# tphakala/go-audio-resampler

Hardware: AMD Instinct MI355X
Metric: Msamples/s resampled (float32, 44.1k→48k QualityHigh) + RMS error vs Go ref (higher is better)
Workload: dtype f32

## Files before the change

### go-audio-resampler_amd/csrc/gar_engine.cpp

```cpp
#include <hip/hip_runtime.h>
#include <immintrin.h>

#include <algorithm>
#include <chrono>
#include <atomic>
#include <cmath>
#include <condition_variable>
#include <cstdio>
#include <cstdlib>
#include <cstring>
#include <functional>
#include <memory>
#include <mutex>
#include <string>
#include <thread>
#include <type_traits>
#include <vector>

#include "gar.h"
#include "gar_design.hpp"
#include "gar_hxs_launch.hpp"
#include "gar_kernels.hpp"
#include "gar_plan.hpp"
#include "gar_pool.hpp"
// ... 133 lines not shown
    d.hRbK0 = p.rbAligned ? p.rbK0.data() : nullptr;
    for (size_t rb = 0; p.rbAligned && rb + 1 < p.rbStart.size(); ++rb)
        d.maxPrb = std::max(d.maxPrb, p.rbStart[rb + 1] - p.rbStart[rb]);
    if (dry) return d;
    if (p.f64) A.upload(p.A64); else A.upload(p.A32);
    std::vector<int> t = p.progTable();
    const std::vector<int> rt = p.redTable();
    const size_t redOff = t.size();
    t.insert(t.end(), rt.begin(), rt.end());
    const size_t rbOff = t.size();
    t.insert(t.end(), p.rbStart.begin(), p.rbStart.end());
    T.upload(t);
    d.A = A.p;
    d.progs = static_cast<const int*>(T.p);
    d.reds = static_cast<const int*>(T.p) + redOff;
    d.rbStart = p.rbAligned ? static_cast<const int*>(T.p) + rbOff : nullptr;
    return d;
}

void attachExact(const BgPlan& p, DevBuf& X, StageRT& s, BgDev& d, bool dry) {
    d.xRowMax = p.rowMax;
    d.xTwoStage = p.twoStage ? 1 : 0;
    d.xT1 = s.d.dft.taps;
    d.xT2 = s.d.poly.taps;
    if (dry) return;
    const size_t nr = p.rows.size(), ni = p.rowInfo.size();
    const size_t listOff = (nr * 8 + ni * 4 + 15) / 16 * 16;
    X.ensure(listOff + kBgNfListBytes);
    HIPCHK(hipMemcpy(X.p, p.rows.data(), nr * 8, hipMemcpyHostToDevice));
    HIPCHK(hipMemcpy(static_cast<char*>(X.p) + nr * 8, p.rowInfo.data(), ni * 4, hipMemcpyHostToDevice));
    HIPCHK(hipMemset(static_cast<char*>(X.p) + listOff, 0, kBgNfListBytes));
    d.xRows = static_cast<const double*>(X.p);
    d.xInfo = reinterpret_cast<const int*>(static_cast<const char*>(X.p) + nr * 8);
    d.nfList = reinterpret_cast<int*>(static_cast<char*>(X.p) + listOff);
    if (p.twoStage) {
        if (!s.xBankA.p) s.xBankA.upload(s.d.poly.a);
        if (!s.xBankC.p) s.xBankC.upload(s.d.dft.c);
        d.xPolyA = static_cast<const double*>(s.xBankA.p);
        d.xDftC = static_cast<const double*>(s.xBankC.p);
    }
}

template <class T>
void uploadBank(const std::vector<double>& v, DevBuf& b) {
    std::vector<T> c(v.begin(), v.end());
    b.upload(c);
}

bool buildStage(StageRT& s, bool f64, bool hx, bool dry, std::string& err) {
    s.f64 = f64;
    hx = hx && !f64;
    const EngineDesign& d = s.d;
    if (d.kind == EngineKind::Cubic) return true;
    if (d.kind == EngineKind::DftOnly || d.kind == EngineKind::DftPoly) {
        if (!buildBgPlan(firFromDft(d.dft), f64, s.dftP)) { err = "DFT plan"; return false; }
        s.dftD = uploadPlan(s.dftP, s.dftA, s.dftT, dry);
        attachExact(s.dftP, s.dftX, s, s.dftD, dry);
        if (hx) attachHx(firFromDft(d.dft), s.dftH, s.dftD, dry, d);
    }
    if (d.kind == EngineKind::Decim) {
        if (!buildBgPlan(firFromDecim(d.decim), f64, s.decimP)) { err = "decimator plan"; return false; }
        s.decimD = uploadPlan(s.decimP, s.decimA, s.decimT, dry);
        attachExact(s.decimP, s.decimX, s, s.decimD, dry);
        if (hx) attachHx(firFromDecim(d.decim), s.decimH, s.decimD, dry, d);
    }
    if (d.kind == EngineKind::DftPoly) {
        if (firComposite(d.dft, d.poly, s.compositeFir) && buildBgPlan(s.compositeFir, f64, s.fusedP)) {
            s.fused = true;
            s.fusedD = uploadPlan(s.fusedP, s.fusedA, s.fusedT, dry);
            attachExact(s.fusedP, s.fusedX, s, s.fusedD, dry);
            if (hx) attachHx(s.compositeFir, s.fusedH, s.fusedD, dry, d);
        }
        PolyDev& p = s.polyD;
        p.f64 = f64 ? 1 : 0;
        p.L = d.poly.L;
        p.T = d.poly.taps;
        p.step = d.poly.step;
        if (!dry) {
            if (f64) {
                uploadBank<double>(d.poly.a, s.pa); uploadBank<double>(d.poly.b, s.pb);
                uploadBank<double>(d.poly.cc, s.pc); uploadBank<double>(d.poly.d, s.pd);
            } else {
                uploadBank<float>(d.poly.a, s.pa); uploadBank<float>(d.poly.b, s.pb);
                uploadBank<float>(d.poly.cc, s.pc); uploadBank<float>(d.poly.d, s.pd);
            }
            p.a = s.pa.p; p.b = s.pb.p; p.c = s.pc.p; p.d = s.pd.p;
            std::vector<double> il(4 * d.poly.a.size());
            for (size_t i = 0; i < d.poly.a.size(); ++i) {
                il[4 * i] = d.poly.a[i]; il[4 * i + 1] = d.poly.b[i]; il[4 * i + 2] = d.poly.cc[i]; il[4 * i + 3] = d.poly.d[i];
            }
            if (f64) uploadBank<double>(il, s.pabcd); else uploadBank<float>(il, s.pabcd);
            p.abcd = s.pabcd.p;
        }
    }
    return true;
}

int stageLatency(const EngineDesign& d) {
    if (d.kind == EngineKind::Cubic) return 2;
    int lat = 0;
    if ((d.kind == EngineKind::DftOnly || d.kind == EngineKind::DftPoly) && d.dft.factor > 1)
        lat += (d.dft.taps * d.dft.factor) / 2;
    if (d.kind == EngineKind::DftPoly) lat += d.poly.taps / 2;
    return lat;
}

struct Counters {
    bool staged = false;
    int64_t x_count = 0;
    int64_t dft_hist = 0;
    int64_t poly_hist = 0;
    int64_t at = 0;
    int64_t u_base = 0;
    int64_t u_count = 0;
    int64_t dec_hist = 0;
    int dec_phase = 0;
    int64_t y_count = 0;
    double cub_phase = 0.0;
};

int64_t cntDft(Counters& s, const DftBank& b, int64_t n) {
    if (b.factor == 1) return n;
    if (n == 0) return 0;
    s.x_count += n;
    s.dft_hist += n;
    if (s.dft_hist < b.taps) return 0;
    const int64_t p = s.dft_hist - b.taps + 1;
    s.dft_hist -= p;
    return p * b.factor;
}

int64_t cntPoly(Counters& s, const PolyBank& b, int64_t m, bool& quirk) {
    if (m == 0) return 0;
    s.poly_hist += m;
    s.u_count += m;
    const int64_t numIn = s.poly_hist - b.taps + 1;
    if (numIn <= 0) return 0;
    const int64_t L = b.L;
    const int64_t limit = (numIn * L) << 16;
    const int64_t nout = (limit - s.at + b.step - 1) / b.step;
    if (nout <= 0) return 0;
    const int64_t at = s.at + nout * b.step;
    const int64_t consumed = (at >> 16) / L;
    if (consumed > 0 && consumed <= s.poly_hist) {
        s.poly_hist -= consumed;
        s.u_base += consumed;
    } else if (consumed > s.poly_hist) {
        quirk = true;
    }
    s.at = at - ((consumed * L) << 16);
    return nout;
}

int64_t cntDecim(Counters& s, const DecimBank& b, int64_t n) {
    if (b.factor == 1) return n;
    if (n == 0) return 0;
    s.x_count += n;
    s.dec_hist += n;
    if (s.dec_hist < b.taps) return 0;
    const int64_t nf = s.dec_hist - b.taps + 1;
    const int64_t nout = s.dec_phase < nf ? (nf - s.dec_phase + b.factor - 1) / b.factor : 0;
    if (nout == 0) return 0;
    s.dec_phase = static_cast<int>(((s.dec_phase - nf) % b.factor + b.factor) % b.factor);
    s.dec_hist -= nf;
    return nout;
}

namespace {
struct CubicRot {
    int F = 0;
    int64_t S = 0, P0 = 0;
};
bool cubicRotation(double step, double ph, CubicRot& r) {
    int e = 0;
    (void)std::frexp(step, &e);
    r.F = 53 - e;
    if (r.F < 1 || r.F > 60) return false;
    const double Sd = std::ldexp(step, r.F), Pd = std::ldexp(ph, r.F);
    if (Sd != std::floor(Sd) || Pd != std::floor(Pd) || Pd < 0.0 || Pd >= Sd) return false;
    r.S = static_cast<int64_t>(Sd);
    r.P0 = static_cast<int64_t>(Pd);
    const int64_t one = int64_t(1) << r.F;
    int bits = 0;
    for (uint64_t v = static_cast<uint64_t>(one + r.S - 1); v; v >>= 1) ++bits;
    const int64_t grid = bits > 53 ? (int64_t(1) << (bits - 53)) : 1;
    return r.S % grid == 0 && r.P0 % grid == 0 && one % grid == 0;
}
}

int64_t cntCubic(Counters& s, double ratio, int64_t n, std::vector<CubicSeg>* segs, int* segLen = nullptr) {
    const double step = 1.0 / ratio;
    CubicRot rot;
    if (n > 0 && cubicRotation(step, s.cub_phase, rot)) {
        const __int128 one = static_cast<__int128>(1) << rot.F, S = rot.S, P0 = rot.P0;
        auto phaseAt = [&](int64_t i) {
            __int128 v = (P0 - static_cast<__int128>(i) * one) % S;
            return v < 0 ? v + S : v;
        };
        auto outsBefore = [&](int64_t i, __int128 Pi) {
            return static_cast<int64_t>((static_cast<__int128>(i) * one + Pi - P0) / S);
        };
        if (segs)
            for (int64_t i = 0; i < n; i += (segLen ? *segLen : kCubicSegInputs)) {
                const __int128 Pi = phaseAt(i);
                segs->push_back({std::ldexp(static_cast<double>(static_cast<int64_t>(Pi)), -rot.F), s.y_count + outsBefore(i, Pi),
                                 s.x_count + i});
            }
        const __int128 Pn = phaseAt(n);
        const int64_t nout = outsBefore(n, Pn);
        s.cub_phase = std::ldexp(static_cast<double>(static_cast<int64_t>(Pn)), -rot.F);
        s.x_count += n;
        return nout;
    }
    if (segLen) *segLen = static_cast<int>(kCubicSegInputs);
    double ph = s.cub_phase;
    int64_t nout = 0;
    for (int64_t i = 0; i < n; ++i) {
        if (segs && i % kCubicSegInputs == 0) segs->push_back({ph, s.y_count + nout, s.x_count + i});
        while (ph < 1.0) {
            ++nout;
            ph += step;
        }
        ph -= 1.0;
    }
    s.cub_phase = ph;
    s.x_count += n;
    return nout;
}

struct Hist {
    DevBuf buf[2];
    int cur = 0;
    int64_t base = 0, len = 0;
    bool zero = false;
    void* ptr() const { return zero ? nullptr : buf[cur].p; }
    void clear() { base = 0; len = 0; zero = false; }
};

struct StageDev {
    Hist xh;
    Hist uh;
};

struct InView {
    const void* p = nullptr;
    int64_t fs = 0, cs = 0;
    int f64 = 0;
    int pcm = 0;
    int64_t n = 0;
    bool zeros = false;
};

struct OutView {
    void* p = nullptr;
    int64_t fs = 0, cs = 0;
    int f64 = 0;
    int pcm = 0;
};

struct PinBuf {
    void* p = nullptr;
    size_t cap = 0;
    hipEvent_t ev = nullptr;
    bool pending = false;
    PinBuf() = default;
    PinBuf(const PinBuf&) = delete;
    PinBuf& operator=(const PinBuf&) = delete;
    PinBuf(PinBuf&& o) noexcept : p(o.p), cap(o.cap), ev(o.ev), pending(o.pending) { o.p = nullptr; o.ev = nullptr; o.cap = 0; o.pending = false; }
    PinBuf& operator=(PinBuf&& o) noexcept {
        if (this != &o) {
            release();
            p = o.p; cap = o.cap; ev = o.ev; pending = o.pending;
            o.p = nullptr; o.ev = nullptr; o.cap = 0; o.pending = false;
        }
        return *this;
    }
    ~PinBuf() { release(); }
    void release() {
        if (ev) { (void)hipEventSynchronize(ev); (void)hipEventDestroy(ev); }
        if (p) (void)hipHostFree(p);
        p = nullptr; ev = nullptr; cap = 0; pending = false;
    }
    void* acquire(size_t bytes) {
        if (pending) HIPCHK(hipEventSynchronize(ev));
        pending = false;
        if (!ev) HIPCHK(hipEventCreateWithFlags(&ev, hipEventDisableTiming));
        if (bytes > cap) {
            if (p) HIPCHK(hipHostFree(p));
            p = nullptr;
            cap = 0;
            const size_t nb = bytes + bytes / 2 + 4096;
            HIPCHK(hipHostMalloc(&p, nb, hipHostMallocDefault));
            cap = nb;
        }
        return p;
    }
    void issued(hipStream_t s) {
        HIPCHK(hipEventRecord(ev, s));
        pending = true;
    }
};

struct HostBuf {
    void* p = nullptr;
    size_t cap = 0;
    unsigned flags = 0;
    HostBuf() = default;
    explicit HostBuf(unsigned f) : flags(f) {}
    HostBuf(const HostBuf&) = delete;
    HostBuf& operator=(const HostBuf&) = delete;
    ~HostBuf() { release(); }
    void release() {
        if (p) (void)hipHostFree(p);
        p = nullptr;
        cap = 0;
    }
    void* ensure(size_t bytes) {
        if (bytes <= cap) return p;
        release();
        const size_t nb = bytes + bytes / 4 + 4096;
        HIPCHK(hipHostMalloc(&p, nb, hipHostMallocMapped | flags));
        cap = nb;
        return p;
    }
};

inline void forSlices(int C, int64_t n, size_t bytesPerSample, const std::function<void(int, int64_t, int64_t)>& f) {
    const size_t total = static_cast<size_t>(C) * static_cast<size_t>(std::max<int64_t>(n, 0)) * bytesPerSample;
    if (total < (size_t(1) << 20)) {
        for (int c = 0; c < C; ++c) f(c, 0, n);
        return;
    }
    Pool& pool = Pool::get();
    const int J = pool.workers() * 2;
    if (C >= J) {
        pool.run(J, [&](int j) {
            for (int c = static_cast<int>(static_cast<int64_t>(C) * j / J); c < static_cast<int64_t>(C) * (j + 1) / J; ++c) f(c, 0, n);
        });
        return;
    }
    const int per = std::max<int>(1, (J + C - 1) / C);
    const int64_t step = (n + per - 1) / per;
    pool.run(C * per, [&](int i) {
        const int c = i / per, k = i - c * per;
        const int64_t lo = k * step, hi = std::min<int64_t>(n, lo + step);
        if (lo < hi) f(c, lo, hi);
    });
}

struct Group {
    int c0 = 0, C = 1;
    std::vector<Counters> cnt;
    int64_t statIn = 0, statOut = 0;
    std::vector<StageDev> dev;
    std::vector<DevBuf> tmp;
    DevBuf utmp;
    PinBuf cubPin[2];
    int cubCur = 0;
    std::vector<CubicSeg> cubSegs;
};

}
}

struct gar_resampler {
    bool newPath = true;
    int channels = 1;
    double ratio = 1.0;
    bool f64 = true;
    bool hx = false;
    bool dry = false;
    int device = 0;
    bool engineF32Io = false;
    hipStream_t stream = nullptr;
    hipEvent_t orderEv = nullptr;
    hipStream_t lastStream = nullptr;
    bool orderValid = false;
    bool unordered = false;
    bool multiStream = false;
    bool poisoned = false;
    hipEvent_t failEv = nullptr;
    bool failEvValid = false;
    int* errHost = nullptr;
    int* errDev = nullptr;
    gar_config cfg{};
    std::vector<std::unique_ptr<gar::StageRT>> stages;
    std::vector<gar::Group> groups;
    gar::DevBuf inStage, outStage;
    gar::HostBuf hostIn{hipHostMallocWriteCombined | hipHostMallocCoherent}, hostOut{hipHostMallocCoherent};
    std::vector<int64_t> scratchSizes;
    bool profile = false;
    uint32_t profileKinds = 0x3f;
    struct Ev { int tag; hipEvent_t a, b; };
    std::vector<Ev> events;
    std::vector<std::pair<hipEvent_t, hipEvent_t>> evPool;
    double profiledMs[6] = {0, 0, 0, 0, 0, 0};
    int64_t profiledLaunches[6] = {0, 0, 0, 0, 0, 0};
    std::vector<float> launchMs[6], readMs[6];
};

namespace gar {
namespace {

using Handle = gar_resampler;

constexpr size_t kPinKeep = size_t(64) << 20;
void trimHost(Handle* h) {
    if (h->hostIn.cap > kPinKeep) h->hostIn.release();
    if (h->hostOut.cap > kPinKeep) h->hostOut.release();
}

struct Ctx {
    Handle* h;
    Group* g;
    hipStream_t s;
    bool launch;
};

template <class L>
hipError_t timed(Ctx& x, int tag, L&& launch) {
    if (!x.h->profile || !((x.h->profileKinds >> tag) & 1u)) return launch();
    hipEvent_t a, b;
    if (!x.h->evPool.empty()) {
        a = x.h->evPool.back().first;
        b = x.h->evPool.back().second;
        x.h->evPool.pop_back();
    } else {
        HIPCHK(hipEventCreateWithFlags(&a, hipEventDisableSystemFence));
        HIPCHK(hipEventCreateWithFlags(&b, hipEventDisableSystemFence));
    }
    HIPCHK(hipEventRecord(a, x.s));
    const hipError_t e = launch();
    HIPCHK(hipEventRecord(b, x.s));
    x.h->events.push_back({tag, a, b});
    return e;
}

hipError_t timedBg(Ctx& x, int tag, const BgDev& p, const SrcDesc& src, const OutDesc& od, int C,
                   HistCopy* hc = nullptr) {
    return timed(x, tag, [&] { return launchBg(p, src, od, C, x.s, hc); });
}

SrcDesc mkSrc(const Hist& hs, int C, int64_t x0, const InView& in) {
    SrcDesc s{};
    s.hist = hs.ptr();
    s.hist_base = hs.base;
    s.hist_len = hs.len;
    s.hist_ld = C;
    s.in = in.zeros ? nullptr : in.p;
    s.in_base = x0;
    s.in_len = in.zeros ? 0 : in.n;
    s.in_fs = in.fs;
    s.in_cs = in.cs;
    s.in_f64 = in.f64;
    s.in_pcm = in.zeros ? 0 : in.pcm;
    s.valid_end = in.zeros ? x0 : x0 + in.n;
    return s;
}

thread_local int* g_curErr = nullptr;

OutDesc mkOut(const OutView& o, int64_t o0, int64_t n) {
    OutDesc d{};
    d.err = g_curErr;
    d.out = o.p;
    d.o0 = o0;
    d.fs = o.fs;
    d.cs = o.cs;
    d.f64 = o.f64;
    d.pcm = o.pcm;
    d.o_lo = o0;
    d.o_hi = o0 + n;
    return d;
}

void hist_update(Ctx& x, Hist& hs, const SrcDesc& src, int64_t k0, int64_t k1) {
    const int C = x.g->C;
    const int tc = x.h->f64 ? 8 : 4;
    if (k1 < k0) k1 = k0;
    if (!x.launch) { hs.base = k0; hs.len = k1 - k0; hs.zero = false; return; }
    const int other = 1 - hs.cur;
    hs.buf[other].ensure(static_cast<size_t>(std::max<int64_t>(k1 - k0, 1)) * C * tc);
    HIPCHK(launchGather(x.h->f64, src, hs.buf[other].p, k0, k1 - k0, C, x.s));
    hs.cur = other;
    hs.base = k0;
    hs.len = k1 - k0;
    hs.zero = false;
}

template <class L>
void withHist(Ctx& x, Hist& hs, const SrcDesc& src, int64_t k0, int64_t k1, bool launch, L&& l) {
    HistCopy hc;
    const int other = 1 - hs.cur;
    if (x.launch && launch && k1 > k0) {
        hs.buf[other].ensure(static_cast<size_t>(k1 - k0) * x.g->C * (x.h->f64 ? 8 : 4));
        hc.dst = hs.buf[other].p;
        hc.t0 = k0;
        hc.n = k1 - k0;
    }
    if (x.launch && launch) HIPCHK(l(&hc));
    if (hc.done) {
        hs.cur = other;
        hs.base = k0;
        hs.len = k1 - k0;
        hs.zero = false;
    } else {
        hist_update(x, hs, src, k0, k1);
    }
}

void materialize(Ctx& x, StageRT& rt, Counters& c, StageDev& dv, const SrcDesc& xsrc) {
    const int C = x.g->C;
    const int tc = rt.tc();
    if (x.launch) {
        Hist& uh = dv.uh;
        const int other = 1 - uh.cur;
        const int64_t n = c.u_count - c.u_base;
        uh.buf[other].ensure(static_cast<size_t>(std::max<int64_t>(n, 1)) * C * tc);
        OutView ov{uh.buf[other].p, C, 1, rt.f64 ? 1 : 0};
        HIPCHK(timedBg(x, 1, rt.dftD, xsrc, mkOut(ov, c.u_base, n), C));
        uh.cur = other;
        uh.base = c.u_base;
        uh.len = n;
    } else {
        dv.uh.base = c.u_base;
        dv.uh.len = c.u_count - c.u_base;
    }
    hist_update(x, dv.xh, xsrc, c.x_count - c.dft_hist, c.x_count);
    c.staged = true;
}

int64_t stageProcess(Ctx& x, int si, const InView& in, const OutView& out) {
    StageRT& rt = *x.h->stages[si];
    Counters& c = x.g->cnt[si];
    StageDev& dv = x.g->dev[si];
    const int C = x.g->C;
    const EngineDesign& d = rt.d;
    const int64_t n = in.n;
    if (n == 0) return 0;
    switch (d.kind) {
        case EngineKind::Cubic: {
            const int64_t x0 = c.x_count;
            std::vector<CubicSeg>* segs = x.launch ? &x.g->cubSegs : nullptr;
            if (segs) segs->clear();
            const SrcDesc src = mkSrc(dv.xh, C, x0, in);
            const int64_t y0 = c.y_count;
            int segLen = n * C <= (int64_t(1) << 20) ? kCubicSegInputsShort : static_cast<int>(kCubicSegInputs);
            const int64_t nout = cntCubic(c, d.ratio, n, segs, &segLen);
            if (x.launch && nout > 0) {
                PinBuf& pb = x.g->cubPin[x.g->cubCur];
                x.g->cubCur ^= 1;
                void* hp = pb.acquire(segs->size() * sizeof(CubicSeg));
                std::memcpy(hp, segs->data(), segs->size() * sizeof(CubicSeg));
                HIPCHK(timed(x, 5, [&] {
                    return launchCubic(rt.f64 ? 1 : 0, static_cast<const CubicSeg*>(hp), static_cast<int64_t>(segs->size()),
                                       c.x_count, 1.0 / d.ratio, src, mkOut(out, y0, nout), C, x.s, segLen);
                }));
                pb.issued(x.s);
            }
            hist_update(x, dv.xh, src, std::max<int64_t>(0, c.x_count - 3), c.x_count);
            c.y_count += nout;
            return nout;
        }
        case EngineKind::Passthrough: {
            if (x.launch && !in.zeros) {
                HIPCHK(launchCopy(in.p, in.f64, in.fs, in.cs, out.p, out.f64, out.fs, out.cs, n, C, x.s));
            }
            c.y_count += n;
            return n;
        }
        case EngineKind::DftOnly: {
            const int64_t x0 = c.x_count;
            const int64_t y0 = c.y_count;
            const int64_t nout = cntDft(c, d.dft, n);
            const SrcDesc src = mkSrc(dv.xh, C, x0, in);
            withHist(x, dv.xh, src, c.x_count - c.dft_hist, c.x_count, nout > 0,
                     [&](HistCopy* hc) { return timedBg(x, 1, rt.dftD, src, mkOut(out, y0, nout), C, hc); });
            c.y_count += nout;
            return nout;
        }
        case EngineKind::Decim: {
            const int64_t x0 = c.x_count;
            const int64_t y0 = c.y_count;
            const int64_t nout = cntDecim(c, d.decim, n);
            const SrcDesc src = mkSrc(dv.xh, C, x0, in);
            withHist(x, dv.xh, src, c.x_count - c.dec_hist, c.x_count, nout > 0,
                     [&](HistCopy* hc) { return timedBg(x, 2, rt.decimD, src, mkOut(out, y0, nout), C, hc); });
            c.y_count += nout;
            return nout;
        }
        case EngineKind::DftPoly: {
            const int64_t x0 = c.x_count;
            const int64_t y0 = c.y_count;
            const Counters before = c;
            const SrcDesc xsrc = mkSrc(dv.xh, C, x0, in);
            const int64_t nu = cntDft(c, d.dft, n);
            bool quirk = false;
            const int64_t nout = cntPoly(c, d.poly, nu, quirk);
            if (!c.staged) {
                if (quirk) {
                    if (x.launch && nout > 0) HIPCHK(timedBg(x, 0, rt.fusedD, xsrc, mkOut(out, y0, nout), C));
                    materialize(x, rt, c, dv, xsrc);
                } else {
                    withHist(x, dv.xh, xsrc, c.u_base / 2, c.x_count, nout > 0, [&](HistCopy* hc) {
                        return timedBg(x, 0, rt.fusedD, xsrc, mkOut(out, y0, nout), C, hc);
                    });
                }
            } else {
                const int64_t p0 = before.x_count - before.dft_hist;
                const int64_t dy0 = p0 * d.dft.factor;
                InView uin;
                if (x.launch) x.g->utmp.ensure(static_cast<size_t>(std::max<int64_t>(nu, 1)) * C * rt.tc());
                withHist(x, dv.xh, xsrc, c.x_count - c.dft_hist, c.x_count, nu > 0, [&](HistCopy* hc) {
                    OutView uv{x.g->utmp.p, C, 1, rt.f64 ? 1 : 0};
                    return timedBg(x, 1, rt.dftD, xsrc, mkOut(uv, dy0, nu), C, hc);
                });
                uin.p = x.g->utmp.p; uin.fs = C; uin.cs = 1; uin.f64 = rt.f64 ? 1 : 0; uin.n = nu;
                const SrcDesc usrc = mkSrc(dv.uh, C, before.u_count, uin);
                if (x.launch && nout > 0) {
                    PolyDev p = rt.polyD;
                    p.at0 = before.at;
                    p.u_base = before.u_base;
                    p.m0 = before.y_count;
                    HIPCHK(timed(x, 4, [&] { return launchPoly(p, usrc, mkOut(out, y0, nout), nout, C, x.s); }));
                }
                if (nu > 0) hist_update(x, dv.uh, usrc, c.u_base, c.u_count);
            }
            c.y_count += nout;
            return nout;
        }
        default:
            throw DevError{hipErrorNotSupported, "unsupported stage"};
    }
}

int64_t stageFlush(Ctx& x, int si, const OutView& out) {
    StageRT& rt = *x.h->stages[si];
    Counters& c = x.g->cnt[si];
    StageDev& dv = x.g->dev[si];
    const int C = x.g->C;
    const EngineDesign& d = rt.d;
    InView z;
    z.zeros = true;
    switch (d.kind) {
        case EngineKind::Passthrough:
            return 0;
        case EngineKind::DftOnly:
            if (c.dft_hist == 0) return 0;
            z.n = d.dft.taps;
            return stageProcess(x, si, z, out);
        case EngineKind::Decim:
            if (c.dec_hist == 0) return 0;
            z.n = d.decim.taps;
            return stageProcess(x, si, z, out);
        case EngineKind::DftPoly: {
            if (!c.staged) {
                InView none;
                none.zeros = true;
                const SrcDesc xsrc = mkSrc(dv.xh, C, c.x_count, none);
                Counters t = c;
                bool quirk = false;
                int64_t nA = 0, nB = 0;
                if (t.dft_hist > 0) nA = cntPoly(t, d.poly, cntDft(t, d.dft, d.dft.taps), quirk);
                if (t.poly_hist > 0) nB = cntPoly(t, d.poly, d.poly.taps, quirk);
                if (!quirk) {
                    const int64_t y0 = c.y_count, n = nA + nB;
                    if (x.launch && n > 0) HIPCHK(timedBg(x, 3, rt.fusedD, xsrc, mkOut(out, y0, n), C));
                    c = t;
                    c.y_count = y0 + n;
                    c.staged = true;
                    dv.xh.base = c.x_count - c.dft_hist;
                    dv.xh.len = c.dft_hist;
                    dv.xh.zero = true;
                    dv.uh.base = c.u_base;
                    dv.uh.len = c.u_count - c.u_base;
                    dv.uh.zero = true;
                    return n;
                }
                materialize(x, rt, c, dv, xsrc);
            }
            int64_t total = 0;
            if (c.dft_hist > 0) {
                z.n = d.dft.taps;
                total += stageProcess(x, si, z, out);
            }
            if (c.poly_hist > 0) {
                const int64_t y0 = c.y_count;
                const Counters before = c;
                bool quirk = false;
                const int64_t nout = cntPoly(c, d.poly, d.poly.taps, quirk);
                InView uz;
                uz.zeros = true;
                uz.n = d.poly.taps;
                const SrcDesc usrc = mkSrc(dv.uh, C, before.u_count, uz);
                OutView o2 = out;
                if (x.launch && nout > 0) {
                    const int es = out.f64 ? 8 : 4;
                    o2.p = static_cast<char*>(out.p) + total * out.fs * es;
                    PolyDev p = rt.polyD;
                    p.at0 = before.at;
                    p.u_base = before.u_base;
                    p.m0 = before.y_count;
                    HIPCHK(timed(x, 4, [&] { return launchPoly(p, usrc, mkOut(o2, y0, nout), nout, C, x.s); }));
                }
                hist_update(x, dv.uh, usrc, c.u_base, c.u_count);
                c.y_count += nout;
                total += nout;
            }
            return total;
        }
        default:
            return 0;
    }
}

OutView offsetView(const OutView& o, int64_t rows) {
    OutView r = o;
    if (o.p) r.p = static_cast<char*>(o.p) + rows * o.fs * (o.pcm ? pcmBytes(o.pcm) : (o.f64 ? 8 : 4));
    return r;
}

int64_t chainProcess(Ctx& x, const InView& in, const OutView& out, std::vector<int64_t>& sizes) {
    const int ns = static_cast<int>(x.h->stages.size());
    sizes.assign(ns, 0);
    if (ns == 0) {
        if (x.launch && in.n > 0)
            HIPCHK(launchCopy(in.p, in.f64, in.fs, in.cs, out.p, out.f64, out.fs, out.cs, in.n, x.g->C, x.s));
        return in.n;
    }
    InView cur = in;
    for (int i = 0; i < ns; ++i) {
        const bool last = i == ns - 1;
        OutView o = out;
        if (!last) {
            const int tc = x.h->f64 ? 8 : 4;
            if (x.launch) {
                x.g->tmp[i].ensure(static_cast<size_t>(std::max<int64_t>(x.h->scratchSizes[i], 1)) * x.g->C * tc);
                o = OutView{x.g->tmp[i].p, x.g->C, 1, x.h->f64 ? 1 : 0};
            }
        }
        int64_t m = 0;
        if (cur.n >= 1) m = stageProcess(x, i, cur, o);
        sizes[i] = m;
        InView nx;
        nx.p = o.p; nx.fs = o.fs; nx.cs = o.cs; nx.f64 = o.f64; nx.n = m;
        cur = nx;
    }
    return cur.n;
}

int64_t chainFlush(Ctx& x, const OutView& out, std::vector<int64_t>& sizes) {
    const int ns = static_cast<int>(x.h->stages.size());
    sizes.assign(ns, 0);
    if (ns == 0) return 0;
    InView pending;
    for (int i = 0; i < ns; ++i) {
        const bool last = i == ns - 1;
        OutView o = out;
        if (!last && x.launch) {
            const int tc = x.h->f64 ? 8 : 4;
            x.g->tmp[i].ensure(static_cast<size_t>(std::max<int64_t>(x.h->scratchSizes[i], 1)) * x.g->C * tc);
            o = OutView{x.g->tmp[i].p, x.g->C, 1, x.h->f64 ? 1 : 0};
        }
        int64_t m = 0;
        if (pending.n > 0) m += stageProcess(x, i, pending, o);
        m += stageFlush(x, i, offsetView(o, m));
        sizes[i] = m;
        InView nx;
        nx.p = o.p; nx.fs = o.fs; nx.cs = o.cs; nx.f64 = o.f64; nx.n = m;
        pending = nx;
    }
    return pending.n;
}

Group* groupOf(Handle* h, int ch) {
    for (auto& g : h->groups)
        if (ch >= g.c0 && ch < g.c0 + g.C) return &g;
    return nullptr;
}

Group freshGroup(Handle* h, int c0, int C) {
    Group g;
    g.c0 = c0;
    g.C = C;
    const size_t ns = h->stages.size();
    g.cnt.assign(ns, Counters());
    g.dev.resize(ns);
    g.tmp.resize(ns);
    for (size_t i = 0; i < ns; ++i)
        if (!h->stages[i]->fused) g.cnt[i].staged = true;
    return g;
}

Group splitCopy(Handle* h, Group& g, int k0, int kc) {
    Group ng = freshGroup(h, g.c0 + k0, kc);
    const int tc = h->f64 ? 8 : 4;
    for (size_t i = 0; i < h->stages.size(); ++i) {
        ng.cnt[i] = g.cnt[i];
        ng.statIn = g.statIn;
        ng.statOut = g.statOut;
        Hist* src[2] = {&g.dev[i].xh, &g.dev[i].uh};
        Hist* dst[2] = {&ng.dev[i].xh, &ng.dev[i].uh};
        for (int k = 0; k < 2; ++k) {
            dst[k]->base = src[k]->base;
            dst[k]->len = src[k]->len;
            dst[k]->zero = src[k]->zero;
            if (!h->dry && src[k]->len > 0 && !src[k]->zero) {
                dst[k]->buf[0].ensure(static_cast<size_t>(src[k]->len) * kc * tc);
                const char* sp = static_cast<const char*>(src[k]->ptr()) + static_cast<size_t>(k0) * tc;
                HIPCHK(launchCopy(sp, h->f64, g.C, 1, dst[k]->buf[0].p, h->f64, kc, 1, src[k]->len, kc, h->stream));
            }
        }
    }
    return ng;
}

void isolate(Handle* h, int ch) {
    Group* g = groupOf(h, ch);
    if (!g || g->C == 1) return;
    std::vector<Group> out;
    for (auto& gg : h->groups) {
        if (&gg != g) { out.push_back(std::move(gg)); continue; }
        const int k = ch - gg.c0;
        if (k > 0) out.push_back(splitCopy(h, gg, 0, k));
        out.push_back(splitCopy(h, gg, k, 1));
        if (k + 1 < gg.C) out.push_back(splitCopy(h, gg, k + 1, gg.C - k - 1));
    }
    if (!h->dry) HIPCHK(hipStreamSynchronize(h->stream));
    h->groups = std::move(out);
}

int64_t simulate(Handle* h, Group& g, int64_t n, bool flush, std::vector<int64_t>& sizes) {
    Group sim;
    sim.c0 = g.c0;
    sim.C = g.C;
    sim.cnt = g.cnt;
    sim.dev.resize(g.dev.size());
    for (size_t i = 0; i < g.dev.size(); ++i) {
        sim.dev[i].xh.base = g.dev[i].xh.base; sim.dev[i].xh.len = g.dev[i].xh.len;
        sim.dev[i].uh.base = g.dev[i].uh.base; sim.dev[i].uh.len = g.dev[i].uh.len;
    }
    Ctx x{h, &sim, nullptr, false};
    InView in;
    in.n = n;
    OutView o;
    return flush ? chainFlush(x, o, sizes) : chainProcess(x, in, o, sizes);
}

void countStats(const Handle* h, Group& g, int64_t nIn, int64_t nOut, bool flush) {
    if (!flush) {
        if (nIn <= 0) return;
        g.statIn += nIn;
        g.statOut += nOut;
        return;
    }
    const bool cubicEngine = !h->newPath && h->stages.size() == 1 && h->stages[0]->d.kind == EngineKind::Cubic;
    if (!cubicEngine) g.statOut += nOut;
}

int64_t runGroup(Handle* h, Group& g, const InView& in, const OutView& out, bool flush, hipStream_t s,
                 int64_t cap, gar_status& st) {
    std::vector<int64_t> sizes;
    const int64_t n = simulate(h, g, in.n, flush, sizes);
    if (n > cap) { st = GAR_ERR_BUFFER_TOO_SMALL; return n; }
    st = GAR_OK;
    if (h->dry) {
        Ctx x{h, &g, nullptr, false};
        std::vector<int64_t> s2;
        OutView o;
        if (flush) chainFlush(x, o, s2); else chainProcess(x, in, o, s2);
        countStats(h, g, in.n, n, flush);
        return n;
    }
    h->scratchSizes = sizes;
    Ctx x{h, &g, s, true};
    std::vector<int64_t> s2;
    const int64_t got = flush ? chainFlush(x, out, s2) : chainProcess(x, in, out, s2);
    if (got != n) { st = GAR_ERR_INTERNAL; g_err = "size mismatch between count and launch"; }
    else countStats(h, g, in.n, got, flush);
    return got;
}

gar_status guard(gar_status s, const char* msg) {
    if (s != GAR_OK) g_err = msg;
    return s;
}

struct DeviceGuard {
    int prev = -1;
    bool set = false;
    explicit DeviceGuard(int dev) {
        if (dev < 0) return;
        if (hipGetDevice(&prev) == hipSuccess && prev != dev && hipSetDevice(dev) == hipSuccess) set = true;
    }
    ~DeviceGuard() {
        if (set) (void)hipSetDevice(prev);
    }
    DeviceGuard(const DeviceGuard&) = delete;
    DeviceGuard& operator=(const DeviceGuard&) = delete;
};

thread_local bool g_launchLimit = false;

template <class F>
gar_status wrap(F&& f) {
    g_launchLimit = false;
    try {
        return f();
    } catch (const DevError& e) {
        if (e.e == hipErrorInvalidConfiguration && !launchLimitMsg().empty()) {
            g_err = launchLimitMsg() + " (at " + e.what + ")";
            launchLimitMsg().clear();
            g_launchLimit = true;
            return GAR_ERR_INVALID_ARGUMENT;
        }
        g_err = std::string("HIP error ") + hipGetErrorString(e.e) + " at " + e.what;
        return GAR_ERR_DEVICE;
    } catch (const std::bad_alloc&) {
        g_err = "out of host memory";
        return GAR_ERR_INTERNAL;
    }
}

bool devFault(Handle* h) {
    if (!h->errHost) return false;
    const int v = __atomic_load_n(h->errHost, __ATOMIC_ACQUIRE);
    if (!v) return false;
    h->poisoned = true;
    const char* what = v == kHxtErrLoadWait   ? "hxt_kernel: a compute wave's LDS load-progress wait expired"
                       : v == kHxtErrSlotWait ? "hxt_kernel: a loader's LDS ring-slot wait expired"
                                              : "unknown code";
    g_err = std::string("device error reported by ") + what + " (code " + std::to_string(v) +
            "); outputs of the launch are invalid; call Reset";
    return true;
}

void drainOrder(Handle* h) {
    if (h->orderValid) (void)hipEventSynchronize(h->orderEv);
    else if (h->unordered) (void)hipDeviceSynchronize();
    h->unordered = false;
}

template <class F>
gar_status callOn(Handle* h, hipStream_t s, F&& f, bool hostSynced = false) {
    if (h->poisoned) return guard(GAR_ERR_DEVICE, "handle unusable after an earlier device error; call Reset");
    if (h->dry) return wrap(f);
    if (devFault(h)) return GAR_ERR_DEVICE;
    DeviceGuard dg(h->device);
    struct ErrScope {
        int* prev;
        explicit ErrScope(int* e) : prev(g_curErr) { g_curErr = e; }
        ~ErrScope() { g_curErr = prev; }
    } es(h->errDev);
    gar_status st = wrap([&]() -> gar_status {
        if (h->orderValid && h->lastStream != s) {
            HIPCHK(hipStreamWaitEvent(s, h->orderEv, 0));
        } else if (h->unordered && h->lastStream != s) {
            HIPCHK(hipDeviceSynchronize());
            h->unordered = false;
            h->multiStream = true;
        }
        const gar_status r = f();
        if (hostSynced) {
            h->orderValid = false;
            h->unordered = false;
        } else if (h->multiStream) {
            HIPCHK(hipEventRecord(h->orderEv, s));
            h->lastStream = s;
            h->orderValid = true;
        } else {
            h->lastStream = s;
            h->orderValid = false;
            h->unordered = true;
        }
        return r;
    });
    if (st == GAR_ERR_DEVICE || (st == GAR_ERR_INVALID_ARGUMENT && g_launchLimit)) {
        h->poisoned = true;
        h->failEvValid = h->failEv && hipEventRecord(h->failEv, s) == hipSuccess;
    } else if (st == GAR_OK && hostSynced && devFault(h)) {
        st = GAR_ERR_DEVICE;
    }
    return st;
}

gar_quality_spec presetSpec(int32_t preset) {
    gar_quality_spec q{};
    switch (preset) {
        case GAR_QUALITY_QUICK: q = {GAR_QUALITY_QUICK, 8, 50.0, 0.7, 1.0, 0}; break;
        case GAR_QUALITY_LOW: q = {GAR_QUALITY_LOW, 16, 50.0, 0.80, 0.95, 0}; break;
        case GAR_QUALITY_MEDIUM: q = {GAR_QUALITY_MEDIUM, 16, 50.0, 0.90, 0.98, 0}; break;
        case GAR_QUALITY_HIGH: q = {GAR_QUALITY_HIGH, 24, 50.0, 0.95, 0.99, 0}; break;
        case GAR_QUALITY_VERYHIGH: q = {GAR_QUALITY_VERYHIGH, 32, 50.0, 0.99, 0.995, 0}; break;
        default: q = {GAR_QUALITY_MEDIUM, 0, 0, 0, 0, 0}; break;
    }
    return q;
}

gar_status validate(const gar_config* c) {
    if (!c) return guard(GAR_ERR_INVALID_CONFIG, "invalid resampler configuration: config is nil");
    if (!(c->input_rate > 0) || !(c->output_rate > 0))
        return guard(GAR_ERR_INVALID_CONFIG, "invalid resampler configuration: sample rates must be positive");
    if (c->channels < 1) return guard(GAR_ERR_INVALID_CONFIG, "invalid resampler configuration: channels must be at least 1");
    if (c->channels > 256) return guard(GAR_ERR_INVALID_CONFIG, "invalid resampler configuration: too many channels (max 256)");
    if (c->compute_dtype == GAR_F16 || c->compute_dtype == GAR_BF16)
        return guard(GAR_ERR_INVALID_CONFIG, "invalid resampler configuration: f16 / bf16 are sample types of the device entry points, not compute types");
    if (c->compute_dtype == GAR_PCM24_PACKED)
        return guard(GAR_ERR_INVALID_CONFIG, "invalid resampler configuration: packed 24-bit PCM is a sample type of the device entry points, not a compute type");
    const double r = c->output_rate / c->input_rate;
    if (r < 1.0 / 256.0 || r > 256.0)
        return guard(GAR_ERR_INVALID_CONFIG, "invalid resampler configuration: resampling ratio out of range");
    const gar_quality_spec& q = c->quality;
    if (q.preset == GAR_QUALITY_CUSTOM) {
        if (q.precision < 8 || q.precision > 33) return guard(GAR_ERR_INVALID_CONFIG, "precision must be 8-33 bits");
        if (q.phase_response < 0 || q.phase_response > 100) return guard(GAR_ERR_INVALID_CONFIG, "phase response must be 0-100");
        if (q.passband_end <= 0 || q.passband_end >= 1) return guard(GAR_ERR_INVALID_CONFIG, "passband end must be in (0, 1)");
        if (q.stopband_begin <= q.passband_end || q.stopband_begin > 1)
            return guard(GAR_ERR_INVALID_CONFIG, "stopband begin must be in (passband_end, 1]");
    }
    return GAR_OK;
}

bool hxEnabled() {
    static const bool on = [] {
        const char* e = std::getenv("GAR_HX");
        return !(e && e[0] == '0');
    }();
    return on;
}

gar_status initDevice(Handle* h) {
    if (h->dry) return GAR_OK;
    int n = 0;
    if (hipGetDeviceCount(&n) != hipSuccess || n <= h->device) {
        g_err = "no HIP device visible (the GPU path requires an MI355X / gfx950)";
        return GAR_ERR_DEVICE;
    }
    HIPCHK(hipSetDevice(h->device));
    HIPCHK(hipStreamCreateWithFlags(&h->stream, hipStreamNonBlocking));
    HIPCHK(hipEventCreateWithFlags(&h->orderEv, hipEventDisableTiming | hipEventDisableSystemFence));
    HIPCHK(hipEventCreateWithFlags(&h->failEv, hipEventDisableTiming));
    void* w = nullptr;
    HIPCHK(hipHostMalloc(&w, 64, hipHostMallocMapped | hipHostMallocCoherent));
    h->errHost = static_cast<int*>(w);
    *h->errHost = 0;
    void* d = nullptr;
    HIPCHK(hipHostGetDevicePointer(&d, w, 0));
    h->errDev = static_cast<int*>(d);
    return GAR_OK;
}

gar_status addStage(Handle* h, double inRate, double outRate, Quality q) {
    auto rt = std::make_unique<StageRT>();
    std::string err;
    if (!designEngine(inRate, outRate, q, rt->d, err)) return guard(GAR_ERR_INVALID_CONFIG, err.c_str());
    if (!buildStage(*rt, h->f64, h->hx, h->dry, err)) {
        g_err = err;
        return GAR_ERR_INTERNAL;
    }
    h->stages.push_back(std::move(rt));
    return GAR_OK;
}

gar_status newCommon(gar_config* cfg, int32_t nstreams, gar_resampler** out) {
    if (!out) return guard(GAR_ERR_INVALID_ARGUMENT, "out is NULL");
    *out = nullptr;
    gar_status s = validate(cfg);
    if (s != GAR_OK) return s;
    if (nstreams < 1) return guard(GAR_ERR_INVALID_CONFIG, "n_streams must be >= 1");
    if (cfg->quality.preset != GAR_QUALITY_CUSTOM) cfg->quality = presetSpec(cfg->quality.preset);
    auto h = std::make_unique<Handle>();
    h->newPath = true;
    h->cfg = *cfg;
    h->channels = cfg->channels * nstreams;
    h->ratio = cfg->output_rate / cfg->input_rate;
    h->f64 = cfg->compute_dtype != GAR_F32 && cfg->compute_dtype != GAR_F32_EXACT;
    h->hx = cfg->compute_dtype == GAR_F32 && hxEnabled();
    h->dry = cfg->dry_run != 0;
    h->device = cfg->device;
    DeviceGuard dg(h->dry ? -1 : cfg->device);
    return wrap([&]() -> gar_status {
        gar_status st = initDevice(h.get());
        if (st != GAR_OK) return st;
        const int prec = cfg->quality.precision;
        const std::vector<StageSpec> specs = buildPipeline(h->ratio, prec);
        for (const StageSpec& sp : specs) {
            if (sp.type == StageType::Cubic) {
                st = addStage(h.get(), 1.0, sp.ratio, Quality::Quick);
                if (st != GAR_OK) return st;
                continue;
            }
            const double ir = 48000.0;
            st = addStage(h.get(), ir, ir * sp.ratio, precisionToEngineQuality(prec));
            if (st != GAR_OK) return st;
        }
        h->groups.push_back(freshGroup(h.get(), 0, h->channels));
        *out = h.release();
        return GAR_OK;
    });
}

gar_status newEngineCommon(double in_rate, double out_rate, Quality q, int32_t dtype, bool dry, gar_resampler** out) {
    if (!out) return guard(GAR_ERR_INVALID_ARGUMENT, "out is NULL");
    *out = nullptr;
    if (dtype != GAR_F64 && dtype != GAR_F32 && dtype != GAR_F32_EXACT) return guard(GAR_ERR_INVALID_ARGUMENT, "unknown dtype");
    if (!(in_rate > 0) || !(out_rate > 0)) return guard(GAR_ERR_INVALID_CONFIG, "sample rates must be positive");
    auto h = std::make_unique<gar_resampler>();
    h->newPath = false;
    h->channels = 1;
    h->dry = dry;
    h->f64 = dtype == GAR_F64;
    h->hx = dtype == GAR_F32 && hxEnabled();
    h->engineF32Io = dtype != GAR_F64;
    h->ratio = out_rate / in_rate;
    DeviceGuard dg(dry ? -1 : 0);
    return wrap([&]() -> gar_status {
        gar_status st = initDevice(h.get());
        if (st != GAR_OK) return st;
        st = addStage(h.get(), in_rate, out_rate, q);
        if (st != GAR_OK) return st;
        h->ratio = h->stages[0]->d.ratio;
        h->groups.push_back(freshGroup(h.get(), 0, 1));
        *out = h.release();
        return GAR_OK;
    });
}

int64_t estimate(const Handle* h, int64_t n) {
    return static_cast<int64_t>(static_cast<double>(n) * h->ratio) + 64;
}

__attribute__((target("avx2"))) void cvtD2F(float* d, const double* s, int64_t n) {
    int64_t i = 0;
    for (; i + 8 <= n; i += 8)
        _mm256_storeu_ps(d + i, _mm256_set_m128(_mm256_cvtpd_ps(_mm256_loadu_pd(s + i + 4)),
                                                _mm256_cvtpd_ps(_mm256_loadu_pd(s + i))));
    for (; i < n; ++i) d[i] = static_cast<float>(s[i]);
}
__attribute__((target("avx2"))) void cvtF2DStream(double* d, const float* s, int64_t n) {
    int64_t i = 0;
    for (; i < n && (reinterpret_cast<uintptr_t>(d + i) & 31); ++i) d[i] = static_cast<double>(s[i]);
    for (; i + 8 <= n; i += 8) {
        _mm256_stream_pd(d + i, _mm256_cvtps_pd(_mm_loadu_ps(s + i)));
        _mm256_stream_pd(d + i + 4, _mm256_cvtps_pd(_mm_loadu_ps(s + i + 4)));
    }
    for (; i < n; ++i) d[i] = static_cast<double>(s[i]);
    _mm_sfence();
}
__attribute__((target("avx2"))) void copyD2DStream(double* d, const double* s, int64_t n) {
    int64_t i = 0;
    for (; i < n && (reinterpret_cast<uintptr_t>(d + i) & 31); ++i) d[i] = s[i];
    for (; i + 8 <= n; i += 8) {
        _mm256_stream_pd(d + i, _mm256_loadu_pd(s + i));
        _mm256_stream_pd(d + i + 4, _mm256_loadu_pd(s + i + 4));
    }
    for (; i < n; ++i) d[i] = s[i];
    _mm_sfence();
}
bool hostAvx2() {
    static const bool a = __builtin_cpu_supports("avx2");
    return a;
}

template <class T>
void packChannel(void* dst, bool f64, const T* src, int64_t lo, int64_t hi) {
    if constexpr (std::is_same<T, double>::value) {
        if (!f64 && hostAvx2()) {
            cvtD2F(static_cast<float*>(dst) + lo, src + lo, hi - lo);
            return;
        }
    }
    if (f64) {
        double* d = static_cast<double*>(dst);
        for (int64_t i = lo; i < hi; ++i) d[i] = static_cast<double>(src[i]);
    } else {
        float* d = static_cast<float*>(dst);
        for (int64_t i = lo; i < hi; ++i) d[i] = static_cast<float>(src[i]);
    }
}
template <class T>
void unpackChannel(T* dst, bool f64, const void* src, int64_t lo, int64_t hi) {
    if constexpr (std::is_same<T, double>::value) {
        if (hostAvx2() && hi - lo >= 64) {
            if (f64) copyD2DStream(dst + lo, static_cast<const double*>(src) + lo, hi - lo);
            else cvtF2DStream(dst + lo, static_cast<const float*>(src) + lo, hi - lo);
            return;
        }
    }
    if (f64) {
        const double* s = static_cast<const double*>(src);
        for (int64_t i = lo; i < hi; ++i) dst[i] = static_cast<T>(s[i]);
    } else {
        const float* s = static_cast<const float*>(src);
        for (int64_t i = lo; i < hi; ++i) dst[i] = static_cast<T>(s[i]);
    }
}

template <class T>
gar_status monoCall(Handle* h, int ch, const T* in, int64_t n, T* out, int64_t cap, int64_t* nOut, bool flush,
                    bool intoSemantics) {
    if (!h) return guard(GAR_ERR_INVALID_ARGUMENT, "nil resampler");
// ... 341 lines not shown
int64_t gar_device_output_size(const gar_resampler* r, int64_t frames) {
    if (!r || r->groups.size() != 1) return -1;
    gar_resampler* h = const_cast<gar_resampler*>(r);
    std::vector<int64_t> s;
    return simulate(h, h->groups[0], frames, false, s);
}

int64_t gar_device_flush_size(const gar_resampler* r) {
    if (!r || r->groups.size() != 1) return -1;
    gar_resampler* h = const_cast<gar_resampler*>(r);
    std::vector<int64_t> s;
    return simulate(h, h->groups[0], 0, true, s);
}

gar_status gar_process_device(gar_resampler* r, const void* in, int32_t in_dtype, int64_t in_fs, int64_t in_cs,
                              int64_t frames, int32_t channels, void* out, int32_t out_dtype, int64_t out_fs,
                              int64_t out_cs, int64_t out_cap, int64_t* out_frames, void* stream) {
    if (!r) return guard(GAR_ERR_INVALID_ARGUMENT, "nil resampler");
    if (out_frames) *out_frames = 0;
    if (channels != r->channels) {
        g_err = "expected " + std::to_string(r->channels) + " channels, got " + std::to_string(channels);
        return GAR_ERR_CHANNEL_MISMATCH;
    }
    if (frames < 0) return guard(GAR_ERR_INVALID_ARGUMENT, "negative length");
    if (frames > 0 && !in) return guard(GAR_ERR_INVALID_ARGUMENT, "input is NULL");
    if (!ioTypeOk(in_dtype) || !ioTypeOk(out_dtype)) return guard(GAR_ERR_INVALID_ARGUMENT, "unknown sample type");
    if (r->groups.size() != 1) return guard(GAR_ERR_NOT_SUPPORTED, "channels are not in lockstep (per-channel calls were made)");
    return callOn(r, static_cast<hipStream_t>(stream), [&]() -> gar_status {
        hipStream_t s = static_cast<hipStream_t>(stream);
        const bool fuseAny = pcmFusable(r);
        bool fuse = fuseAny && in_dtype != GAR_PCM24_PACKED;
        InView iv;
        iv.p = in;
        iv.f64 = in_dtype == GAR_F64 ? 1 : 0;
        iv.fs = in_fs;
        iv.cs = in_cs;
        iv.n = frames;
        if (isNarrow(in_dtype)) {
            iv.f64 = 0;
            if (fuse) {
                iv.pcm = in_dtype;
            } else if (!r->dry) {
                const int cf = r->f64 ? 1 : 0;
                r->inStage.ensure(static_cast<size_t>(std::max<int64_t>(frames, 1)) * r->channels * (cf ? 8 : 4));
                HIPCHK(launchConvert(in, in_dtype, in_fs, in_cs, r->inStage.p, cf, r->channels, 1, frames, r->channels, s));
                iv.p = r->inStage.p;
                iv.f64 = cf;
                iv.fs = r->channels;
                iv.cs = 1;
            }
        }
        fuse = fuseAny && out_dtype != GAR_PCM24_PACKED;
        OutView ov;
        ov.p = out;
        ov.f64 = out_dtype == GAR_F64 ? 1 : 0;
        ov.fs = out_fs;
        ov.cs = out_cs;
        const bool stageOut = isNarrow(out_dtype) && !fuse && !r->dry;
        if (isNarrow(out_dtype)) {
            ov.f64 = 0;
            if (fuse) ov.pcm = out_dtype;
        }
        if (stageOut) {
            std::vector<int64_t> sz;
            const int64_t need = simulate(r, r->groups[0], frames, false, sz);
            const int cf = r->f64 ? 1 : 0;
            r->outStage.ensure(static_cast<size_t>(std::max<int64_t>(need, 1)) * r->channels * (cf ? 8 : 4));
            ov.p = r->outStage.p;
            ov.f64 = cf;
            ov.fs = r->channels;
            ov.cs = 1;
        }
        gar_status st;
        const int64_t got = runGroup(r, r->groups[0], iv, ov, false, s, out_cap, st);
        if (st == GAR_OK && stageOut && got > 0)
            HIPCHK(launchConvert(r->outStage.p, r->f64 ? 1 : 0, r->channels, 1, out, out_dtype, out_fs, out_cs, got,
                                 r->channels, s));
        if (st == GAR_OK && out_frames) *out_frames = got;
        return st;
    });
}

gar_status gar_flush_device(gar_resampler* r, int32_t channels, void* out, int32_t out_dtype, int64_t out_fs,
                            int64_t out_cs, int64_t out_cap, int64_t* out_frames, void* stream) {
    if (!r) return guard(GAR_ERR_INVALID_ARGUMENT, "nil resampler");
    if (out_frames) *out_frames = 0;
    if (channels != r->channels) {
        g_err = "expected " + std::to_string(r->channels) + " channels, got " + std::to_string(channels);
        return GAR_ERR_CHANNEL_MISMATCH;
    }
    if (!ioTypeOk(out_dtype)) return guard(GAR_ERR_INVALID_ARGUMENT, "unknown sample type");
    if (r->groups.size() != 1) return guard(GAR_ERR_NOT_SUPPORTED, "channels are not in lockstep");
    return callOn(r, static_cast<hipStream_t>(stream), [&]() -> gar_status {
        hipStream_t s = static_cast<hipStream_t>(stream);
        const bool fuse = pcmFusable(r) && out_dtype != GAR_PCM24_PACKED;
        OutView ov;
        ov.p = out;
        ov.f64 = out_dtype == GAR_F64 ? 1 : 0;
        ov.fs = out_fs;
        ov.cs = out_cs;
        const bool stageOut = isNarrow(out_dtype) && !fuse && !r->dry;
        if (isNarrow(out_dtype)) {
            ov.f64 = 0;
            if (fuse) ov.pcm = out_dtype;
        }
        if (stageOut) {
            std::vector<int64_t> sz;
            const int64_t need = simulate(r, r->groups[0], 0, true, sz);
            const int cf = r->f64 ? 1 : 0;
            r->outStage.ensure(static_cast<size_t>(std::max<int64_t>(need, 1)) * r->channels * (cf ? 8 : 4));
            ov.p = r->outStage.p;
            ov.f64 = cf;
            ov.fs = r->channels;
            ov.cs = 1;
        }
        gar_status st;
        const int64_t got = runGroup(r, r->groups[0], InView(), ov, true, s, out_cap, st);
        if (st == GAR_OK && stageOut && got > 0)
            HIPCHK(launchConvert(r->outStage.p, r->f64 ? 1 : 0, r->channels, 1, out, out_dtype, out_fs, out_cs, got,
                                 r->channels, s));
        if (st == GAR_OK && out_frames) *out_frames = got;
        return st;
    });
}

void gar_reset(gar_resampler* r) {
    if (!r) return;
    DeviceGuard dg(r->dry ? -1 : r->device);
    try {
        if (!r->dry) (void)devFault(r);
        if (r->poisoned) {
            if (r->failEvValid) (void)hipEventSynchronize(r->failEv);
            if (r->stream) (void)hipStreamSynchronize(r->stream);
            drainOrder(r);
            (void)hipGetLastError();
            if (r->errHost) __atomic_store_n(r->errHost, 0, __ATOMIC_RELEASE);
            r->groups.clear();
            r->groups.push_back(freshGroup(r, 0, r->channels));
            r->poisoned = false;
            r->failEvValid = false;
            r->orderValid = false;
            return;
        }
        if (r->groups.size() == 1 && r->groups[0].c0 == 0 && r->groups[0].C == r->channels) {
            gar::Group& g = r->groups[0];
            for (size_t i = 0; i < g.cnt.size(); ++i) {
                g.cnt[i] = gar::Counters();
                g.cnt[i].staged = !r->stages[i]->fused;
            }
            for (auto& d : g.dev) {
                d.xh.clear();
                d.uh.clear();
            }
            g.statIn = g.statOut = 0;
            return;
        }
        if (r->stream) (void)hipStreamSynchronize(r->stream);
        drainOrder(r);
        r->groups.clear();
        r->groups.push_back(freshGroup(r, 0, r->channels));
    } catch (...) {
    }
}

double gar_get_ratio(const gar_resampler* r) { return r ? r->ratio : 0.0; }

int32_t gar_get_latency(const gar_resampler* r) {
    if (!r || r->stages.empty()) return 0;
    int tot = 0;
    for (const auto& s : r->stages) tot += static_cast<int>(static_cast<double>(stageLatency(s->d)) * s->d.ratio);
    return tot;
}

int32_t gar_channels(const gar_resampler* r) { return r ? r->channels : 0; }

gar_status gar_get_statistics(const gar_resampler* r, int32_t ch, int64_t* samples_in, int64_t* samples_out) {
    if (samples_in) *samples_in = 0;
    if (samples_out) *samples_out = 0;
    if (!r || ch < 0 || ch >= r->channels) return guard(GAR_ERR_INVALID_ARGUMENT, "channel out of range");
    const Group* g = groupOf(const_cast<gar_resampler*>(r), ch);
    if (!g) return guard(GAR_ERR_INTERNAL, "channel without a group");
    if (samples_in) *samples_in = g->statIn;
    if (samples_out) *samples_out = g->statOut;
    return GAR_OK;
}

gar_status gar_get_info(const gar_resampler* r, gar_info* info) {
    if (!r || !info) return GAR_ERR_INVALID_ARGUMENT;
    std::memset(info, 0, sizeof(*info));
    std::snprintf(info->algorithm, sizeof(info->algorithm), "%s", "multi-stage");
    info->latency = gar_get_latency(r);
    const int64_t es = 8;
    int64_t perCh = 0;
    for (size_t j = 0; j <= r->stages.size(); ++j)
        perCh += (j == 0 && r->cfg.max_input_size > 0 ? r->cfg.max_input_size * 2 : 8192) * 8;
    for (const auto& s : r->stages) {
        const EngineDesign& d = s->d;
        if ((d.kind == EngineKind::DftOnly || d.kind == EngineKind::DftPoly) && d.dft.factor > 1)
            perCh += static_cast<int64_t>(d.dft.factor) * d.dft.taps * es + 2 * static_cast<int64_t>(d.dft.taps) * es;
        if (d.kind == EngineKind::DftPoly)
            perCh += static_cast<int64_t>(d.poly.L) * d.poly.taps * es + 2 * static_cast<int64_t>(d.poly.taps) * es;
    }
    info->memory_usage = perCh * r->channels;
    if (!r->stages.empty()) {
        const EngineDesign& d = r->stages[0]->d;
        int len = 0;
        if ((d.kind == EngineKind::DftOnly || d.kind == EngineKind::DftPoly) && d.dft.factor > 1) len += d.dft.taps * d.dft.factor;
        if (d.kind == EngineKind::DftPoly) len += d.poly.taps * d.poly.L;
        if (d.kind == EngineKind::Cubic) {
            info->filter_length = 4;
            info->phases = 0;
            info->memory_usage += 64 * r->channels;
        } else {
            info->filter_length = len;
            info->phases = d.kind == EngineKind::DftPoly ? d.poly.L : 0;
            info->simd_enabled = 1;
            std::snprintf(info->simd_type, sizeof(info->simd_type), "%s", "gfx950 MFMA (HIP)");
        }
    }
    return GAR_OK;
}

const char* gar_status_string(gar_status s) {
    switch (s) {
        case GAR_OK: return "ok";
        case GAR_ERR_INVALID_CONFIG: return "invalid resampler configuration";
        case GAR_ERR_BUFFER_TOO_SMALL: return "output buffer too small";
        case GAR_ERR_NOT_SUPPORTED: return "operation not supported";
        case GAR_ERR_CHANNEL_MISMATCH: return "channel count mismatch";
        case GAR_ERR_DEVICE: return "device error";
        case GAR_ERR_INTERNAL: return "internal error";
        case GAR_ERR_INVALID_ARGUMENT: return "invalid argument";
    }
    return "unknown";
}

const char* gar_last_error(void) { return g_err.c_str(); }

void gar_profile_enable(gar_resampler* r, int32_t on) {
    if (!r) return;
    r->profile = on != 0;
}

gar_status gar_dev_half_convert(int32_t half_type, const double* in, int64_t n, uint16_t* from_f64, uint16_t* from_f32,
                                float* widened) {
    if (!isHalf(half_type) || n < 0 || (n > 0 && !in)) return guard(GAR_ERR_INVALID_ARGUMENT, "bad half conversion arguments");
    for (int64_t i = 0; i < n; ++i) {
        const uint16_t b = halfOfF64(in[i], half_type);
        if (from_f64) from_f64[i] = b;
        if (from_f32) from_f32[i] = halfOfF32(static_cast<float>(in[i]), half_type);
        if (widened) widened[i] = halfToF32(b, half_type);
    }
    return GAR_OK;
}

gar_status gar_dev_pcm24_convert(const double* in, int64_t n, uint8_t* packed, int32_t* unpacked) {
    if (n < 0 || (n > 0 && !in)) return guard(GAR_ERR_INVALID_ARGUMENT, "bad packed 24-bit conversion arguments");
    static_assert(kSampPcm24P == GAR_PCM24_PACKED, "the kernels' packed 24-bit code is the ABI's");
    for (int64_t i = 0; i < n; ++i) {
        uint8_t b[3];
        pcmWrite(b, 0, kSampPcm24P, in[i]);
        if (packed) std::memcpy(packed + 3 * i, b, 3);
        if (unpacked) unpacked[i] = pcm24Load(b);
    }
    return GAR_OK;
}

gar_status gar_dev_hxs_plan(const gar_resampler* r, int32_t stage, int32_t in_type, int64_t in_fs, int64_t in_cs,
                            uint64_t in_addr, int64_t in_base, int64_t in_len, int64_t valid_end, uint64_t hist_addr,
                            int64_t hist_len, int64_t hist_ld, int32_t out_type, uint64_t out_addr, int64_t o0,
                            int64_t out_fs, int64_t out_cs, int64_t o_lo, int64_t o_hi, int32_t channels,
                            int32_t cu_count, int64_t hist_keep, char* buf, int64_t cap) {
    if (!r || !buf || cap < 1 || stage < 0 || stage >= static_cast<int32_t>(r->stages.size()) || channels < 1 ||
        cu_count < 1 || !ioTypeOk(in_type) || !ioTypeOk(out_type))
        return guard(GAR_ERR_INVALID_ARGUMENT, "bad launch-plan arguments");
    const gar::StageRT& st = *r->stages[stage];
    const HxDev* hx = st.fusedD.hx ? st.fusedD.hx : (st.dftD.hx ? st.dftD.hx : st.decimD.hx);
    if (!hx) return guard(GAR_ERR_INVALID_ARGUMENT, "the stage has no split-f16 plan");
    SrcDesc src{};
    src.hist = reinterpret_cast<const void*>(static_cast<uintptr_t>(hist_addr));
    src.hist_len = hist_len;
    src.hist_ld = hist_ld;
    src.in = reinterpret_cast<const void*>(static_cast<uintptr_t>(in_addr));
    src.in_base = in_base; src.in_len = in_len; src.in_fs = in_fs; src.in_cs = in_cs;
    src.in_f64 = in_type == GAR_F64;
    src.in_pcm = isNarrow(in_type) ? in_type : 0;
    src.valid_end = valid_end;
    OutDesc od{};
    od.out = reinterpret_cast<void*>(static_cast<uintptr_t>(out_addr));
    od.o0 = o0; od.fs = out_fs; od.cs = out_cs;
    od.f64 = out_type == GAR_F64;
    od.pcm = isNarrow(out_type) ? out_type : 0;
    od.o_lo = o_lo; od.o_hi = o_hi;
    buf[0] = 0;
    if (o_hi <= o_lo) return GAR_OK;
    const gar::HxsLaunchPlan pl = gar::hxsPlanLaunch(*hx, src, od, channels, cu_count, gar::hxsReadKnobs(), hist_keep > 0, hist_keep);
    if (!pl.ok) std::snprintf(buf, static_cast<size_t>(cap), "not supported\n");
    else gar::hxsTraceLines(pl, od, channels, buf, static_cast<size_t>(cap));
    return GAR_OK;
}

int64_t gar_dev_pool_selftest(int32_t threads, int32_t iters, int32_t channels, int64_t frames) {
    if (threads < 1 || iters < 0 || channels < 1 || frames < 0) return -1;
    std::atomic<int64_t> bad{0};
    auto body = [&](int t) {
        const int channels_t = channels + t;
        std::vector<double> src(static_cast<size_t>(channels_t) * frames), dst(src.size());
        std::vector<float> mid(src.size());
        for (size_t i = 0; i < src.size(); ++i) src[i] = static_cast<double>((i * 2654435761u + t) % 65536) / 65536.0 - 0.5;
        for (int k = 0; k < iters; ++k) {
            std::fill(dst.begin(), dst.end(), -9.0);
            gar::forSlices(channels_t, frames, 12, [&](int c, int64_t lo, int64_t hi) {
                gar::packChannel<double>(mid.data() + static_cast<size_t>(c) * frames, false,
                                         src.data() + static_cast<size_t>(c) * frames, lo, hi);
            });
            gar::forSlices(channels_t, frames, 12, [&](int c, int64_t lo, int64_t hi) {
                gar::unpackChannel<double>(dst.data() + static_cast<size_t>(c) * frames, false,
                                           mid.data() + static_cast<size_t>(c) * frames, lo, hi);
            });
            int64_t b = 0;
            for (size_t i = 0; i < src.size(); ++i) b += dst[i] != static_cast<double>(static_cast<float>(src[i]));
            bad += b;
        }
    };
    std::vector<std::thread> th;
    for (int t = 1; t < threads; ++t) th.emplace_back(body, t);
    body(0);
    for (auto& x : th) x.join();
    return bad.load();
}

void gar_profile_kinds(gar_resampler* r, uint32_t kinds) {
    if (!r) return;
    r->profileKinds = kinds & 0x3fu;
}

gar_status gar_stage_state(const gar_resampler* r, int32_t stage, int32_t* fused_plan, int32_t* fused_now) {
    if (!r || !fused_plan || !fused_now || stage < 0 || stage >= static_cast<int32_t>(r->stages.size()))
        return GAR_ERR_INVALID_ARGUMENT;
    const gar::StageRT& st = *r->stages[stage];
    *fused_plan = st.fused ? 1 : 0;
    const gar::Group* g = r->groups.empty() ? nullptr : &r->groups[0];
    *fused_now = (st.fused && g && !g->cnt[stage].staged) ? 1 : 0;
    return GAR_OK;
}

gar_status gar_stage_geometry(const gar_resampler* r, int32_t stage, double* stage_ratio, gar_engine_geometry* geom) {
    if (!r || !geom || stage < 0 || stage >= static_cast<int32_t>(r->stages.size())) return GAR_ERR_INVALID_ARGUMENT;
    const gar::EngineDesign& d = r->stages[stage]->d;
    fillGeometry(d, geom);
    if (stage_ratio) *stage_ratio = d.ratio;
    return GAR_OK;
}

int32_t gar_num_stages(const gar_resampler* r) { return r ? static_cast<int32_t>(r->stages.size()) : 0; }

gar_status gar_profile_read(gar_resampler* r, int32_t kind, double* ms, int64_t* launches) {
    if (!r || kind < 0 || kind > 5) return GAR_ERR_INVALID_ARGUMENT;
    DeviceGuard dg(r->dry ? -1 : r->device);
    return wrap([&]() -> gar_status {
        for (auto& ev : r->events) {
            HIPCHK(hipEventSynchronize(ev.b));
            float t = 0;
            HIPCHK(hipEventElapsedTime(&t, ev.a, ev.b));
            r->profiledMs[ev.tag] += t;
            r->profiledLaunches[ev.tag] += 1;
            r->launchMs[ev.tag].push_back(t);
            r->evPool.emplace_back(ev.a, ev.b);
        }
        r->events.clear();
        if (ms) *ms = r->profiledMs[kind];
        if (launches) *launches = r->profiledLaunches[kind];
        r->profiledMs[kind] = 0;
        r->profiledLaunches[kind] = 0;
        r->readMs[kind].swap(r->launchMs[kind]);
        r->launchMs[kind].clear();
        return GAR_OK;
    });
}

gar_status gar_profile_launch_stats(gar_resampler* r, int32_t kind, double* min_ms, double* median_ms, double* max_ms) {
    if (!r || kind < 0 || kind > 5) return GAR_ERR_INVALID_ARGUMENT;
    std::vector<float> v = r->readMs[kind];
    if (v.empty()) {
        if (min_ms) *min_ms = 0;
        if (median_ms) *median_ms = 0;
        if (max_ms) *max_ms = 0;
        return GAR_OK;
    }
    std::sort(v.begin(), v.end());
    const size_t n = v.size();
    if (min_ms) *min_ms = v.front();
    if (max_ms) *max_ms = v.back();
    if (median_ms) *median_ms = n % 2 ? v[n / 2] : 0.5 * (static_cast<double>(v[n / 2 - 1]) + v[n / 2]);
    return GAR_OK;
}

gar_status gar_design_engine(double in_rate, double out_rate, int32_t q, gar_engine_geometry* geom, double* dft,
                             double* pa, double* pb, double* pc, double* pd, double* decim) {
    EngineDesign d;
    std::string err;
    if (!designEngine(in_rate, out_rate, static_cast<Quality>(q), d, err)) return guard(GAR_ERR_INVALID_CONFIG, err.c_str());
    if (geom) fillGeometry(d, geom);
    if (dft && !d.dft.c.empty()) std::memcpy(dft, d.dft.c.data(), d.dft.c.size() * 8);
    if (pa && !d.poly.a.empty()) std::memcpy(pa, d.poly.a.data(), d.poly.a.size() * 8);
    if (pb && !d.poly.b.empty()) std::memcpy(pb, d.poly.b.data(), d.poly.b.size() * 8);
    if (pc && !d.poly.cc.empty()) std::memcpy(pc, d.poly.cc.data(), d.poly.cc.size() * 8);
    if (pd && !d.poly.d.empty()) std::memcpy(pd, d.poly.d.data(), d.poly.d.size() * 8);
    if (decim && !d.decim.c.empty()) std::memcpy(decim, d.decim.c.data(), d.decim.c.size() * 8);
    return GAR_OK;
}

gar_status gar_design_composite(double in_rate, double out_rate, int32_t q, double* rows, int64_t* offsets) {
    EngineDesign d;
    std::string err;
    if (!designEngine(in_rate, out_rate, static_cast<Quality>(q), d, err)) return guard(GAR_ERR_INVALID_CONFIG, err.c_str());
    FirPeriodic f;
    if (d.kind != EngineKind::DftPoly || !firComposite(d.dft, d.poly, f)) return guard(GAR_ERR_NOT_SUPPORTED, "no composite FIR");
    size_t w = 0;
    for (const auto& r : f.rows) w = std::max(w, r.size());
    for (int r = 0; r < f.P; ++r) {
        if (offsets) offsets[r] = f.off[r];
        if (rows)
            for (size_t k = 0; k < w; ++k) rows[r * w + k] = k < f.rows[r].size() ? f.rows[r][k] : 0.0;
    }
    return GAR_OK;
}

}
```

### go-audio-resampler_amd/csrc/gar_hxs.hip

```cpp
#include <hip/hip_runtime.h>

#include <algorithm>
#include <cstdio>
#include <cstdlib>
#include <utility>
#include <vector>

#include "gar_hxs_launch.hpp"
#include "gar_hxt.hpp"

namespace gar {

#define GAR_HXS_EXT(NS, V) extern template hipError_t hxsLaunch<NS, V>(const HxsArgs&, size_t, int64_t, hipStream_t);
GAR_HXS_FOR_ALL(GAR_HXS_EXT)
#undef GAR_HXS_EXT
#define GAR_HXT_EXT(NS, F, V, L) extern template hipError_t hxtLaunch<NS, F, V, L>(const HxsArgs&, size_t, int64_t, hipStream_t);
GAR_HXT_FOR_A(GAR_HXT_EXT)
GAR_HXT_FOR_B(GAR_HXT_EXT)
#undef GAR_HXT_EXT
#define GAR_HXT_EXT_LEAN(NS, F, V, L, E) extern template hipError_t hxtLaunch<NS, F, V, L, E>(const HxsArgs&, size_t, int64_t, hipStream_t);
GAR_HXT_FOR_LEAN(GAR_HXT_EXT_LEAN)
#undef GAR_HXT_EXT_LEAN

namespace {
constexpr int kProfWords = 64 + 2 * 4096;
unsigned long long* profBuf(bool on) {
    static unsigned long long* p = nullptr;
    static bool init = false;
    if (!init) {
        init = true;
        if (on && hipMalloc(&p, kProfWords * sizeof(unsigned long long)) == hipSuccess) {
            (void)hipMemset(p, 0, kProfWords * sizeof(unsigned long long));
            (void)hipMemset(p + 10, 0xff, sizeof(unsigned long long));
            (void)hipMemset(p + 13, 0xff, sizeof(unsigned long long));
            std::atexit([] {
                static unsigned long long h[kProfWords] = {};
                if (hipDeviceSynchronize() == hipSuccess && hipMemcpy(h, p, sizeof(h), hipMemcpyDeviceToHost) == hipSuccess) {
                    const double nl = h[3] ? static_cast<double>(h[3]) : 1, nc = h[6] ? static_cast<double>(h[6]) : 1;
                    fprintf(stderr, "hxs prof per wave (cycles): loaders convert %.0f issue+wait %.0f (issue %.0f) barrier %.0f (life %.1f us) | compute convert+mfma %.0f barrier %.0f\n",
                            h[0] / nl, h[1] / nl, h[7] / nl, h[2] / nl, h[9] / nl / 100.0, h[4] / nc, h[5] / nc);
                    fprintf(stderr, "hxs loader pre-loop %.2f us, post-loop %.2f us; compute convert %.0f\n", h[8] / nl / 100.0, h[12] / nl / 100.0, h[15] / nc);
                    if (h[23]) fprintf(stderr, "hxs wave-0 first block (cycles): entry->window %.0f, window->steps done %.0f, ->exit (stores drained) %.0f, n %llu\n",
                                       static_cast<double>(h[20]) / h[23], static_cast<double>(h[21]) / h[23], static_cast<double>(h[22]) / h[23], h[23]);
                    if (h[23]) fprintf(stderr, "hxs wave-0: entry->A landed %.0f, entry->barrier 1 %.0f; wave entry spread in a workgroup %.0f, wave 0 after first wave %.0f\n",
                                       static_cast<double>(h[24]) / h[23], static_cast<double>(h[25]) / h[23], static_cast<double>(h[26]) / h[23], static_cast<double>(h[27]) / h[23]);
                    if (h[34]) fprintf(stderr, "hxt roles per block (cycles): compute wave 0 %.0f (waiting %.0f), loader 0 %.0f (waiting %.0f), n %llu\n",
                                       static_cast<double>(h[30]) / h[34], static_cast<double>(h[32]) / h[34], static_cast<double>(h[31]) / h[34],
                                       static_cast<double>(h[33]) / h[34], h[34]);
                    if (h[34]) fprintf(stderr, "hxt compute wave 0: entry -> first group %.0f cycles, last group -> exit %.0f cycles, periods %.0f, arrivals %.0f\n",
                                       static_cast<double>(h[35]) / h[34], static_cast<double>(h[36]) / h[34],
                                       static_cast<double>(h[37]) / h[34], static_cast<double>(h[38]) / h[34]);
                    if (h[34] && h[57]) fprintf(stderr, "hxt fill (cycles): entry -> A issued %.0f, -> fill barrier %.0f, -> first group %.0f; in-kernel clock %.3f GHz\n",
                                       static_cast<double>(h[53]) / h[34], static_cast<double>(h[54]) / h[34], static_cast<double>(h[55]) / h[34],
                                       0.1 * static_cast<double>(h[56]) / static_cast<double>(h[57]));
                    if (h[34]) fprintf(stderr, "hxt loader 0 phases (cycles): load data wait %.0f, conversion %.0f, arrival %.0f\n",
                                       static_cast<double>(h[50]) / h[34], static_cast<double>(h[51]) / h[34], static_cast<double>(h[52]) / h[34]);
                    if (h[44]) fprintf(stderr, "hxq wave 0 (cycles): entry->barrier 1 %.0f, ->image %.0f, ->MFMA+stores issued %.0f, ->drained %.0f, n %llu\n",
                                       static_cast<double>(h[40]) / h[44], static_cast<double>(h[41]) / h[44], static_cast<double>(h[42]) / h[44],
                                       static_cast<double>(h[43]) / h[44], h[44]);
                    fprintf(stderr, "hxs span: first start -> last end %.1f us; loader wave life min %.1f max %.1f us\n",
                            (h[11] - h[10]) / 100.0, h[13] / 100.0, h[14] / 100.0);
                    std::vector<std::pair<double, int>> v;
                    unsigned long long t0 = ~0ull;
                    for (int b = 0; b < 4096; ++b)
                        if (h[65 + 2 * b]) { v.push_back({h[65 + 2 * b] / 100.0, b}); t0 = std::min(t0, h[64 + 2 * b]); }
                    if (!v.empty()) {
                        std::vector<std::pair<double, int>> sv = v;
                        std::sort(sv.begin(), sv.end());
                        auto pc = [&](double q) { return sv[std::min(sv.size() - 1, static_cast<size_t>(q * sv.size()))].first; };
                        fprintf(stderr, "hxs WG life us: n %zu min %.1f p10 %.1f p50 %.1f p90 %.1f max %.1f |", sv.size(), sv.front().first, pc(0.1), pc(0.5), pc(0.9), sv.back().first);
                        for (int m = 0; m < 8; ++m) {
                            double s = 0; int n = 0;
                            for (auto& e : v) if (e.second % 8 == m) { s += e.first; ++n; }
                            fprintf(stderr, " x%d %.1f", m, n ? s / n : 0.0);
                        }
                        fprintf(stderr, "\n  slowest:");
                        for (size_t k = sv.size(); k-- > 0 && k + 8 >= sv.size();)
                            fprintf(stderr, " b%d %.1fus@+%.1f", sv[k].second, sv[k].first, (h[64 + 2 * sv[k].second] - t0) / 100.0);
                        fprintf(stderr, "\n");
                    }
                }
            });
        }
    }
    return p;
}

template <int NS, int NL>
hipError_t hxtFmtL(const HxsArgs& x, size_t lds, int64_t blocks, hipStream_t st, bool lean) {
    if constexpr (NS == kHxtLeanNS)
        if (lean && x.fmt == kFmtStereo && x.vst == kVstStereo) return hxtLaunch<NS, kFmtStereo, kVstStereo, NL, 1>(x, lds, blocks, st);
    if (x.fmt == kFmtStereo && x.vst == kVstStereo) return hxtLaunch<NS, kFmtStereo, kVstStereo, NL>(x, lds, blocks, st);
    if (x.fmt == kFmtRow16 && x.vst == kVstAny) return hxtLaunch<NS, kFmtRow16, kVstAny, NL>(x, lds, blocks, st);
    if (x.fmt == kFmtRow16 && x.vst == kVstRows) return hxtLaunch<NS, kFmtRow16, kVstRows, NL>(x, lds, blocks, st);
    if (x.fmt == kFmtRow32 && x.vst == kVstAny) return hxtLaunch<NS, kFmtRow32, kVstAny, NL>(x, lds, blocks, st);
    return hipErrorNotSupported;
}
template <int NS>
hipError_t hxtFmt(const HxsArgs& x, size_t lds, int64_t blocks, hipStream_t st, bool lean) {
    return hxtLoadersFor(x.ncomp) == 6 ? hxtFmtL<NS, 6>(x, lds, blocks, st, lean) : hxtFmtL<NS, 4>(x, lds, blocks, st, lean);
}

template <int NS>
hipError_t hxsVst(const HxsArgs& x, size_t lds, int64_t blocks, hipStream_t st) {
    switch (x.vst) {
        case kVstAny: return hxsLaunch<NS, kVstAny>(x, lds, blocks, st);
        case kVstRows: return hxsLaunch<NS, kVstRows>(x, lds, blocks, st);
        case kVstStereo: return hxsLaunch<NS, kVstStereo>(x, lds, blocks, st);
        case kVstStereoPcm16: return hxsLaunch<NS, kVstStereoPcm16>(x, lds, blocks, st);
        case kVstStereoHalf: return hxsLaunch<NS, kVstStereoHalf>(x, lds, blocks, st);
        default: return hxsLaunch<NS, kVstF64>(x, lds, blocks, st);
    }
}

HxsArgs hxsArgsOf(const HxsLaunchPlan& pl, const HxDev& p, const SrcDesc& src, const OutDesc& od, int C, const HxsKnobs& k) {
    HxsArgs x{};
    x.A = static_cast<const h8v*>(p.A);
    x.progs = p.progs;
    x.ea = p.ea;
    x.Pc = p.Pc; x.Qc = p.Qc; x.Kc = p.Kc; x.Kread = p.Kread; x.G = pl.G; x.C = C;
    x.nprog = p.nw;
    x.ncols = static_cast<int>(pl.ncols);
    x.nblocks = pl.nblocks;
    x.Np = static_cast<int>(pl.Np);
    x.ngroups = pl.ngroups;
    x.R = pl.R; x.Rt = pl.Rt; x.mirror = pl.mirror; x.Wg = pl.Wg;
    x.a_lo = pl.a_lo; x.a_hi = pl.a_hi;
    x.dbg = k.dbg;
    x.prof = profBuf(k.prof != 0);
    x.o_lo = od.o_lo; x.o_hi = od.o_hi;
    x.in_esz = pl.in_esz;
    x.in_pcm = src.in_pcm;
    x.in = reinterpret_cast<const char*>(pl.inBase);
    x.in_fs = src.in_fs;
    x.in_cs = src.in_cs;
    x.fastLo = pl.fastLo;
    x.fastHi = pl.fastHi;
    x.fmt = pl.fmt;
    x.small = pl.small;
    x.bigSmall = pl.bigSmall;
    x.nt = k.nt;
    x.xcdPair = pl.xcdPair;
    x.out_pcm = od.pcm;
    x.out_f64 = od.f64;
    x.out = reinterpret_cast<char*>(pl.outBase);
    x.out_fs = od.fs * pl.out_esz;
    x.out_cs = od.cs * pl.out_esz;
    x.vst = pl.vst;
    x.ncomp = pl.ncomp;
    for (int w = 0; w < kHxtMaxComp; ++w) x.role[w] = pl.role[w];
    const bool fault = pl.kernel == HxsKernel::Hxt && k.fault;
    x.err = od.err;
    x.pollMax = fault ? 1 << 12 : 1 << 24;
    x.faultNeed = fault ? 1 << 28 : 0;
    x.coop = std::max(0, std::min(2, k.coop));
    x.src = src;
    x.od = od;
    x.rows = p.rows;
    x.rowOff = p.rowOff;
    x.rowLen = p.rowLen;
    x.rowMax = p.rowMax;
    x.twoStage = p.twoStage;
    x.rowPh = p.rowPh;
    x.rowPar = p.rowPar;
    x.polyA = p.polyA;
    x.dftC = p.dftC;
    x.T1 = p.T1;
    x.T2 = p.T2;
    if (pl.qGroups > 0) {
        x.qOpt = pl.qOpt;
        x.qRbs = pl.qRbs;
        x.qGroups = pl.qGroups;
        for (int w = 0; w < p.nw; ++w) { x.qU0[w] = p.hU0[w]; x.qRbw[w] = p.hRbw[w]; }
    }
    return x;
}
}

hipError_t launchHxs(const HxDev& p, const SrcDesc& src, const OutDesc& od, int C, hipStream_t stream, HistCopy* hc) {
    if (od.o_hi <= od.o_lo) return hipSuccess;
    int dev = 0, ncu = 256;
    if (hipGetDevice(&dev) == hipSuccess) (void)hipDeviceGetAttribute(&ncu, hipDeviceAttributeMultiprocessorCount, dev);
    const HxsKnobs k = hxsLaunchKnobs();
    const HxsLaunchPlan pl = hxsPlanLaunch(p, src, od, C, ncu, k, hc && hc->dst, hc ? hc->n : 0);
    if (!pl.ok) return hipErrorNotSupported;
    if (k.trace) {
        char line[512];
        hxsTraceLines(pl, od, C, line, sizeof(line));
        fputs(line, stderr);
    }
    HxsArgs x = hxsArgsOf(pl, p, src, od, C, k);
    if (pl.histFolded) {
        x.hdst = static_cast<float*>(hc->dst);
        x.ht0 = hc->t0;
        x.hn = hc->n;
        hc->done = true;
    }
    const int64_t blocks = pl.nblocks;
    if (pl.kernel == HxsKernel::Hxt) {
        switch (p.NS) {
#define GAR_HXT_NS(n) case n: return hxtFmt<n>(x, pl.lds, blocks, stream, pl.lean);
#if !GAR_HXS_QUICK
            GAR_HXT_NS(1) GAR_HXT_NS(2) GAR_HXT_NS(3) GAR_HXT_NS(4) GAR_HXT_NS(5) GAR_HXT_NS(6) GAR_HXT_NS(7)
            GAR_HXT_NS(8)
#endif
            GAR_HXT_NS(9) GAR_HXT_NS(10)
#undef GAR_HXT_NS
            default: return hipErrorNotSupported;
        }
    }
    switch (p.NS) {
#define GAR_HXS_NS(n) case n: return hxsVst<n>(x, pl.lds, blocks, stream);
#if !GAR_HXS_QUICK
        GAR_HXS_NS(1) GAR_HXS_NS(2) GAR_HXS_NS(3) GAR_HXS_NS(4) GAR_HXS_NS(5) GAR_HXS_NS(6) GAR_HXS_NS(7)
        GAR_HXS_NS(8)
#endif
        GAR_HXS_NS(9) GAR_HXS_NS(10)
#undef GAR_HXS_NS
        default: return hipErrorNotSupported;
    }
}

}
```

### go-audio-resampler_amd/csrc/gar_hxs.hpp

```cpp
#pragma once
#include <climits>

#include "gar_hx.hpp"
#include "gar_hxs_geo.hpp"

namespace gar {

#ifndef GAR_HXS_D
#define GAR_HXS_D 2
#endif
constexpr int kHxsD = GAR_HXS_D;
constexpr int kHxsItems = (4 * kHxsNP + kHxsLoaders - 1) / kHxsLoaders;
#ifndef GAR_HXS_PRIO
#define GAR_HXS_PRIO 0
#endif
#ifndef GAR_HXS_PF2
#define GAR_HXS_PF2 0
#endif

struct HxsArgs {
    const h8v* A;
    const int* progs;
    int ea, Pc, Qc, Kc, Kread, G, C, nprog;
    int ncols, nblocks, Np, ngroups;
    int R, Rt, mirror;
    int Wg;
    unsigned long long* prof;
    int dbg;
    int small;
    int bigSmall;
    int vst, fmt;
    int xcdPair;
    int nt;
    int64_t a_lo, a_hi;
    int64_t o_lo, o_hi;
    const char* in;
    int64_t in_fs, in_cs, fastLo, fastHi;
    int in_esz, in_pcm;
    int out_pcm;
    float* hdst;
    int64_t ht0, hn;
    char* out;
    int64_t out_fs, out_cs;
    int out_f64;
    SrcDesc src;
    OutDesc od;
    const double* rows;
    const int* rowOff;
    const int* rowLen;
    int rowMax;
    int twoStage;
    const int* rowPh;
    const int* rowPar;
    const double* polyA;
    const double* dftC;
    int T1, T2;
    int ncomp;
    int role[12];
    int* err;
    int pollMax;
    int faultNeed;
    int coop;
    int qRbs, qGroups;
    int qU0[12], qRbw[12];
    int qOpt;
};
typedef const __attribute__((address_space(4))) HxsArgs* HxsArgsP;

__device__ __forceinline__ void hxsBarrier() {
    __atomic_signal_fence(__ATOMIC_SEQ_CST);
    __builtin_amdgcn_s_waitcnt(0xC07F);
    __builtin_amdgcn_s_barrier();
    __atomic_signal_fence(__ATOMIC_SEQ_CST);
}

__device__ __forceinline__ HxsArgsP hxsCold() {
    uint64_t v = reinterpret_cast<uint64_t>(__builtin_amdgcn_kernarg_segment_ptr());
    asm volatile("" : "+s"(v));
    return reinterpret_cast<HxsArgsP>(v);
}

__device__ __forceinline__ int hxsBlock(const HxsArgs& x, int i) {
    if (!x.xcdPair) return i;
    const int s = i >> 3, xc = i & 7;
    return ((s >> 1) * 8 + xc) * 2 + (s & 1);
}

__device__ __forceinline__ double hxsExact(HxsArgsP x, int64_t a, int r, int c) {
    const SrcDesc src = kload(&x->src);
    const int64_t t = a * x->Qc + x->rowOff[r];
    const int len = x->rowLen[r];
    const double* row = x->rows + static_cast<size_t>(r) * x->rowMax;
    double s = 0.0, z = 0.0;
    for (int k = 0; k < len; ++k) {
        const double v = static_cast<double>(srcRead<float>(src, t + k, c));
        s += row[k] * v;
        z += v * 0.0;
    }
    if (z == z || !x->twoStage) return s;
    const int ph = x->rowPh[r], par = x->rowPar[r], T1 = x->T1, T2 = x->T2;
    const double* pa = x->polyA + static_cast<size_t>(ph) * T2;
    double y = 0.0;
    for (int k2 = 0; k2 < T2; ++k2) {
        const int q = par + k2;
        const double* cq = x->dftC + static_cast<size_t>(q & 1) * T1;
        double u = 0.0;
        for (int k1 = 0; k1 < T1; ++k1) u += cq[k1] * static_cast<double>(srcRead<float>(src, t + (q >> 1) + k1, c));
        y += pa[k2] * u;
    }
    return y;
}

__device__ __forceinline__ void hxsFixup(HxsArgsP xp, int b, const int* loudLo, const int* loudHi) {
    const SrcDesc src = kload(&xp->src);
    const OutDesc od = kload(&xp->od);
    const int Pc = xp->Pc, Qc = xp->Qc, Np = xp->Np, C = xp->C, ncols = xp->ncols;
    const int64_t a_lo = xp->a_lo, a_hi = xp->a_hi;
    for (int j = 0; j < 16; ++j) {
        const int lo = loudLo[j], hi = loudHi[j];
        const int col = b * 16 + j;
        if (hi < 0 || col >= ncols) continue;
        const int k = col / C, c = col - k * C;
        const int p0 = max(0, (lo - xp->Kread) / Qc), p1 = min(Np - 1, hi / Qc);
        const int n = (p1 - p0 + 1) * Pc;
        for (int idx = threadIdx.x; idx < n; idx += blockDim.x) {
            const int p = p0 + idx / Pc, r = idx - (idx / Pc) * Pc;
            const int64_t a = a_lo + static_cast<int64_t>(k) * Np + p;
            if (a >= a_hi) continue;
            const int64_t o = a * Pc + r;
            if (o < od.o_lo || o >= od.o_hi) continue;
            const int w0 = p * Qc + xp->rowOff[r], w1 = w0 + xp->rowLen[r];
            if (w1 <= lo || w0 > hi) continue;
            const int64_t t0 = a * Qc + xp->rowOff[r];
            bool loud = false;
            for (int kk = 0; kk < w1 - w0 && !loud; ++kk) loud = hxLoud(srcRead<float>(src, t0 + kk, c));
            if (loud) outWrite<float>(od, o, c, static_cast<float>(hxsExact(xp, a, r, c)));
        }
    }
}

struct HxsStage {
    int T0, nrow;
    bool fast;
};

typedef unsigned u32x4v __attribute__((ext_vector_type(4)));
template <class XP>
__device__ __forceinline__ u32x4v hxsRsrc(XP x, int64_t row0, int64_t cofs, int elemBytes) {
    const uint64_t base = reinterpret_cast<uint64_t>(x->in + (row0 * x->in_fs + cofs) * x->in_esz);
    const int64_t nb = x->fastHi > row0 ? (x->fastHi - row0 - 1) * x->in_fs * x->in_esz + elemBytes : 0;
    const unsigned nrec = static_cast<unsigned>(nb < 0x7fffffff ? nb : 0x7fffffff);
    u32x4v r;
    r.x = __builtin_amdgcn_readfirstlane(static_cast<unsigned>(base));
    r.y = __builtin_amdgcn_readfirstlane(static_cast<unsigned>(base >> 32) & 0xffffu);
    r.z = __builtin_amdgcn_readfirstlane(nrec);
    r.w = 0x00020000u;
    return r;
}

template <class XP>
__device__ __forceinline__ __amdgpu_buffer_rsrc_t hxsRsrcT(XP x, int64_t row0, int64_t cofs, int elemBytes) {
    const u32x4v r = hxsRsrc(x, row0, cofs, elemBytes);
    const uint64_t base = static_cast<uint64_t>(r.x) | (static_cast<uint64_t>(r.y) << 32);
    return __builtin_amdgcn_make_buffer_rsrc(reinterpret_cast<void*>(base), 0, static_cast<int>(r.z), 0x00020000);
}

__device__ __forceinline__ float hxsGather(const SrcDesc& s, int64_t t, int c, const void* dummy) {
    const int64_t h = t - s.hist_base, i = t - s.in_base;
    const bool valid = t >= 0 && t < s.valid_end;
    const bool inH = valid && s.hist && h >= 0 && h < s.hist_len;
    const bool inI = valid && !inH && s.in && i >= 0 && i < s.in_len;
    const float* hp = static_cast<const float*>(s.hist) + (inH ? h * s.hist_ld + c : 0);
    if (s.in_pcm) {
        const int64_t e = inI ? i * s.in_fs + static_cast<int64_t>(c) * s.in_cs : 0;
        const float vh = *(inH ? hp : static_cast<const float*>(dummy));
        const float vi = inI ? static_cast<float>(pcmRead(s.in, e, s.in_pcm)) : 0.f;
        return inH ? vh : vi;
    }
    if (s.in_f64) {
        const double* ip = static_cast<const double*>(s.in) + (inI ? i * s.in_fs + static_cast<int64_t>(c) * s.in_cs : 0);
        const float vh = *(inH ? hp : static_cast<const float*>(dummy));
        const double vi = *(inI ? ip : static_cast<const double*>(dummy));
        return inH ? vh : (inI ? static_cast<float>(vi) : 0.f);
    }
    const float* ip = static_cast<const float*>(s.in) + (inI ? i * s.in_fs + static_cast<int64_t>(c) * s.in_cs : 0);
    const float v = *(inH ? hp : (inI ? ip : static_cast<const float*>(dummy)));
    return (inH || inI) ? v : 0.f;
}

template <class XP>
__device__ __forceinline__ int64_t hxsChunkRow(XP x, int k, int T0) {
    return (x->a_lo + static_cast<int64_t>(k) * x->Np) * x->Qc + T0;
}

template <class XP>
__device__ __forceinline__ HxsStage hxsStage(XP x, int b, int T0, int nrow) {
    HxsStage s;
    s.T0 = T0;
    s.nrow = nrow;
    const int c0 = b * 16, c1 = c0 + 15;
    const int64_t tlo = (x->a_lo + static_cast<int64_t>(c0 / x->C) * x->Np) * x->Qc + T0;
    s.fast = ((x->fmt >= 1 && x->fmt <= 4) || x->fmt == 6 || x->fmt == 7) && c1 < x->ncols && tlo >= x->fastLo && x->fastHi > x->fastLo;
    return s;
}
template <class XP>
__device__ __forceinline__ HxsStage hxsLoad(XP x, int b, int j, int P) {
    const int GQ = x->G * x->Qc;
    if (j < P) return hxsStage(x, b, j * GQ, min(GQ, x->Wg - j * GQ));
    return hxsStage(x, b, x->Wg + (j - P) * GQ, GQ);
}

template <class XP>
__device__ __forceinline__ void hxsPutItem(XP x, const HxsStage& st, int p0, int q, int row, f32x4 e,
                                           char* ring, uint32_t QS, int* loudLo, int* loudHi, int* flag) {
    const int t = st.T0 + row;
    int p = p0 + row;
    if (p >= x->R) p -= x->R;
    const bool l0 = hxLoud(e[0]), l1 = hxLoud(e[1]), l2 = hxLoud(e[2]), l3 = hxLoud(e[3]);
    if (__builtin_expect(l0 | l1 | l2 | l3, 0)) {
        if (l0) { atomicMin(loudLo + 4 * q, t); atomicMax(loudHi + 4 * q, t); e[0] = 0.f; }
        if (l1) { atomicMin(loudLo + 4 * q + 1, t); atomicMax(loudHi + 4 * q + 1, t); e[1] = 0.f; }
        if (l2) { atomicMin(loudLo + 4 * q + 2, t); atomicMax(loudHi + 4 * q + 2, t); e[2] = 0.f; }
        if (l3) { atomicMin(loudLo + 4 * q + 3, t); atomicMax(loudHi + 4 * q + 3, t); e[3] = 0.f; }
        *flag = 1;
    }
    uint2 hv, lv;
    hxSplit2(e[0], e[1], hv.x, lv.x);
    hxSplit2(e[2], e[3], hv.y, lv.y);
    char* qb = ring + q * QS;
    *reinterpret_cast<uint2*>(qb + 8 * p) = hv;
    *reinterpret_cast<uint2*>(qb + 8 * x->Rt + 8 * p) = lv;
    if (p < x->mirror) {
        p += x->R;
        *reinterpret_cast<uint2*>(qb + 8 * p) = hv;
        *reinterpret_cast<uint2*>(qb + 8 * x->Rt + 8 * p) = lv;
    }
}

template <class XP>
__device__ __forceinline__ void hxsSmallStage(XP x, int b, int tid, int nth, char* ring, uint32_t QS,
                                              int* loudLo, int* loudHi, int* flag) {
    const HxsArgsP xc = hxsCold();
    const SrcDesc src = kload(&xc->src);
    HxsStage st;
    st.T0 = 0;
    st.nrow = x->Wg;
    st.fast = false;
    constexpr int kB = 4;
    const int nit = 4 * x->Wg;
    for (int i0 = tid; i0 < nit; i0 += kB * nth) {
        f32x4 e[kB];
#pragma unroll
        for (int u = 0; u < kB; ++u) {
            const int i = i0 + u * nth;
            const int q = i & 3, row = i >> 2;
#pragma unroll
            for (int n = 0; n < 4; ++n) {
                const int col = b * 16 + 4 * q + n;
                const int k = col / x->C, c = col - k * x->C;
                e[u][n] = (i < nit && col < x->ncols) ? hxsGather(src, hxsChunkRow(x, k, row), c, x->A) : 0.f;
            }
        }
#pragma unroll
        for (int u = 0; u < kB; ++u) {
            const int i = i0 + u * nth;
            if (i < nit) hxsPutItem(x, st, 0, i & 3, i >> 2, e[u], ring, QS, loudLo, loudHi, flag);
        }
    }
}

template <int FMT>
struct HxsRegBuf {
    f2v a[kHxsItems], b[kHxsItems];
};
template <>
struct HxsRegBuf<2> {
    f32x4 v[kHxsItems];
};
template <>
struct HxsRegBuf<3> {
    uint32_t a[kHxsItems], b[kHxsItems];
};
template <>
struct HxsRegBuf<4> {
    uint2 a[kHxsItems], b[kHxsItems];
};
template <>
struct HxsRegBuf<6> {
    uint32_t a[kHxsItems], b[kHxsItems];
// ... 992 lines not shown
```

### go-audio-resampler_amd/csrc/gar_hxs_launch.cpp

```cpp
#include "gar_hxs_launch.hpp"

#include <algorithm>
#include <cstdio>
#include <cstdlib>

namespace gar {

namespace {
enum KnobKind { kInt, kIsSet, kIsOne };
struct KnobRow {
    const char* name;
    int HxsKnobs::*field;
    KnobKind kind;
    bool perLaunch;
};
constexpr KnobRow kHxsKnobTable[] = {
    {"GAR_HXS_G", &HxsKnobs::g, kInt, false},
    {"GAR_HXS_WGPERCU", &HxsKnobs::wgPerCu, kInt, false},
    {"GAR_HX_TRACE", &HxsKnobs::trace, kIsSet, false},
    {"GAR_HXS_DBG", &HxsKnobs::dbg, kInt, false},
    {"GAR_HXS_PROF", &HxsKnobs::prof, kIsSet, false},
    {"GAR_HXS_SMALL", &HxsKnobs::small, kInt, false},
    {"GAR_HXS_NP", &HxsKnobs::np, kInt, false},
    {"GAR_HXT", &HxsKnobs::hxt, kInt, false},
    {"GAR_HXS_SMALLK", &HxsKnobs::smallK, kInt, false},
    {"GAR_HXS_NT", &HxsKnobs::nt, kInt, false},
    {"GAR_HXS_PAIR", &HxsKnobs::pair, kInt, false},
    {"GAR_HXT_CHUNKMAJOR", &HxsKnobs::chunkMajor, kInt, false},
    {"GAR_HXT_COOP", &HxsKnobs::coop, kInt, false},
    {"GAR_HXQ", &HxsKnobs::hxq, kInt, false},
    {"GAR_HXQ_NR", &HxsKnobs::hxqNr, kInt, false},
    {"GAR_HXQ_OPT", &HxsKnobs::hxqOpt, kInt, false},
    {"GAR_HXT_ROLES", &HxsKnobs::roles, kInt, true},
    {"GAR_HXT_WIDE", &HxsKnobs::wide, kInt, true},
    {"GAR_HXT_LEAN", &HxsKnobs::lean, kInt, true},
    {"GAR_HXT_FAULT", &HxsKnobs::fault, kIsOne, true},
};

void readKnobs(HxsKnobs& k, bool perLaunchOnly) {
    for (const KnobRow& r : kHxsKnobTable) {
        if (perLaunchOnly && !r.perLaunch) continue;
        const char* e = std::getenv(r.name);
        if (r.kind == kIsSet) k.*r.field = e != nullptr;
        else if (r.kind == kIsOne) k.*r.field = e && e[0] == '1';
        else k.*r.field = e ? std::atoi(e) : HxsKnobs{}.*r.field;
    }
}
}

HxsKnobs hxsReadKnobs() {
    HxsKnobs k;
    readKnobs(k, false);
    return k;
}

HxsKnobs hxsLaunchKnobs() {
    static const HxsKnobs perProcess = hxsReadKnobs();
    HxsKnobs k = perProcess;
    readKnobs(k, true);
    return k;
}

namespace {

int sampleBytes(int pcm, int f64) { return pcm ? pcmBytes(pcm) : (f64 ? 8 : 4); }

struct HxtRoles {
    int ncomp = 0, maxStride = 1;
    int role[kHxtMaxComp] = {};
};
HxtRoles hxtRoles(int nprog, int NS, bool leanPlan, const HxsKnobs& k) {
    const bool balanced = k.roles >= 0 ? k.roles != 0 : (NS >= 10 || leanPlan);
    HxtRoles r;
    int w = 0;
    if (!balanced) {
        for (int i = 0; i < nprog; ++i) r.role[w++] = i | (1 << 16);
        r.ncomp = w;
        return r;
    }
    const int q = nprog / 4 * 4, rem = nprog - q;
    for (int i = 0; i < q; ++i) r.role[w++] = i | (1 << 16);
    if (rem == 2 && q + 4 <= kHxtMaxComp) {
        for (int i = 0; i < 4; ++i) r.role[w++] = (q + (i & 1)) | ((i >> 1) << 8) | (2 << 16);
        r.maxStride = 2;
    } else if (rem == 1 && q + 4 <= kHxtMaxComp) {
        for (int i = 0; i < 4; ++i) r.role[w++] = q | (i << 8) | (4 << 16);
        r.maxStride = 4;
    } else {
        for (int i = q; i < nprog; ++i) r.role[w++] = i | (1 << 16);
    }
    r.ncomp = w;
    return r;
}

bool isSmall(int64_t nmac, int C, int ncu, const HxsKnobs& k) {
    return k.small >= 0 ? k.small == 1 : nmac * C <= static_cast<int64_t>(16) * 2 * ncu;
}

bool wantsWideBlocks(const HxDev& p, const SrcDesc& src, const OutDesc& od, int C, bool small, const HxsKnobs& k) {
    const bool rows32 = !small && src.in && !src.in_pcm && !src.in_f64 && !od.pcm && !od.f64 && C % 32 == 0 && od.cs == 1 &&
                        (reinterpret_cast<uintptr_t>(src.in) & 15) == 0 && src.in_cs == 1 && src.in_fs % 4 == 0;
    if (!rows32 || k.wide == 0) return false;
    const HxtRoles roles = hxtRoles(p.nw, p.NS, false, k);
    const HxsRing r2 = hxsRingFor(p.Qc, p.Kread, 2);
    return roles.maxStride == 1 && hxtLdsWide(r2.Rt) <= kHxsLdsMax &&
           2 * p.Qc <= hxtMaxRowsF(kFmtRow32, hxtLoadersFor(roles.ncomp)) && r2.R / (2 * p.Qc) + 3 <= kHxtSlots;
}

struct HxsChunks {
    int64_t Np, nchunk, ncols;
    bool rawSpan;
};
HxsChunks chunkLaunch(const HxDev& p, const SrcDesc& src, int C, int ncu, int64_t nmac, bool small, int bw, int inEsz,
                      const HxsKnobs& k) {
    const int64_t Qc = p.Qc;
    const int64_t targetBlocks = static_cast<int64_t>(ncu) * (k.wgPerCu > 0 ? k.wgPerCu : 1);
    const int64_t nchunkT = small ? nmac : std::max<int64_t>(1, (targetBlocks * bw + C - 1) / C);
    const int64_t NpT = (k.np > 0 && !small) ? k.np : std::max<int64_t>(1, ceilDiv(nmac, nchunkT));
    const int64_t rowBytes = std::max<int64_t>(4, src.in_fs * inEsz);
    const int64_t chunksPerRsrc = (C <= 16 && 16 % C == 0) ? 16 / C : 1;
    const int64_t npMax = ((int64_t(1) << 31) / rowBytes / chunksPerRsrc - (3 * Qc + p.Kread + 256)) / Qc;
    HxsChunks c;
    c.rawSpan = npMax >= 1;
    c.Np = c.rawSpan ? std::min(NpT, npMax) : NpT;
    const int64_t nchunk = ceilDiv(nmac, c.Np);
    c.nchunk = (16 % C == 0 && !small) ? ceilDiv(nchunk * C, 16) * 16 / C : nchunk;
    c.ncols = c.nchunk * C;
    return c;
}

int loadLayout(const SrcDesc& src, int C) {
    if (!src.in) {
        const uintptr_t hA = reinterpret_cast<uintptr_t>(src.hist);
        if (C == 2 && src.hist_ld == 2 && (hA & 7) == 0) return kFmtStereo;
        if (C % 16 == 0 && src.hist_ld % 4 == 0 && (hA & 15) == 0) return kFmtRow16;
        return kFmtGather;
    }
    const uintptr_t inA = reinterpret_cast<uintptr_t>(src.in);
    const bool stereoIl = C == 2 && src.in_fs == 2 && src.in_cs == 1;
    const bool rows16 = C % 16 == 0 && src.in_cs == 1 && src.in_fs % 4 == 0;
    if (sampIsHalf(src.in_pcm)) {
        if ((inA & 3) == 0 && stereoIl) return kFmtStereoHalf;
        if ((inA & 7) == 0 && rows16) return kFmtRow16Half;
        return kFmtGather;
    }
    if (src.in_pcm == 16) return ((inA & 3) == 0 && stereoIl) ? kFmtStereoPcm16 : kFmtGather;
    if (src.in_pcm) return ((inA & 7) == 0 && stereoIl) ? kFmtStereoPcm32 : kFmtGather;
    if (src.in_f64) return kFmtGather;
    if ((inA & 7) == 0 && stereoIl) return kFmtStereo;
    if ((inA & 15) == 0 && rows16) return kFmtRow16;
    return kFmtGather;
}

int storeLayout(const OutDesc& od, int C, int Pc, uintptr_t outBase) {
    const bool al = (outBase & 15) == 0;
    const bool stereoIl = C == 2 && od.fs == 2 && od.cs == 1 && Pc % 4 == 0;
    if (od.pcm == 16 && al && stereoIl) return kVstStereoPcm16;
    if (sampIsHalf(od.pcm) && (outBase & 7) == 0 && stereoIl) return kVstStereoHalf;
    if (od.pcm) return kVstAny;
    if (od.f64) return kVstF64;
    if (al && stereoIl) return kVstStereo;
    if (al && od.fs == 1 && (od.cs * 4) % 16 == 0 && Pc % 4 == 0) return kVstRows;
    return kVstAny;
}

bool hxtApplies(const SrcDesc& src, const OutDesc& od, bool small, int fmt, int vst, const HxsKnobs& k) {
    return k.hxt != 0 && !small && !od.pcm && !od.f64 && !src.in_pcm &&
           ((fmt == kFmtStereo && vst == kVstStereo) || (fmt == kFmtRow16 && (vst == kVstAny || vst == kVstRows)));
}

bool isLeanPlan(const HxDev& p, const SrcDesc& src, bool hxt, int fmt, int vst, int inEsz, int64_t Np, const HxsKnobs& k) {
    using Geo = HxtLeanGeo<4>;
    return hxt && !kHxsDev && p.NS == kHxtLeanNS && p.Pc == kHxtLeanPc && p.Qc == Geo::Qc && p.Kread == Geo::Kread &&
           p.nw == kHxtLeanNw && fmt == kFmtStereo && vst == kVstStereo && src.in_fs == 2 && inEsz == 4 && Np >= Geo::G &&
           k.lean != 0;
}
template <int NL>
bool leanGeoIs(const HxDev& p, int G, const HxsRing& r) {
    using Geo = HxtLeanGeo<NL>;
    return p.Qc == Geo::Qc && G == Geo::G && r.R == Geo::R && r.Rt == Geo::Rt && r.Wg == Geo::Wg &&
           std::max(0, r.Wg - G * p.Qc) == Geo::mirror;
}

struct HxsGroup {
    int G = 0;
    HxsRing ring{0, 0, 0};
};
HxsGroup pickGroup(const HxDev& p, int fmt, bool hxt, const HxtRoles& roles, bool small, int64_t Np, const HxsKnobs& k) {
    for (int pass = hxt && roles.maxStride > 1 ? 0 : 1; pass < 2; ++pass) {
        for (int cand = small ? 1 : kHxsMaxG; cand >= 1; --cand) {
            const HxsRing r = hxsRingFor(p.Qc, p.Kread, cand);
            if (cand > 1 && cand > Np) continue;
            if (k.g > 0 && cand > k.g && cand > 1) continue;
            if (fmt == kFmtRow32 ? hxtLdsWide(r.Rt) > kHxsLdsMax : !hxsRingFits(p.Qc, cand, r.Rt)) continue;
            if (hxt && cand * p.Qc > hxtMaxRowsF(fmt, hxtLoadersFor(roles.ncomp))) continue;
            if (hxt && r.R / (cand * p.Qc) + 3 > kHxtSlots) continue;
            if (pass == 0 && cand % roles.maxStride != 0) continue;
            return {cand, r};
        }
    }
    return {};
}

struct HxsChoice {
    bool hxt = false;
    int fmt = kFmtGather;
    HxtRoles roles;
    HxsGroup grp;
};
HxsChoice chooseKernel(const HxDev& p, int fmt, bool hxt, bool wide, const HxtRoles& roles, bool small, int64_t Np,
                       const HxsKnobs& k) {
    if (wide) {
        const HxsGroup g = pickGroup(p, kFmtRow32, true, roles, small, Np, k);
        if (g.G >= 2 && roles.maxStride == 1) return {true, kFmtRow32, roles, g};
    }
    const HxsGroup g = pickGroup(p, fmt, hxt, roles, small, Np, k);
    if (g.G > 0 || !hxt) return {hxt, fmt, hxt ? roles : HxtRoles{}, g};
    return {false, fmt, HxtRoles{}, pickGroup(p, fmt, false, HxtRoles{}, small, Np, k)};
}

int xcdOrder(int fmt, int C, int nblocks, const HxsKnobs& k) {
    if (k.chunkMajor && fmt == kFmtRow32 && nblocks % 8 == 0) return 2;
    return k.pair && fmt == kFmtRow16 && (C / 16) % 2 == 0 && nblocks % 16 == 0 ? 1 : 0;
}

int hxqRowBlocks(const HxDev& p, const SrcDesc& src, int C, int ncu, const HxsLaunchPlan& pl, bool rawSpan, int64_t histN,
                 const HxsKnobs& k) {
    const int fmt = pl.fmt, inEsz = pl.in_esz;
    const uintptr_t hA = reinterpret_cast<uintptr_t>(src.hist);
    const int hAl = fmt == kFmtStereo ? 8 : (fmt == kFmtRow16 ? 16 : 4), hLd = fmt == kFmtStereo ? 2 : (fmt == kFmtRow16 ? 4 : 1);
    const bool histOk = !src.hist || src.hist_len <= 0 ||
                        ((hA % hAl) == 0 && src.hist_ld % hLd == 0 && src.hist_len * src.hist_ld * 4 < (int64_t(1) << 31));
    const int64_t spanRows = (16 / C + 2) * pl.Np * p.Qc + pl.Wg;
    const bool gen = fmt == kFmtGather && !src.in_pcm && src.in_fs >= 0 && src.in_cs >= 0 &&
                     (spanRows * src.in_fs + static_cast<int64_t>(C) * src.in_cs) * inEsz < (int64_t(1) << 31);
    const bool hkOk = histN <= 0 || (histN * src.in_fs + static_cast<int64_t>(C) * src.in_cs) * inEsz < (int64_t(1) << 31);
    const bool loadsOk = (fmt == kFmtStereo || fmt == kFmtRow16) ? rawSpan : gen;
    if (!(pl.small && k.hxq && loadsOk && histOk && hkOk && p.nw <= 12 && pl.Np == 1)) return 0;
    if (k.hxqNr > 0) return std::min(k.hxqNr, p.nw);
    for (int cand = p.nw; cand >= 1; --cand)
        if (pl.nblocks * static_cast<int64_t>(ceilDiv(p.nw, cand)) >= static_cast<int64_t>(ncu)) return cand;
    return 1;
}

}

bool hxsPlanFits(const HxDev& p) {
    if (!p.rb || p.nw > kHxRbMaxWaves || !hxsNsBuilt(p.NS)) return false;
    return hxsRingFits(p.Qc, 1, hxsRingFor(p.Qc, p.Kread, 1).Rt);
}

HxsLaunchPlan hxsPlanLaunch(const HxDev& p, const SrcDesc& src, const OutDesc& od, int C, int ncu, const HxsKnobs& k,
                            bool histKeep, int64_t histN) {
    HxsLaunchPlan pl;
    if (!p.rb || p.nw > kHxRbMaxWaves || !hxsNsBuilt(p.NS)) return pl;
    pl.a_lo = floorDiv(od.o_lo, p.Pc);
    pl.a_hi = ceilDiv(od.o_hi, p.Pc);
    const int64_t nmac = pl.a_hi - pl.a_lo;
    const bool small = isSmall(nmac, C, ncu, k);
    const bool wideWanted = wantsWideBlocks(p, src, od, C, small, k);
    pl.in_esz = sampleBytes(src.in_pcm, src.in_f64);
    pl.out_esz = sampleBytes(od.pcm, od.f64);
    const HxsChunks ch = chunkLaunch(p, src, C, ncu, nmac, small, wideWanted ? 32 : 16, pl.in_esz, k);
    if (ch.ncols > (int64_t(1) << 30) || ch.Np > (int64_t(1) << 24)) return pl;
    pl.inBase = reinterpret_cast<uintptr_t>(src.in) - static_cast<uintptr_t>(src.in_base * src.in_fs * pl.in_esz);
    pl.outBase = reinterpret_cast<uintptr_t>(od.out) - static_cast<uintptr_t>(od.o0 * od.fs * pl.out_esz);
    const int fmt = loadLayout(src, C);
    pl.vst = storeLayout(od, C, p.Pc, pl.outBase);
    const bool hxtWanted = hxtApplies(src, od, small, fmt, pl.vst, k);
    const bool leanPlan = isLeanPlan(p, src, hxtWanted, fmt, pl.vst, pl.in_esz, ch.Np, k);
    const HxtRoles roles = hxtWanted ? hxtRoles(p.nw, p.NS, leanPlan, k) : HxtRoles{};
    const bool wide = wideWanted && hxtWanted && fmt == kFmtRow16 && pl.vst == kVstAny;
    const HxsChoice c = chooseKernel(p, fmt, hxtWanted, wide, roles, small, ch.Np, k);
    if (c.grp.G == 0) return pl;

    pl.ok = true;
    pl.fmt = c.fmt;
    pl.small = small ? 1 : 0;
    pl.bigSmall = k.smallK ? 0 : 1;
    pl.Np = ch.Np; pl.nchunk = ch.nchunk; pl.ncols = ch.ncols;
    pl.nblocks = static_cast<int>(c.fmt == kFmtRow32 ? (ch.ncols + 31) / 32 : (ch.ncols + 15) / 16);
    pl.G = c.grp.G;
    pl.ngroups = static_cast<int>(ceilDiv(ch.Np, pl.G));
    pl.Wg = c.grp.ring.Wg;
    pl.groupR = c.grp.ring.R; pl.groupRt = c.grp.ring.Rt;
    const bool window = small && !pl.bigSmall;
    const int w16 = (pl.Wg + 15) / 16 * 16;
    pl.R = window ? w16 : pl.groupR;
    pl.Rt = window ? w16 : pl.groupRt;
    pl.mirror = window ? 0 : std::max(0, pl.Wg - pl.G * p.Qc);
    pl.ncomp = c.roles.ncomp; pl.maxStride = c.roles.maxStride;
    for (int w = 0; w < kHxtMaxComp; ++w) pl.role[w] = c.roles.role[w];
    pl.loaders = c.hxt ? hxtLoadersFor(pl.ncomp) : 0;
    pl.lean = leanPlan && c.hxt && (pl.loaders == 6 ? leanGeoIs<6>(p, pl.G, c.grp.ring) : leanGeoIs<4>(p, pl.G, c.grp.ring));
    pl.xcdPair = xcdOrder(pl.fmt, C, pl.nblocks, k);
    pl.qRbs = hxqRowBlocks(p, src, C, ncu, pl, ch.rawSpan, histN, k);
    pl.qGroups = pl.qRbs ? static_cast<int>(ceilDiv(p.nw, pl.qRbs)) : 0;
    pl.qOpt = pl.qRbs ? k.hxqOpt : 0;
    const bool rawOk = src.in && pl.fmt != kFmtGather && src.in_len > 0 && src.in_fs > 0 && src.in_cs >= 0 && ch.rawSpan;
    if (rawOk || (pl.qRbs && pl.fmt == kFmtGather && src.in)) {
        pl.fastLo = src.in_base;
        pl.fastHi = std::min(src.in_base + src.in_len, src.valid_end);
    }
    pl.kernel = c.hxt ? HxsKernel::Hxt : pl.qRbs ? HxsKernel::Hxq : window ? HxsKernel::HxsSmall : HxsKernel::Hxs;
    pl.lds = pl.fmt == kFmtRow32 ? hxtLdsWide(pl.Rt) : hxsLds(pl.Rt);
    pl.histFolded = histKeep && histN > 0;
    return pl;
}

int hxsTraceLines(const HxsLaunchPlan& pl, const OutDesc& od, int C, char* buf, size_t cap) {
    const bool raw = pl.fmt != kFmtGather;
    int n = std::snprintf(buf, cap, "%s: small=%d o[%lld,%lld) C=%d G=%d Np=%lld ngroups=%d nblocks=%d R=%d Rt=%d Wg=%d fmt=%d vst=%d fast[%lld,%lld) ncomp=%d lean=%d\n",
                          pl.kernel == HxsKernel::Hxt ? "hxt" : "hxs", pl.small, (long long)od.o_lo, (long long)od.o_hi, C, pl.G,
                          (long long)pl.Np, pl.ngroups, pl.nblocks, pl.groupR, pl.groupRt, pl.Wg, pl.fmt, pl.vst,
                          (long long)(raw ? pl.fastLo : 0), (long long)(raw ? pl.fastHi : 0), pl.ncomp, pl.lean ? 1 : 0);
    if (n < 0 || static_cast<size_t>(n) >= cap) return n;
    if (pl.qGroups > 0)
        n += std::snprintf(buf + n, cap - n, "hxq: qRbs=%d qGroups=%d workgroups=%lld\n", pl.qRbs, pl.qGroups,
                           (long long)pl.nblocks * pl.qGroups);
    return n;
}

}
```

### go-audio-resampler_amd/csrc/gar_hxs_launch.hpp

```cpp
#pragma once
#include <cstddef>
#include <cstdint>

#include "gar_hxs_geo.hpp"
#include "gar_kernels.hpp"

namespace gar {

struct HxsKnobs {
    int g = 0;
    int wgPerCu = 0;
    int trace = 0;
    int dbg = 0;
    int prof = 0;
    int small = -1;
    int np = 0;
    int hxt = -1;
    int smallK = 1;
    int nt = 0;
    int pair = 1;
    int chunkMajor = 1;
    int coop = 2;
    int hxq = 1;
    int hxqNr = 0;
    int hxqOpt = 1;
    int roles = -1;
    int wide = 1;
    int lean = 1;
    int fault = 0;
};
HxsKnobs hxsReadKnobs();
HxsKnobs hxsLaunchKnobs();

enum class HxsKernel { Hxs, HxsSmall, Hxq, Hxt };

struct HxsLaunchPlan {
    bool ok = false;
    HxsKernel kernel = HxsKernel::Hxs;
    int fmt = kFmtGather, vst = kVstAny;
    int small = 0, bigSmall = 0;
    int64_t Np = 0, nchunk = 0, ncols = 0;
    int nblocks = 0, ngroups = 0;
    int G = 0, R = 0, Rt = 0, mirror = 0, Wg = 0;
    int groupR = 0, groupRt = 0;
    int64_t a_lo = 0, a_hi = 0;
    int64_t fastLo = 0, fastHi = 0;
    int in_esz = 4, out_esz = 4;
    uintptr_t inBase = 0, outBase = 0;
    int xcdPair = 0;
    int ncomp = 0, role[kHxtMaxComp] = {}, maxStride = 1;
    bool lean = false;
    int loaders = 0;
    int qRbs = 0, qGroups = 0, qOpt = 0;
    size_t lds = 0;
    bool histFolded = false;
};

HxsLaunchPlan hxsPlanLaunch(const HxDev& p, const SrcDesc& src, const OutDesc& od, int C, int ncu, const HxsKnobs& k,
                            bool histKeep, int64_t histN);
int hxsTraceLines(const HxsLaunchPlan& pl, const OutDesc& od, int C, char* buf, size_t cap);

}
```

### go-audio-resampler_amd/csrc/gar_hxt.hpp

```cpp
#pragma once
#include "gar_hxs.hpp"

namespace gar {

__host__ __device__ constexpr int hxtMaxRows(int NL) { return 64 * hxtPieces(NL); }
template <int NL>
constexpr int hxtItems() { return (4 * hxtPieces(NL) + NL - 1) / NL; }
__host__ __device__ constexpr int hxtQuads(int FMT) { return FMT == 5 ? 8 : 4; }
__host__ __device__ constexpr int hxtCols(int FMT) { return 4 * hxtQuads(FMT); }
#ifndef GAR_HXT_CPRIO
#define GAR_HXT_CPRIO 0
#endif
#ifndef GAR_HXT_LPRIO
#define GAR_HXT_LPRIO 0
#endif
#ifndef GAR_HXT_CTDBG
#define GAR_HXT_CTDBG 0
#endif
constexpr uint32_t kHxtLoudBits = 0x417FF000u;
static_assert(__builtin_bit_cast(uint32_t, kHxLoud) == kHxtLoudBits, "hxt's loud test must match hxLoud");

struct HxtRole {
    int rb, ph, st;
};
// ... 449 lines not shown
    for (int k = 0; k < M::kItems; ++k) {
        const uint32_t o = v0 + 2u * M::q(k) * chunkB + 512u * M::pcS(k);
        r.a[k] = __builtin_bit_cast(f2v, __builtin_amdgcn_raw_buffer_load_b64(rs.r, static_cast<int>(o), 0, 0));
        r.b[k] = __builtin_bit_cast(f2v, __builtin_amdgcn_raw_buffer_load_b64(rs.r, static_cast<int>(o + chunkB), 0, 0));
    }
}

template <int NL, class Geo>
__device__ __forceinline__ uint32_t hxtConvertLean(const HxtBuf<1, NL>& r, int slot, uint32_t rb, int laneRow) {
    using M = HxtLeanMap<NL>;
    constexpr int K = M::kItems, GQ = Geo::GQ, R = Geo::R, kMaxLaneRow = 64 * M::kMaxPcL + 63, kSplitChunk = 4;
    const int p0 = (Geo::mirror + (slot + 1) * GQ) % R;
    uint32_t m = 0;
#pragma unroll
    for (int k0 = 0; k0 < K; k0 += kSplitChunk) {
        uint2 hv[kSplitChunk], lv[kSplitChunk];
#pragma unroll
        for (int u = 0; u < kSplitChunk; ++u) {
            if (k0 + u >= K) break;
            const f32x4 e = hxtItem<1, NL>(r, k0 + u);
            m = max(m, max(max(hxtMag(e[0]), hxtMag(e[1])), max(hxtMag(e[2]), hxtMag(e[3]))));
            hxSplit2(e[0], e[1], hv[u].x, lv[u].x);
            hxSplit2(e[2], e[3], hv[u].y, lv[u].y);
        }
#pragma unroll
        for (int u = 0; u < kSplitChunk; ++u) {
            if (k0 + u >= K) break;
            const int rowS = 64 * M::pcS(k0 + u);
            const int pu = p0 + rowS;
            const int wrapAt = R - pu;
            const uint32_t a = rb + static_cast<uint32_t>(M::q(k0 + u)) * Geo::QS + 8u * static_cast<uint32_t>(pu);
            if (rowS + kMaxLaneRow < GQ || laneRow < GQ - rowS) {
                hxtLdsPut(a, hv[u]);
                hxtLdsPut(a + Geo::dL, lv[u]);
                if (wrapAt <= kMaxLaneRow && laneRow >= wrapAt) {
                    hxtLdsPut(a - 8u * R, hv[u]);
                    hxtLdsPut(a - 8u * R + Geo::dL, lv[u]);
                }
            }
        }
    }
    return m;
}

template <class Geo>
__device__ __forceinline__ int hxtLeanFrom(const HxsArgs& x, int b, int kU) {
    const bool blockLive = b * 16 + 15 < x.ncols && x.fastHi > x.fastLo;
    if (!blockLive) return INT_MAX;
    const int64_t row0 = (x.a_lo + static_cast<int64_t>((b * 16) / x.C) * x.Np) * Geo::Qc;
    const int64_t lack = x.fastLo - (row0 + Geo::Wg);
    const int64_t i = lack <= 0 ? 0 : (lack + Geo::GQ - 1) / Geo::GQ;
    const int64_t iu = (i + kU - 1) / kU * kU;
    return iu > (1 << 28) ? INT_MAX : Geo::P + static_cast<int>(iu);
}

template <int NL, class Geo>
__device__ __forceinline__ void hxtLoadersLean(const HxsArgs& x, const HxsShared& sh, const HxtSync& sy, int b, int l,
                                               int lane, int coop, int jBegin, unsigned long long* waited) {
    using M = HxtLeanMap<NL>;
    static_assert(M::kItems == hxtItems<NL>() && 64 * (M::kMaxPcL + 1 + M::pcS(M::kItems - 1)) >= Geo::GQ, "lean items cover a load");
    static_assert(kHxtD == 2, "two register buffers");
    constexpr int GQ = Geo::GQ, P = Geo::P, kU = (Geo::nslot % 2 ? 2 : 1) * Geo::nslot;
    if constexpr (GAR_HXT_LPRIO > 0) __builtin_amdgcn_s_setprio(GAR_HXT_LPRIO);
    const HxsArgsP xp = hxsCold();
    const int nL = P + x.ngroups - 1;
    const int dbg = kHxsDev ? x.dbg : GAR_HXT_CTDBG;
    const HxsRegSrc rs = hxsRegSrc<1>(xp, b, lane);
    const uint32_t chunkB = static_cast<uint32_t>(rs.chunkB);
    const int laneRow = 64 * M::pcL(l) + lane;
    const uint32_t rb = static_cast<uint32_t>(reinterpret_cast<uintptr_t>((lds_s4p)(sh.ring))) +
                        static_cast<uint32_t>(M::qL(l)) * Geo::QS + 8u * static_cast<uint32_t>(laneRow);
    uint32_t vo = 8u * static_cast<uint32_t>(laneRow) + 2u * static_cast<uint32_t>(M::qL(l)) * chunkB +
                  8u * static_cast<uint32_t>(Geo::Wg + (jBegin - P) * GQ);
    int jI = jBegin;
    HxtBuf<1, NL> buf[kHxtD];
    auto issue = [&](HxtBuf<1, NL>& r) {
        const bool live = jI < nL && !(dbg & 1);
        hxtIssueLean<NL>(rs, live ? vo : 0x80000000u, chunkB, r);
        vo += 8u * GQ;
        ++jI;
    };
    if (coop == 2) {
        hxsBarrier();
        issue(buf[0]);
        hxsBarrier();
        issue(buf[1]);
    } else {
        issue(buf[0]);
        issue(buf[1]);
        if (coop) hxsBarrier();
    }
    for (int j0 = jBegin; j0 < nL; j0 += kU) {
#pragma unroll
        for (int u = 0; u < kU; ++u) {
            const int j = j0 + u;
            if (j < nL) {
                const int need = j - P - Geo::i0 + 1;
                if (need > 0 && !(dbg & 64)) hxtWait(x, sy, sy.cpArr, need - 1, x.ncomp, kHxtErrSlotWait, lane, waited);
                if (!(dbg & 16)) {
                    const uint32_t m = hxtConvertLean<NL, Geo>(buf[u % kHxtD], u % Geo::nslot, rb, laneRow);
                    if (__builtin_expect(__builtin_amdgcn_ballot_w64(m >= kHxtLoudBits) != 0, 0))
                        hxtLoudLoadLean<NL, Geo>(xp, Geo::Wg + (j - P) * GQ, b, l, lane, sh);
                }
                hxtArrive(sy.ldArr, j, lane);
            }
            issue(buf[u % kHxtD]);
        }
    }
}

__device__ __forceinline__ int hxtBlock(const HxsArgs& x, int i) {
    if (x.xcdPair == 2) return (i & 7) * (x.nblocks >> 3) + (i >> 3);
    return hxsBlock(x, i);
}

#ifndef GAR_HXT_NTST2
#define GAR_HXT_NTST2 1
#endif
__device__ __forceinline__ void hxtStoreStereoNt(char* p, const f32x4& y, int lane) {
    const bool even = (lane & 1) == 0;
    const float s0 = even ? y[2] : y[0], s1 = even ? y[3] : y[1];
    const float q0 = __int_as_float(__builtin_amdgcn_mov_dpp(__float_as_int(s0), 0xB1, 0xf, 0xf, false));
    const float q1 = __int_as_float(__builtin_amdgcn_mov_dpp(__float_as_int(s1), 0xB1, 0xf, 0xf, false));
    f32x4 w;
    if (even) { w[0] = y[0]; w[1] = q0; w[2] = y[1]; w[3] = q1; }
    else      { w[0] = q0; w[1] = y[2]; w[2] = q1; w[3] = y[3]; }
    __builtin_nontemporal_store(w, reinterpret_cast<f32x4*>(p));
}

template <int NS, int VST, bool FAST, int NT = 1>
__device__ __forceinline__ void hxtGroups(const HxsArgs& x, const HxsShared& sh_, const HxtSync& sy, int wt, int lane,
                                          const h8v (&Ah)[NS], const h8v (&Al)[NS], uint32_t laneOff, int u0, int P,
                                          int nslot, const HxtRole& ro, char* obase, int64_t pstride, int64_t aCol,
                                          int64_t oRow0, bool colOk, int ccol, bool fullRb, int nl, unsigned long long* st) {
    const int sh = -(x.ea + kHxXs);
    const int GQ = x.G * x.Qc;
    const uint32_t dL = 8u * static_cast<uint32_t>(x.Rt);
    const uint32_t pst = 8u * static_cast<uint32_t>(x.Qc) * static_cast<uint32_t>(ro.st);
    const int dbg = kHxsDev ? x.dbg : GAR_HXT_CTDBG;
    const uint32_t tileLds = 4u * sh_.QS;
    const int64_t tileOut = 16 * x.out_cs;
    auto epilogue = [&](const f32x4& oA, const f32x4& oL, int p, int h) {
        const f32x4 y = hxScale(oA, oL, sh);
        if (dbg & 2) return;
        if constexpr (FAST && VST == 2 && GAR_HXT_NTST2) {
            static_assert(NT == 1, "stereo frame-pair stores: one tile per period");
            hxtStoreStereoNt(obase + static_cast<int64_t>(p) * pstride, y, lane);
        } else if constexpr (FAST) {
            hxsStoreFast<VST>(x, obase + static_cast<int64_t>(p) * pstride + h * tileOut, y, lane);
        } else {
            const int ccol_ = ccol + 16 * h;
            const int64_t a = aCol + p;
            const int64_t o0 = a * x.Pc + oRow0;
            const bool live = colOk && a < x.a_hi;
            if (fullRb && live && a * x.Pc >= x.o_lo && (a + 1) * x.Pc <= x.o_hi) {
                char* pp = x.out + (o0 + ((VST == 2 && (lane & 1)) ? 2 : 0)) * x.out_fs + (VST == 2 ? 0 : ccol_ * x.out_cs);
                hxsStoreFast<VST>(x, pp, y, lane);
            } else if (live) {
#pragma unroll
                for (int i = 0; i < 4; ++i) {
                    const int64_t o = o0 + i;
                    if (oRow0 + i < x.Pc && o >= x.o_lo && o < x.o_hi)
                        *reinterpret_cast<float*>(x.out + o * x.out_fs + ccol_ * x.out_cs) = y[i];
                }
            }
        }
    };
    int first = ro.ph;
    for (int g = 0; g < x.ngroups; ++g) {
        const int p0 = g * x.G;
        const int pend = min(p0 + x.G, x.Np);
        while (first < p0) first += ro.st;
        const int n = first >= pend ? 0 : (pend - first + ro.st - 1) / ro.st;
        if (n > 0) {
            if (!(dbg & 32)) hxtWait(x, sy, sy.ldArr, P + g - 1 + x.faultNeed, nl, kHxtErrLoadWait, lane, st);
            if (kHxsDev && st) {
                const unsigned long long tg = __builtin_amdgcn_s_memtime();
                if (st[1] == 0) st[1] = tg;
                st[5] = tg;
            }
            int ln = lane;
            asm volatile("" : "+v"(ln));
            const uint32_t lo = ((ln & 15) & 3) * sh_.QS + 8u * (4 * (ln >> 4) + ((ln & 15) >> 2));
            uint32_t aH = static_cast<uint32_t>(reinterpret_cast<uintptr_t>((lds_s4p)(sh_.ring))) + lo + 8u * static_cast<uint32_t>(u0) +
                          8u * static_cast<uint32_t>((g % nslot) * GQ) + 8u * static_cast<uint32_t>(x.Qc) * static_cast<uint32_t>(first - p0);
            h8v bh0 = (dbg & 8) ? h8v{} : bFragA(aH), bl0 = (dbg & 8) ? h8v{} : bFragA(aH + dL);
            for (int i = 0; i < n; ++i) {
#pragma unroll
              for (int h = 0; h < NT; ++h) {
                asm volatile("" : "+v"(aH));
                const bool last = i + 1 == n && h + 1 == NT;
                uint32_t aL = aH + dL;
#if GAR_HXT_LOBASE
                asm volatile("" : "+v"(aL));
#endif
                const uint32_t aN = h + 1 < NT ? aH + tileLds : aH - (NT - 1) * tileLds + pst, aNL = aN + dL;
                f32x4 nA = {0, 0, 0, 0}, nL = nA;
#pragma unroll
                for (int s = 0; s < NS; ++s) {
                    const int ug = (s + 1) / NS, us = (s + 1) % NS;
                    h8v bhn = bh0, bln = bl0;
                    if (!(ug == 1 && last) && !(dbg & 8)) {
                        bhn = bFragA((ug == 0 ? aH : aN) + 256 * us);
                        bln = bFragA((ug == 0 ? aL : aNL) + 256 * us);
                    }
                    if (!(dbg & 4)) {
                        nA = mfma16(Ah[s], bh0, nA);
                        nA = mfma16(Al[s], bh0, nA);
                        nL = mfma16(Ah[s], bl0, nL);
                    }
                    bh0 = bhn;
                    bl0 = bln;
                    __builtin_amdgcn_sched_group_barrier(0x100, 4, 0);
                    __builtin_amdgcn_sched_group_barrier(0x008, 3, 0);
                    __builtin_amdgcn_sched_barrier(0);
                }
                epilogue(nA, nL, first + i * ro.st, h);
                aH = aN;
              }
            }
        }
        const unsigned long long ta = (kHxsDev && st) ? __builtin_amdgcn_s_memtime() : 0;
        if (kHxsDev && st && n > 0) st[3] += ta - st[5];
        hxtArrive(sy.cpArr, g, lane);
        if (kHxsDev && st) st[4] += __builtin_amdgcn_s_memtime() - ta;
    }
    if (kHxsDev && st) st[2] = __builtin_amdgcn_s_memtime();
}

template <int NS, int VST, int FMT>
__device__ __forceinline__ void hxtCompute(const HxsArgs& x, const HxsShared& sh_, const HxtSync& sy, int b, int wt,
                                           int lane, int nl, int coop, unsigned long long* st) {
    if constexpr (GAR_HXT_CPRIO > 0) __builtin_amdgcn_s_setprio(GAR_HXT_CPRIO);
    const HxtRole ro = hxtRole(x, wt);
    const int* pt = x.progs + kBgProgInts * ro.rb;
    const int u0 = uni(pt[4]), rbw = uni(pt[3]);
    h8v Ah[NS], Al[NS];
#pragma unroll
    for (int i = 0; i < NS; ++i) {
        Ah[i] = x.A[((static_cast<size_t>(ro.rb) * NS + i) * 2 + 0) * 64 + lane];
        Al[i] = x.A[((static_cast<size_t>(ro.rb) * NS + i) * 2 + 1) * 64 + lane];
    }
    if (kHxsDev && st) st[6] = __builtin_amdgcn_s_memtime();
    if (coop) {
        if (coop == 2) hxtCoopStage0<FMT, 4, true>(x, sh_, b, wt, x.ncomp, lane);
        else hxtCoopStage0<FMT, 4, false>(x, sh_, b, wt, x.ncomp, lane);
        hxsBarrier();
    }
    if (kHxsDev && st) st[7] = __builtin_amdgcn_s_memtime();
    const uint32_t QS = sh_.QS;
    const int GQ = x.G * x.Qc;
    const int grp = lane >> 4, l16 = lane & 15;
    const uint32_t laneOff = (l16 & 3) * QS + 8u * (4 * grp + (l16 >> 2));
    const bool fullRb = (rbw + 1) * 16 <= x.Pc;
    const int nslot = x.R / GQ;
    const int P = (x.Wg + GQ - 1) / GQ;
    const int64_t pstride = static_cast<int64_t>(x.Pc) * x.out_fs;
    const int col = b * hxtCols(FMT) + l16;
    const bool colOk = col < x.ncols;
    const int kcol = col / x.C, ccol = col - kcol * x.C;
    const int64_t aCol = x.a_lo + static_cast<int64_t>(kcol) * x.Np;
    const int64_t oRow0 = static_cast<int64_t>(rbw) * 16 + 4 * grp;
    const bool laneFast = fullRb && colOk && aCol + x.Np <= x.a_hi && aCol * x.Pc >= x.o_lo &&
                          (aCol + x.Np) * x.Pc <= x.o_hi;
    char* obase = x.out + (aCol * x.Pc + oRow0 + ((VST == 2 && (lane & 1)) ? 2 : 0)) * x.out_fs +
                  (VST == 2 ? 0 : ccol * x.out_cs);
    constexpr int NT = FMT == 5 ? 2 : 1;
    if (__builtin_amdgcn_ballot_w64(!laneFast) == 0)
        hxtGroups<NS, VST, true, NT>(x, sh_, sy, wt, lane, Ah, Al, laneOff, u0, P, nslot, ro, obase, pstride, aCol, oRow0,
                                     colOk, ccol, fullRb, nl, st);
    else
        hxtGroups<NS, VST, false, NT>(x, sh_, sy, wt, lane, Ah, Al, laneOff, u0, P, nslot, ro, obase, pstride, aCol, oRow0,
                                      colOk, ccol, fullRb, nl, st);
}

template <int NS, int FMT, int VST, int NL, int LEAN = 0>
__global__ __launch_bounds__(64 * kHxtWaves) void hxt_kernel(HxsArgs x) {
    extern __shared__ __attribute__((aligned(16))) unsigned char smem[];
    HxsShared s;
    s.stamp = nullptr;
    s.QS = 16u * static_cast<uint32_t>(x.Rt) + 64u;
    s.ring = reinterpret_cast<char*>(smem);
    constexpr int NQ = hxtQuads(FMT), NC = hxtCols(FMT);
    s.loudLo = reinterpret_cast<int*>(smem + NQ * static_cast<size_t>(s.QS));
    s.loudHi = s.loudLo + NC;
    s.flag = s.loudHi + NC;
    HxtSync sy;
    sy.ldArr = (lds_i32*)(smem + NQ * static_cast<size_t>(s.QS) + hxtSyncOff(FMT));
    sy.cpArr = sy.ldArr + kHxtSlots;
    sy.abort = sy.cpArr + kHxtSlots;
    const int lane = threadIdx.x & 63;
    const int wt = uni(threadIdx.x >> 6);
    const bool comp = wt < x.ncomp;
    if (threadIdx.x == 0) *sy.abort = 0;
    const bool stampW = kHxsDev && x.prof && lane == 0 && (wt == 0 || wt == x.ncomp);
    const unsigned long long tEntry = stampW ? __builtin_amdgcn_s_memtime() : 0;
    const unsigned long long rEntry = stampW ? __builtin_amdgcn_s_memrealtime() : 0;
    unsigned long long st[8] = {0, 0, 0, 0, 0, 0, 0, 0};
    unsigned long long tBlockEnd = 0;
    for (int bi = blockIdx.x; bi < x.nblocks; bi += gridDim.x) {
        const int b = hxtBlock(x, bi);
        __syncthreads();
        if (threadIdx.x < NC) {
            s.loudLo[threadIdx.x] = INT_MAX;
            s.loudHi[threadIdx.x] = -1;
        }
        const int GQb = x.G * x.Qc, Pb = (x.Wg + GQb - 1) / GQb;
        const int coop = hxtStage0Fast(x, b) ? x.coop : 0;
        if (threadIdx.x < 2 * kHxtSlots) sy.ldArr[threadIdx.x] = (coop && static_cast<int>(threadIdx.x) < Pb) ? NL : 0;
        if (threadIdx.x == 64) *s.flag = 0;
        __syncthreads();
        const bool first = bi == static_cast<int>(blockIdx.x);
        unsigned long long* stp = (stampW && first) ? st : nullptr;
        if (comp) hxtCompute<NS, VST, FMT>(x, s, sy, b, wt, lane, NL, coop, stp);
        else if constexpr (LEAN != 0) {
            static_assert(FMT == 1, "lean loaders: stereo f32 frames");
// ... 71 lines not shown
```

### go-audio-resampler_amd/csrc/gar_kernels.hpp

```cpp
#pragma once
#include <string>
#include <hip/hip_runtime.h>

#include <cstdint>
#include <vector>

namespace gar {

struct SrcDesc {
    const void* hist;
    int64_t hist_base, hist_len, hist_ld;
    const void* in;
    int64_t in_base, in_len, in_fs, in_cs;
    int in_f64;
    int in_pcm;
    int64_t valid_end;
};

struct OutDesc {
    void* out;
    int64_t o0, fs, cs;
    int f64;
    int pcm;
    int64_t o_lo, o_hi;
    int* err;
};

constexpr int kSampPcm24P = 280;
__host__ __device__ inline double pcmMax(int bits) {
    return bits == 16 ? 32767.0 : ((bits == 24 || bits == kSampPcm24P) ? 8388607.0 : 2147483647.0);
}
constexpr int kSampF16 = 4, kSampBF16 = 5;
__host__ __device__ inline bool sampIsHalf(int t) { return t == kSampF16 || t == kSampBF16; }
__host__ __device__ inline float halfToF32(uint16_t b, int code) {
    if (code == kSampBF16) return __builtin_bit_cast(float, static_cast<uint32_t>(b) << 16);
    return static_cast<float>(__builtin_bit_cast(_Float16, b));
}
__host__ __device__ inline uint16_t halfOfF32(float v, int code) {
    if (code == kSampBF16) {
        uint32_t u = __builtin_bit_cast(uint32_t, v);
        if ((u & 0x7fffffffu) > 0x7f800000u) return static_cast<uint16_t>((u >> 16) | 0x40u);
        u += 0x7fffu + ((u >> 16) & 1u);
        return static_cast<uint16_t>(u >> 16);
    }
    return __builtin_bit_cast(uint16_t, static_cast<_Float16>(v));
}
__host__ __device__ inline float f32OddOfF64(double d) {
    const float f = static_cast<float>(d);
    if (d != d || static_cast<double>(f) == d) return f;
    uint32_t u = __builtin_bit_cast(uint32_t, f);
    if (u & 1u) return f;
    const double af = f < 0 ? -static_cast<double>(f) : static_cast<double>(f), ad = d < 0 ? -d : d;
    u += af > ad ? ~0u : 1u;
    return __builtin_bit_cast(float, u);
}
__host__ __device__ inline uint16_t halfOfF64(double d, int code) { return halfOfF32(f32OddOfF64(d), code); }

__host__ __device__ inline int pcmBytes(int bits) { return bits == kSampPcm24P ? 3 : (bits <= 16 ? 2 : 4); }
__host__ __device__ inline double pcmToF64(int32_t i, int bits) { return static_cast<double>(i) * (1.0 / pcmMax(bits)); }
__host__ __device__ inline int32_t pcmOfF64(double y, int bits) {
    const double v = y > 1.0 ? 1.0 : (y < -1.0 ? -1.0 : y);
    const double s = v * pcmMax(bits);
    return s == s ? static_cast<int32_t>(s) : 0;
}
__host__ __device__ inline int32_t pcm24Load(const uint8_t* b) {
    const uint32_t u = static_cast<uint32_t>(b[0]) | (static_cast<uint32_t>(b[1]) << 8) | (static_cast<uint32_t>(b[2]) << 16);
    return static_cast<int32_t>(u << 8) >> 8;
}
__host__ __device__ inline void pcm24Store(uint8_t* b, int32_t i) {
    b[0] = static_cast<uint8_t>(i);
    b[1] = static_cast<uint8_t>(i >> 8);
    b[2] = static_cast<uint8_t>(i >> 16);
}
typedef uint32_t u32x3a __attribute__((ext_vector_type(3), aligned(4)));
__host__ __device__ inline void pcm24Pack4(const int32_t (&i)[4], uint32_t (&d)[3]) {
    const uint32_t a = static_cast<uint32_t>(i[0]) & 0xffffffu, b = static_cast<uint32_t>(i[1]) & 0xffffffu;
    const uint32_t c = static_cast<uint32_t>(i[2]) & 0xffffffu, e = static_cast<uint32_t>(i[3]) & 0xffffffu;
    d[0] = a | (b << 24);
    d[1] = (b >> 8) | (c << 16);
    d[2] = (c >> 16) | (e << 8);
}
__host__ __device__ inline void pcm24Unpack4(const uint32_t (&d)[3], int32_t (&i)[4]) {
    i[0] = static_cast<int32_t>(d[0] << 8) >> 8;
    i[1] = static_cast<int32_t>(((d[0] >> 24) | (d[1] << 8)) << 8) >> 8;
    i[2] = static_cast<int32_t>(((d[1] >> 16) | (d[2] << 16)) << 8) >> 8;
    i[3] = static_cast<int32_t>(d[2]) >> 8;
}
__host__ __device__ inline double pcmRead(const void* p, int64_t e, int bits) {
    if (sampIsHalf(bits)) return static_cast<double>(halfToF32(static_cast<const uint16_t*>(p)[e], bits));
    if (bits == kSampPcm24P) return pcmToF64(pcm24Load(static_cast<const uint8_t*>(p) + 3 * e), 24);
    return bits == 16 ? pcmToF64(static_cast<const int16_t*>(p)[e], 16) : pcmToF64(static_cast<const int32_t*>(p)[e], bits);
}
__host__ __device__ inline void pcmWrite(void* p, int64_t e, int bits, double y) {
    if (sampIsHalf(bits)) {
        static_cast<uint16_t*>(p)[e] = halfOfF64(y, bits);
        return;
    }
    if (bits == kSampPcm24P) {
        pcm24Store(static_cast<uint8_t*>(p) + 3 * e, pcmOfF64(y, 24));
        return;
    }
    const double v = y > 1.0 ? 1.0 : (y < -1.0 ? -1.0 : y);
    const double s = v * pcmMax(bits);
    if (bits == 16) static_cast<int16_t*>(p)[e] = static_cast<int16_t>(s == s ? static_cast<int32_t>(s) : 0);
    else static_cast<int32_t*>(p)[e] = s == s ? static_cast<int32_t>(s) : 0;
}

struct HxDev;

constexpr int kHxtErrLoadWait = 1, kHxtErrSlotWait = 2;

std::string& launchLimitMsg();
hipError_t ldsTooBig(const char* kernel, size_t need, size_t limit);

struct BgDev {
    int f64;
    int Pc, Qc, Kc, Kread, NS, nrb;
    int nprog, kch, nw, ncg, nred, nslots;
    const void* A;
    const int* progs;
    const int* reds;
    const HxDev* hx;
    int rbAligned;
    int maxPrb;
    const int* rbStart;
    const int* hRbStart;
    const int* hRbK0;
    const double* xRows;
    const int* xInfo;
    int xRowMax, xTwoStage, xT1, xT2;
    const double* xPolyA;
    const double* xDftC;
    int* nfList;
};
constexpr size_t kBgNfListBytes = 4 * (2 + 256 * 129 + 1);

struct HxDev {
    int Pc, Qc, Kc, Kread, NS, nrb;
    int nw, kch, nred, nslots, ea, rowMax;
    int rb;
    const void* A;
    const int* progs;
    const int* reds;
    const double* rows;
    const int* rowOff;
    const int* rowLen;
    int twoStage;
    int T1, T2;
    const int* rowPh;
    const int* rowPar;
    const double* polyA;
    const double* dftC;
    int* fix;
    int fixCap;
    int hxsOk;
    int hU0[16], hRbw[16];
};

struct PolyDev {
    int f64;
    int L, T;
    int64_t step, at0, u_base;
    int64_t m0;
    const void *a, *b, *c, *d;
    const void* abcd;
};

struct CubicSeg {
    double phase;
    int64_t o, i;
};
constexpr int64_t kCubicSegInputs = 256;
constexpr int kCubicSegInputsShort = 16;

struct HistCopy {
    void* dst = nullptr;
    int64_t t0 = 0, n = 0;
    bool done = false;
};

hipError_t launchBg(const BgDev& p, const SrcDesc& src, const OutDesc& out, int C, hipStream_t stream,
                    HistCopy* hc = nullptr);
hipError_t launchHx(const HxDev& p, const SrcDesc& src, const OutDesc& out, int C, hipStream_t stream,
                    HistCopy* hc = nullptr);
bool hxsPlanFits(const HxDev& p);
hipError_t launchHxs(const HxDev& p, const SrcDesc& src, const OutDesc& out, int C, hipStream_t stream,
                     HistCopy* hc = nullptr);
hipError_t launchPoly(const PolyDev& p, const SrcDesc& src, const OutDesc& out, int64_t nout, int C,
                      hipStream_t stream);
hipError_t launchCubic(int f64, const CubicSeg* segs, int64_t nseg, int64_t x_end, double step, const SrcDesc& src,
                       const OutDesc& od, int C, hipStream_t stream, int segLen = static_cast<int>(kCubicSegInputs));
hipError_t launchGather(int f64, const SrcDesc& src, void* dst, int64_t t0, int64_t n, int C, hipStream_t stream);
hipError_t launchCopy(const void* src, int src_f64, int64_t s_fs, int64_t s_cs, void* dst, int dst_f64,
                      int64_t d_fs, int64_t d_cs, int64_t n, int C, hipStream_t stream);
hipError_t launchConvert(const void* src, int s_type, int64_t s_fs, int64_t s_cs, void* dst, int d_type, int64_t d_fs,
                         int64_t d_cs, int64_t n, int C, hipStream_t stream);

}
```

### go-audio-resampler_amd/gar/__init__.py

```python
import ctypes as C
import os

import numpy as np

_HERE = os.path.dirname(os.path.abspath(__file__))
LIB_PATH = os.environ.get("GAR_LIB_PATH") or os.path.join(os.path.dirname(_HERE), "libgar.so")

QualityQuick, QualityLow, QualityMedium, QualityHigh, QualityVeryHigh, QualityCustom = range(6)
(EngineQuick, EngineLow, EngineMedium, EngineHigh, EngineVeryHigh,
 Engine16Bit, Engine20Bit, Engine24Bit, Engine28Bit, Engine32Bit) = range(10)
F64, F32, F32_EXACT = 0, 1, 2

GAR_OK, INVALID_CONFIG, BUFFER_TOO_SMALL, NOT_SUPPORTED, CHANNEL_MISMATCH, DEVICE, INTERNAL, INVALID_ARGUMENT = range(8)


class ResamplerError(Exception):
    code = -1


class ErrInvalidConfig(ResamplerError):
    code = INVALID_CONFIG


class ErrBufferTooSmall(ResamplerError):
    code = BUFFER_TOO_SMALL


class ErrNotSupported(ResamplerError):
    code = NOT_SUPPORTED


class ErrChannelMismatch(ResamplerError):
    code = CHANNEL_MISMATCH


class ErrDevice(ResamplerError):
    code = DEVICE


class ErrInternal(ResamplerError):
    code = INTERNAL


_ERRS = {c.code: c for c in (ErrInvalidConfig, ErrBufferTooSmall, ErrNotSupported, ErrChannelMismatch,
                             ErrDevice, ErrInternal)}


class QualitySpec(C.Structure):
    _fields_ = [("Preset", C.c_int32), ("Precision", C.c_int32), ("PhaseResponse", C.c_double),
                ("PassbandEnd", C.c_double), ("StopbandBegin", C.c_double), ("Flags", C.c_uint32)]


class _Config(C.Structure):
    _fields_ = [("InputRate", C.c_double), ("OutputRate", C.c_double), ("Channels", C.c_int32),
                ("Quality", QualitySpec), ("MaxInputSize", C.c_int64), ("EnableSIMD", C.c_int32),
                ("EnableParallel", C.c_int32), ("ComputeDtype", C.c_int32), ("Device", C.c_int32),
                ("DryRun", C.c_int32)]


class Info(C.Structure):
    _fields_ = [("Algorithm", C.c_char * 32), ("FilterLength", C.c_int32), ("Phases", C.c_int32),
                ("Latency", C.c_int32), ("MemoryUsage", C.c_int64), ("SIMDEnabled", C.c_int32),
                ("SIMDType", C.c_char * 48)]


class EngineGeometry(C.Structure):
    _fields_ = [("kind", C.c_int32), ("dft_factor", C.c_int32), ("dft_taps", C.c_int32),
                ("poly_phases", C.c_int32), ("poly_taps", C.c_int32), ("poly_step", C.c_int64),
                ("decim_factor", C.c_int32), ("decim_taps", C.c_int32), ("fused", C.c_int32),
                ("fir_period_out", C.c_int32), ("fir_period_in", C.c_int32), ("fir_taps_max", C.c_int32),
                ("useful_macs_per_output", C.c_double), ("mfma_macs_per_output", C.c_double)]


EXPORTED = [
    "gar_config_validate", "gar_preset_spec", "gar_new", "gar_new_batch", "gar_new_engine", "gar_new_engine_quality", "gar_new_engine_dry", "gar_free",
    "gar_estimate_output", "gar_output_size", "gar_flush_size", "gar_process_f64", "gar_process_f32",
    "gar_process_into_f64", "gar_process_into_f32", "gar_process_multi_f64", "gar_flush_f64", "gar_flush_f32",
    "gar_flush_multi_f64", "gar_process_device", "gar_flush_device", "gar_device_output_size",
    "gar_device_flush_size", "gar_reset", "gar_get_ratio", "gar_get_latency", "gar_get_info", "gar_channels",
    "gar_status_string", "gar_last_error", "gar_design_engine", "gar_design_composite", "gar_profile_enable",
    "gar_profile_read", "gar_stage_state", "gar_num_stages", "gar_stage_geometry", "gar_get_statistics",
    "gar_synchronize", "gar_profile_launch_stats", "gar_profile_kinds", "gar_dev_half_convert",
    "gar_dev_pcm24_convert", "gar_dev_hxs_plan",
]

_lib = None


def lib():
    global _lib
    if _lib is not None:
        return _lib
    if not os.path.exists(LIB_PATH):
        raise ImportError(f"libgar.so not built ({LIB_PATH}); run __graft_entry__.build()")
    try:
        import torch
    except ImportError:
        pass
    L = C.CDLL(LIB_PATH)
    vp, i32, i64, d, dp = C.c_void_p, C.c_int32, C.c_int64, C.c_double, C.POINTER(C.c_double)
    sig = {
        "gar_config_validate": (i32, [C.POINTER(_Config)]),
        "gar_preset_spec": (QualitySpec, [i32]),
        "gar_new": (i32, [C.POINTER(_Config), C.POINTER(vp)]),
        "gar_new_batch": (i32, [C.POINTER(_Config), i32, C.POINTER(vp)]),
        "gar_new_engine": (i32, [d, d, i32, i32, C.POINTER(vp)]),
        "gar_new_engine_quality": (i32, [d, d, i32, i32, C.POINTER(vp)]),
        "gar_new_engine_dry": (i32, [d, d, i32, i32, C.POINTER(vp)]),
        "gar_free": (None, [vp]),
        "gar_estimate_output": (i64, [vp, i64]),
        "gar_output_size": (i64, [vp, i32, i64]),
        "gar_flush_size": (i64, [vp, i32]),
        "gar_process_f64": (i32, [vp, vp, i64, vp, i64, C.POINTER(i64)]),
        "gar_process_f32": (i32, [vp, vp, i64, vp, i64, C.POINTER(i64)]),
        "gar_process_into_f64": (i32, [vp, vp, i64, vp, i64, C.POINTER(i64)]),
        "gar_process_into_f32": (i32, [vp, vp, i64, vp, i64, C.POINTER(i64)]),
        "gar_process_multi_f64": (i32, [vp, vp, i32, i64, vp, i64, vp]),
        "gar_flush_f64": (i32, [vp, vp, i64, C.POINTER(i64)]),
        "gar_flush_f32": (i32, [vp, vp, i64, C.POINTER(i64)]),
        "gar_flush_multi_f64": (i32, [vp, vp, i32, i64, vp]),
        "gar_process_device": (i32, [vp, vp, i32, i64, i64, i64, i32, vp, i32, i64, i64, i64, C.POINTER(i64), vp]),
        "gar_flush_device": (i32, [vp, i32, vp, i32, i64, i64, i64, C.POINTER(i64), vp]),
        "gar_device_output_size": (i64, [vp, i64]),
        "gar_device_flush_size": (i64, [vp]),
        "gar_reset": (None, [vp]),
        "gar_get_ratio": (d, [vp]),
        "gar_get_latency": (i32, [vp]),
        "gar_get_info": (i32, [vp, C.POINTER(Info)]),
        "gar_channels": (i32, [vp]),
        "gar_status_string": (C.c_char_p, [i32]),
        "gar_last_error": (C.c_char_p, []),
        "gar_design_engine": (i32, [d, d, i32, C.POINTER(EngineGeometry), vp, vp, vp, vp, vp, vp]),
        "gar_design_composite": (i32, [d, d, i32, vp, vp]),
        "gar_profile_enable": (None, [vp, i32]),
        "gar_profile_read": (i32, [vp, i32, C.POINTER(d), C.POINTER(i64)]),
        "gar_stage_state": (i32, [vp, i32, C.POINTER(i32), C.POINTER(i32)]),
        "gar_num_stages": (i32, [vp]),
        "gar_stage_geometry": (i32, [vp, i32, C.POINTER(d), C.POINTER(EngineGeometry)]),
        "gar_get_statistics": (i32, [vp, i32, C.POINTER(i64), C.POINTER(i64)]),
        "gar_synchronize": (i32, [vp]),
        "gar_profile_kinds": (None, [vp, C.c_uint32]),
        "gar_profile_launch_stats": (i32, [vp, i32, C.POINTER(d), C.POINTER(d), C.POINTER(d)]),
        "gar_dev_half_convert": (i32, [i32, vp, i64, vp, vp, vp]),
        "gar_dev_pcm24_convert": (i32, [vp, i64, vp, vp]),
        "gar_dev_hxs_plan": (i32, [vp, i32, i32, i64, i64, C.c_uint64, i64, i64, i64, C.c_uint64, i64, i64, i32, C.c_uint64,
                                   i64, i64, i64, i64, i64, i32, i32, i64, C.c_char_p, i64]),
    }
    ab = os.environ.get("GAR_LIB_PATH") is not None
    for name, (res, args) in sig.items():
        if ab and not hasattr(L, name):
            setattr(L, name, lambda *a, _r=res: None if _r is None else 0)
            continue
        f = getattr(L, name)
        f.restype = res
        f.argtypes = args
    _lib = L
    return L


def _check(rc):
    if rc != GAR_OK:
        msg = lib().gar_last_error().decode(errors="replace")
        raise _ERRS.get(rc, ResamplerError)(msg or lib().gar_status_string(rc).decode())


def _p(a):
    return C.c_void_p(a.ctypes.data) if a is not None and a.size else C.c_void_p(0)


def Config(InputRate, OutputRate, Channels=1, Quality=None, MaxInputSize=0, EnableSIMD=True,
           EnableParallel=False, ComputeDtype=F64, Device=0, DryRun=False):
    c = _Config()
    c.InputRate, c.OutputRate, c.Channels = float(InputRate), float(OutputRate), int(Channels)
    if Quality is None:
        Quality = QualitySpec(Preset=QualityHigh)
    elif isinstance(Quality, int):
        Quality = QualitySpec(Preset=Quality)
    c.Quality = Quality
    c.MaxInputSize, c.EnableSIMD, c.EnableParallel = int(MaxInputSize), int(EnableSIMD), int(EnableParallel)
    c.ComputeDtype, c.Device, c.DryRun = int(ComputeDtype), int(Device), int(bool(DryRun))
    return c


def GetPresetSpec(preset):
    return lib().gar_preset_spec(preset)


class Resampler:

    def __init__(self, handle, f32_io=False):
        self._h = C.c_void_p(handle)
        self._f32_io = f32_io
        self._free = lib().gar_free

    def __del__(self):
        h = getattr(self, "_h", None)
        free = getattr(self, "_free", None)
        if h is not None and h.value and free is not None:
            free(h)
            self._h = None

    def Process(self, x):
        x = np.ascontiguousarray(x, dtype=np.float64)
        n = lib().gar_output_size(self._h, 0, len(x))
        out = np.empty(max(n, 1))
        got = C.c_int64(0)
        _check(lib().gar_process_f64(self._h, _p(x), len(x), _p(out), len(out), C.byref(got)))
        return out[: got.value].copy()

    def ProcessFloat32(self, x):
        x = np.ascontiguousarray(x, dtype=np.float32)
        n = lib().gar_output_size(self._h, 0, len(x))
        out = np.empty(max(n, 1), dtype=np.float32)
        got = C.c_int64(0)
        _check(lib().gar_process_f32(self._h, _p(x), len(x), _p(out), len(out), C.byref(got)))
        return out[: got.value].copy()

    def ProcessInto(self, x, out):
        x = np.ascontiguousarray(x, dtype=np.float64)
        assert out.dtype == np.float64 and out.flags.c_contiguous
        got = C.c_int64(0)
        _check(lib().gar_process_into_f64(self._h, _p(x), len(x), _p(out), len(out), C.byref(got)))
        return got.value

    def ProcessFloat32Into(self, x, out):
        x = np.ascontiguousarray(x, dtype=np.float32)
        assert out.dtype == np.float32 and out.flags.c_contiguous
        got = C.c_int64(0)
        _check(lib().gar_process_into_f32(self._h, _p(x), len(x), _p(out), len(out), C.byref(got)))
        return got.value

    def EstimateOutput(self, n):
        return lib().gar_estimate_output(self._h, n)

    def OutputSize(self, n, channel=0):
        return lib().gar_output_size(self._h, channel, n)

    def FlushSize(self, channel=0):
        return lib().gar_flush_size(self._h, channel)

    def ProcessMulti(self, xs):
        nch = len(xs)
        n = len(xs[0]) if nch else 0
        arrs = [np.ascontiguousarray(x, dtype=np.float64) for x in xs]
        if any(len(a) != n for a in arrs):
            raise ValueError("ProcessMulti requires equal channel lengths")
        cap = max([lib().gar_output_size(self._h, c, n) for c in range(self.Channels)] + [1]) if nch == self.Channels else 1
        outs = [np.empty(cap) for _ in range(nch)]
        inp = (C.c_void_p * max(nch, 1))(*[_p(a) for a in arrs])
        outp = (C.c_void_p * max(nch, 1))(*[_p(o) for o in outs])
        counts = np.zeros(max(nch, 1), dtype=np.int64)
        _check(lib().gar_process_multi_f64(self._h, inp, nch, n, outp, cap, _p(counts)))
        return [o[: counts[c]].copy() for c, o in enumerate(outs)]

    def Flush(self):
        n = lib().gar_flush_size(self._h, 0)
        out = np.empty(max(n, 1), dtype=np.float32 if self._f32_io else np.float64)
        got = C.c_int64(0)
        fn = lib().gar_flush_f32 if self._f32_io else lib().gar_flush_f64
        _check(fn(self._h, _p(out), len(out), C.byref(got)))
        return out[: got.value].copy()

    def FlushMulti(self):
        nch = self.Channels
        cap = max([lib().gar_flush_size(self._h, c) for c in range(nch)] + [1])
        outs = [np.empty(cap) for _ in range(nch)]
        outp = (C.c_void_p * nch)(*[_p(o) for o in outs])
        counts = np.zeros(nch, dtype=np.int64)
        _check(lib().gar_flush_multi_f64(self._h, outp, nch, cap, _p(counts)))
        return [o[: counts[c]].copy() for c, o in enumerate(outs)]

    def Reset(self):
        lib().gar_reset(self._h)

    def GetRatio(self):
        return lib().gar_get_ratio(self._h)

    def GetLatency(self):
        return lib().gar_get_latency(self._h)

    def GetStatistics(self, channel=0):
        a, b = C.c_int64(0), C.c_int64(0)
        _check(lib().gar_get_statistics(self._h, channel, C.byref(a), C.byref(b)))
        return {"samplesIn": a.value, "samplesOut": b.value}

    def GetInfo(self):
        info = Info()
        _check(lib().gar_get_info(self._h, C.byref(info)))
        return info

    def profile(self, on=True, kinds=None):
        lib().gar_profile_enable(self._h, int(on))
        lib().gar_profile_kinds(self._h, 0x3F if kinds is None else sum(1 << k for k in kinds))

    def profile_read(self, kind=0):
        ms, n = C.c_double(0), C.c_int64(0)
        _check(lib().gar_profile_read(self._h, kind, C.byref(ms), C.byref(n)))
        return ms.value, n.value

# ... 2 lines not shown
        _check(lib().gar_profile_launch_stats(self._h, kind, C.byref(a), C.byref(b), C.byref(c)))
        return a.value, b.value, c.value

    def synchronize(self):
        _check(lib().gar_synchronize(self._h))

    def num_stages(self):
        return lib().gar_num_stages(self._h)

    def stage_geometry(self, stage):
        ratio, g = C.c_double(0), EngineGeometry()
        _check(lib().gar_stage_geometry(self._h, stage, C.byref(ratio), C.byref(g)))
        return ratio.value, g

    def stage_state(self, stage):
        a, b = C.c_int32(0), C.c_int32(0)
        _check(lib().gar_stage_state(self._h, stage, C.byref(a), C.byref(b)))
        return bool(a.value), bool(b.value)

    @property
    def Channels(self):
        return lib().gar_channels(self._h)

    def process_device(self, x, out=None, stream=None, pcm_bits=None):
        import torch
        _check_form(x)
        if out is not None:
            _check_form(out)
        assert x.is_cuda
        if x.shape[1] != self.Channels or (out is not None and out.shape[1] != self.Channels):
            raise ErrChannelMismatch(f"expected {self.Channels} channels, got {x.shape[1]}"
                                     + ("" if out is None else f" (out {out.shape[1]})"))
        frames = x.shape[0]
        n = lib().gar_device_output_size(self._h, frames)
        if n < 0:
            raise ErrNotSupported("channels not in lockstep")
        if out is None:
            out = torch.empty((max(n, 1),) + tuple(x.shape[1:]), dtype=x.dtype, device=x.device)
        got = C.c_int64(0)
        dt = _io_type(x.dtype, pcm_bits)
        odt = _io_type(out.dtype, pcm_bits)
        (xfs, xcs), (ofs, ocs) = _sample_strides(x), _sample_strides(out)
        st = C.c_void_p(stream if stream is not None else torch.cuda.current_stream(x.device).cuda_stream)
        _check(lib().gar_process_device(self._h, C.c_void_p(x.data_ptr()), dt, xfs, xcs, frames,
                                        x.shape[1], C.c_void_p(out.data_ptr()), odt, ofs, ocs,
                                        out.shape[0], C.byref(got), st))
        return out[: got.value]

    def flush_device(self, out=None, dtype=None, stream=None, pcm_bits=None):
        import torch
        if out is not None:
            _check_form(out)
        if out is not None and out.shape[1] != self.Channels:
            raise ErrChannelMismatch(f"expected {self.Channels} channels, got {out.shape[1]}")
        n = lib().gar_device_flush_size(self._h)
        if n < 0:
            raise ErrNotSupported("channels not in lockstep")
        if out is None:
            shape = (max(n, 1), self.Channels) + ((3,) if dtype == torch.uint8 else ())
            out = torch.empty(shape, dtype=dtype or torch.float32, device="cuda")
        got = C.c_int64(0)
        odt = _io_type(out.dtype, pcm_bits)
        ofs, ocs = _sample_strides(out)
        st = C.c_void_p(stream if stream is not None else torch.cuda.current_stream(out.device).cuda_stream)
        _check(lib().gar_flush_device(self._h, out.shape[1], C.c_void_p(out.data_ptr()), odt, ofs,
                                      ocs, out.shape[0], C.byref(got), st))
        return out[: got.value]


PCM16, PCM24, PCM32 = 16, 24, 32
F16, BF16 = 4, 5
PCM24_PACKED = 280


def _io_type(dtype, pcm_bits=None):
    import torch
    if dtype == torch.uint8:
        return PCM24_PACKED
    if dtype == torch.float64:
        return F64
    if dtype == torch.float32:
        return F32
    if dtype == torch.float16:
        return F16
    if dtype == torch.bfloat16:
        return BF16
    if dtype == torch.int16:
        return PCM16
    if dtype == torch.int32:
        bits = pcm_bits or PCM32
        if bits not in (PCM24, PCM32):
            raise ValueError("int32 PCM holds 24- or 32-bit samples")
        return bits
    raise TypeError(f"unsupported sample dtype {dtype}")


def _check_form(t):
    import torch
    if t.dtype == torch.uint8:
        if t.dim() != 3 or t.shape[2] != 3:
            raise ValueError(f"packed 24-bit PCM is a uint8 tensor [frames, channels, 3], got shape {tuple(t.shape)}")
        if t.stride(2) != 1 or t.stride(0) % 3 or t.stride(1) % 3:
            raise ValueError(f"packed 24-bit PCM needs strides (3 a, 3 b, 1), got {tuple(t.stride())}")
    elif t.dim() != 2:
        raise ValueError(f"sample tensors are [frames, channels], got shape {tuple(t.shape)}")


def _sample_strides(t):
    if t.dim() == 3:
        return t.stride(0) // 3, t.stride(1) // 3
    return t.stride(0), t.stride(1)


def pack_pcm24(i):
    a = np.ascontiguousarray(i.cpu().numpy() if hasattr(i, "cpu") else i).astype(np.int32)
    u = a.astype(np.uint32)
    return np.stack([(u & 0xFF), ((u >> 8) & 0xFF), ((u >> 16) & 0xFF)], axis=-1).astype(np.uint8)


def unpack_pcm24(b):
    a = np.asarray(b.cpu().numpy() if hasattr(b, "cpu") else b, dtype=np.uint8)
    if a.ndim < 1 or a.shape[-1] != 3:
        raise ValueError(f"packed 24-bit samples have a last dimension of 3, got shape {a.shape}")
    u = a[..., 0].astype(np.uint32) | (a[..., 1].astype(np.uint32) << 8) | (a[..., 2].astype(np.uint32) << 16)
    return ((u << 8).astype(np.int32) >> 8).astype(np.int32)


def pcm24_convert(x):
    x = np.ascontiguousarray(x, dtype=np.float64)
    b = np.zeros((x.size, 3), dtype=np.uint8)
    i = np.zeros(x.size, dtype=np.int32)
    _check(lib().gar_dev_pcm24_convert(_p(x), x.size, _p(b), _p(i)))
    return b, i


def half_convert(x, half_type):
    x = np.ascontiguousarray(x, dtype=np.float64)
    a, b = np.zeros(x.size, dtype=np.uint16), np.zeros(x.size, dtype=np.uint16)
    w = np.zeros(x.size, dtype=np.float32)
    _check(lib().gar_dev_half_convert(int(half_type), _p(x), x.size, _p(a), _p(b), _p(w)))
    return a, b, w


def hxs_plan(r, in_type, in_fs, in_cs, in_addr, in_base, in_len, valid_end, hist_addr, hist_len, hist_ld,
             out_type, out_addr, o0, out_fs, out_cs, o_lo, o_hi, channels, cu_count, hist_keep=0, stage=0):
    buf = C.create_string_buffer(1024)
    _check(lib().gar_dev_hxs_plan(r._h, int(stage), int(in_type), int(in_fs), int(in_cs), int(in_addr), int(in_base),
                                  int(in_len), int(valid_end), int(hist_addr), int(hist_len), int(hist_ld), int(out_type),
                                  int(out_addr), int(o0), int(out_fs), int(out_cs), int(o_lo), int(o_hi), int(channels),
                                  int(cu_count), int(hist_keep), buf, len(buf)))
    return buf.value.decode()


def New(config):
    if config is None:
        raise ErrInvalidConfig("config is nil")
    h = C.c_void_p(0)
    _check(lib().gar_new(C.byref(config), C.byref(h)))
    return Resampler(h.value)


def NewBatch(config, n_streams):
    h = C.c_void_p(0)
    _check(lib().gar_new_batch(C.byref(config), int(n_streams), C.byref(h)))
    return Resampler(h.value)


def NewEngine(inputRate, outputRate, quality):
    h = C.c_void_p(0)
    _check(lib().gar_new_engine(float(inputRate), float(outputRate), quality, F64, C.byref(h)))
    return Resampler(h.value)


def NewEngineFloat32(inputRate, outputRate, quality):
    h = C.c_void_p(0)
    _check(lib().gar_new_engine(float(inputRate), float(outputRate), quality, F32, C.byref(h)))
    return Resampler(h.value, f32_io=True)


def EngineNewResampler(inputRate, outputRate, quality, dtype=F64):
    h = C.c_void_p(0)
    _check(lib().gar_new_engine_quality(float(inputRate), float(outputRate), int(quality), int(dtype), C.byref(h)))
    return Resampler(h.value, f32_io=dtype != F64)


def NewEngineDry(inputRate, outputRate, quality, dtype=F64):
    h = C.c_void_p(0)
    _check(lib().gar_new_engine_dry(float(inputRate), float(outputRate), quality, dtype, C.byref(h)))
    return Resampler(h.value, f32_io=dtype == F32)


def ResampleMono(x, inputRate, outputRate, quality):
    r = NewEngine(inputRate, outputRate, quality)
    return np.concatenate([r.Process(x), r.Flush()])


def ResampleMonoFloat32(x, inputRate, outputRate, quality):
    r = NewEngineFloat32(inputRate, outputRate, quality)
    return np.concatenate([r.ProcessFloat32(x), r.Flush()])


def ResampleStereo(left, right, inputRate, outputRate, quality):
    r = NewEngine(inputRate, outputRate, quality)
    lo = np.concatenate([r.Process(left), r.Flush()])
    r.Reset()
    ro = np.concatenate([r.Process(right), r.Flush()])
    return lo, ro


def design_engine(in_rate, out_rate, engine_quality):
    g = EngineGeometry()
    _check(lib().gar_design_engine(in_rate, out_rate, engine_quality, C.byref(g), None, None, None, None, None, None))
    dft = np.zeros(max(g.dft_factor * g.dft_taps, 1))
    n = g.poly_phases * g.poly_taps
    pa, pb, pc, pd = (np.zeros(max(n, 1)) for _ in range(4))
    dec = np.zeros(max(g.decim_taps, 1))
    _check(lib().gar_design_engine(in_rate, out_rate, engine_quality, C.byref(g), _p(dft), _p(pa), _p(pb), _p(pc),
                                   _p(pd), _p(dec)))
    return g, {"dft": dft[: g.dft_factor * g.dft_taps], "a": pa[:n], "b": pb[:n], "c": pc[:n], "d": pd[:n],
               "decim": dec[: g.decim_taps]}


def design_composite(in_rate, out_rate, engine_quality):
    g, _ = design_engine(in_rate, out_rate, engine_quality)
    if not g.fused:
        raise ErrNotSupported("engine has no fused composite FIR")
    rows = np.zeros((g.fir_period_out, g.fir_taps_max))
    offs = np.zeros(g.fir_period_out, dtype=np.int64)
    _check(lib().gar_design_composite(in_rate, out_rate, engine_quality, _p(rows), _p(offs)))
    return rows, offs, g
```

### include/gar.h

```cpp
#ifndef GAR_H
#define GAR_H

#include <stdint.h>

#ifdef __cplusplus
extern "C" {
#endif

typedef struct gar_resampler gar_resampler;

typedef enum gar_status {
    GAR_OK = 0,
    GAR_ERR_INVALID_CONFIG = 1,
    GAR_ERR_BUFFER_TOO_SMALL = 2,
    GAR_ERR_NOT_SUPPORTED = 3,
    GAR_ERR_CHANNEL_MISMATCH = 4,
    GAR_ERR_DEVICE = 5,
    GAR_ERR_INTERNAL = 6,
    GAR_ERR_INVALID_ARGUMENT = 7
} gar_status;

enum { GAR_QUALITY_QUICK = 0, GAR_QUALITY_LOW = 1, GAR_QUALITY_MEDIUM = 2, GAR_QUALITY_HIGH = 3,
       GAR_QUALITY_VERYHIGH = 4, GAR_QUALITY_CUSTOM = 5 };
enum { GAR_FLAG_NO_INTERPOLATION = 1, GAR_FLAG_MINIMUM_PHASE = 2, GAR_FLAG_LINEAR_PHASE = 4,
       GAR_FLAG_ALLOW_ALIASING = 8, GAR_FLAG_NO_SIMD = 16 };
enum { GAR_F64 = 0, GAR_F32 = 1, GAR_F32_EXACT = 2 };
enum { GAR_PCM16 = 16, GAR_PCM24 = 24, GAR_PCM32 = 32 };
enum { GAR_F16 = 4, GAR_BF16 = 5 };
enum { GAR_PCM24_PACKED = 0x100 | 24 };
enum { GAR_ENGINE_QUICK = 0, GAR_ENGINE_LOW, GAR_ENGINE_MEDIUM, GAR_ENGINE_HIGH, GAR_ENGINE_VERYHIGH,
       GAR_ENGINE_16BIT, GAR_ENGINE_20BIT, GAR_ENGINE_24BIT, GAR_ENGINE_28BIT, GAR_ENGINE_32BIT };

typedef struct gar_quality_spec {
    int32_t preset;
    int32_t precision;
    double phase_response;
    double passband_end;
    double stopband_begin;
    uint32_t flags;
} gar_quality_spec;

typedef struct gar_config {
    double input_rate;
    double output_rate;
    int32_t channels;
    gar_quality_spec quality;
    int64_t max_input_size;
    int32_t enable_simd;
    int32_t enable_parallel;
    int32_t compute_dtype;
    int32_t device;
    int32_t dry_run;
} gar_config;

typedef struct gar_info {
    char algorithm[32];
    int32_t filter_length;
    int32_t phases;
    int32_t latency;
    int64_t memory_usage;
    int32_t simd_enabled;
    char simd_type[48];
} gar_info;

gar_status gar_config_validate(const gar_config *cfg);
gar_quality_spec gar_preset_spec(int32_t preset);
gar_status gar_new(gar_config *cfg, gar_resampler **out);
gar_status gar_new_batch(gar_config *cfg, int32_t n_streams, gar_resampler **out);
gar_status gar_new_engine(double input_rate, double output_rate, int32_t preset, int32_t dtype,
                          gar_resampler **out);
void gar_free(gar_resampler *r);
gar_status gar_new_engine_quality(double input_rate, double output_rate, int32_t engine_quality, int32_t dtype,
                                  gar_resampler **out);
gar_status gar_new_engine_dry(double input_rate, double output_rate, int32_t preset, int32_t dtype,
                              gar_resampler **out);

int64_t gar_estimate_output(const gar_resampler *r, int64_t input_len);
int64_t gar_output_size(const gar_resampler *r, int32_t channel, int64_t input_len);
int64_t gar_flush_size(const gar_resampler *r, int32_t channel);

gar_status gar_process_f64(gar_resampler *r, const double *in, int64_t n, double *out, int64_t cap, int64_t *n_out);
gar_status gar_process_f32(gar_resampler *r, const float *in, int64_t n, float *out, int64_t cap, int64_t *n_out);
gar_status gar_process_into_f64(gar_resampler *r, const double *in, int64_t n, double *out, int64_t cap,
                                int64_t *n_out);
gar_status gar_process_into_f32(gar_resampler *r, const float *in, int64_t n, float *out, int64_t cap,
                                int64_t *n_out);
gar_status gar_process_multi_f64(gar_resampler *r, const double *const *in, int32_t n_channels, int64_t n,
                                 double *const *out, int64_t cap, int64_t *n_out);
gar_status gar_flush_f64(gar_resampler *r, double *out, int64_t cap, int64_t *n_out);
gar_status gar_flush_f32(gar_resampler *r, float *out, int64_t cap, int64_t *n_out);
gar_status gar_flush_multi_f64(gar_resampler *r, double *const *out, int32_t n_channels, int64_t cap,
                               int64_t *n_out);

gar_status gar_process_device(gar_resampler *r, const void *in, int32_t in_dtype, int64_t in_frame_stride,
                              int64_t in_channel_stride, int64_t frames, int32_t channels, void *out,
                              int32_t out_dtype, int64_t out_frame_stride, int64_t out_channel_stride,
                              int64_t out_cap_frames, int64_t *out_frames, void *stream);
gar_status gar_flush_device(gar_resampler *r, int32_t channels, void *out, int32_t out_dtype,
                            int64_t out_frame_stride, int64_t out_channel_stride, int64_t out_cap_frames,
                            int64_t *out_frames, void *stream);
int64_t gar_device_output_size(const gar_resampler *r, int64_t frames);
int64_t gar_device_flush_size(const gar_resampler *r);
gar_status gar_synchronize(gar_resampler *r);

void gar_reset(gar_resampler *r);
double gar_get_ratio(const gar_resampler *r);
int32_t gar_get_latency(const gar_resampler *r);
gar_status gar_get_info(const gar_resampler *r, gar_info *info);
int32_t gar_channels(const gar_resampler *r);
gar_status gar_get_statistics(const gar_resampler *r, int32_t ch, int64_t *samples_in, int64_t *samples_out);
const char *gar_status_string(gar_status s);
const char *gar_last_error(void);
void gar_profile_enable(gar_resampler *r, int32_t on);
void gar_profile_kinds(gar_resampler *r, uint32_t kinds);
gar_status gar_profile_read(gar_resampler *r, int32_t kind, double *ms, int64_t *launches);
gar_status gar_profile_launch_stats(gar_resampler *r, int32_t kind, double *min_ms, double *median_ms,
                                    double *max_ms);
gar_status gar_stage_state(const gar_resampler *r, int32_t stage, int32_t *fused_plan, int32_t *fused_now);

int64_t gar_dev_pool_selftest(int32_t threads, int32_t iters, int32_t channels, int64_t frames);

gar_status gar_dev_half_convert(int32_t half_type, const double *in, int64_t n, uint16_t *from_f64,
                                uint16_t *from_f32, float *widened);

gar_status gar_dev_pcm24_convert(const double *in, int64_t n, uint8_t *packed, int32_t *unpacked);

gar_status gar_dev_hxs_plan(const gar_resampler *r, int32_t stage, int32_t in_type, int64_t in_fs, int64_t in_cs,
                            uint64_t in_addr, int64_t in_base, int64_t in_len, int64_t valid_end, uint64_t hist_addr,
                            int64_t hist_len, int64_t hist_ld, int32_t out_type, uint64_t out_addr, int64_t o0,
                            int64_t out_fs, int64_t out_cs, int64_t o_lo, int64_t o_hi, int32_t channels,
                            int32_t cu_count, int64_t hist_keep, char *buf, int64_t cap);

typedef struct gar_engine_geometry {
    int32_t kind;
    int32_t dft_factor, dft_taps;
    int32_t poly_phases, poly_taps;
    int64_t poly_step;
    int32_t decim_factor, decim_taps;
    int32_t fused;
    int32_t fir_period_out, fir_period_in, fir_taps_max;
    double useful_macs_per_output;
    double mfma_macs_per_output;
} gar_engine_geometry;
gar_status gar_design_engine(double input_rate, double output_rate, int32_t engine_quality,
                             gar_engine_geometry *geom, double *dft, double *poly_a, double *poly_b,
                             double *poly_c, double *poly_d, double *decim);
gar_status gar_design_composite(double input_rate, double output_rate, int32_t engine_quality, double *rows,
                                int64_t *offsets);

int32_t gar_num_stages(const gar_resampler *r);
gar_status gar_stage_geometry(const gar_resampler *r, int32_t stage, double *stage_ratio, gar_engine_geometry *geom);

#ifdef __cplusplus
}
#endif
#endif
```

Baseline: 448,200.

## Fold flush tail outputs into main HXT launch and cache device CU count

During the main fused DFT+poly launch, the HXT kernel now also computes the flush-tail outputs that would be produced at flush time, when they fall within the last column chunk. It stores them in a side device buffer. At flush, if the counters still match, a cheap copy or convert replaces a second full filter launch. The CU count is also queried once at init and passed through OutDesc, avoiding a per-launch device attribute query. This adds state-validity tracking and extra work in the main kernel, which is wasted if more input arrives before flush.

Result: no change. 456,600 (median of 3 runs) (+1.9%).

```diff
diff --git a/go-audio-resampler_amd/csrc/gar_engine.cpp b/go-audio-resampler_amd/csrc/gar_engine.cpp
--- a/go-audio-resampler_amd/csrc/gar_engine.cpp
+++ b/go-audio-resampler_amd/csrc/gar_engine.cpp
@@ -309,6 +309,19 @@
     return nout;
 }
 
+int64_t cntFusedFlush(Counters& t, const DftBank& dft, const PolyBank& poly, bool& quirk) {
+    int64_t nA = 0, nB = 0;
+    if (t.dft_hist > 0) nA = cntPoly(t, poly, cntDft(t, dft, dft.taps), quirk);
+    if (t.poly_hist > 0) nB = cntPoly(t, poly, poly.taps, quirk);
+    return nA + nB;
+}
+
+bool sameCounters(const Counters& a, const Counters& b) {
+    return a.staged == b.staged && a.x_count == b.x_count && a.dft_hist == b.dft_hist && a.poly_hist == b.poly_hist &&
+           a.at == b.at && a.u_base == b.u_base && a.u_count == b.u_count && a.dec_hist == b.dec_hist &&
+           a.dec_phase == b.dec_phase && a.y_count == b.y_count && a.cub_phase == b.cub_phase;
+}
+
 int64_t cntDecim(Counters& s, const DecimBank& b, int64_t n) {
     if (b.factor == 1) return n;
     if (n == 0) return 0;
@@ -515,6 +528,11 @@
     PinBuf cubPin[2];
     int cubCur = 0;
     std::vector<CubicSeg> cubSegs;
+    DevBuf tail;
+    bool tailValid = false;
+    int tailStage = 0;
+    int64_t tailY0 = 0, tailN = 0;
+    Counters tailCnt;
 };
 
 }
@@ -540,6 +558,7 @@
     bool failEvValid = false;
     int* errHost = nullptr;
     int* errDev = nullptr;
+    int ncu = 0;
     gar_config cfg{};
     std::vector<std::unique_ptr<gar::StageRT>> stages;
     std::vector<gar::Group> groups;
@@ -616,10 +635,12 @@
 }
 
 thread_local int* g_curErr = nullptr;
+thread_local int g_curNcu = 0;
 
 OutDesc mkOut(const OutView& o, int64_t o0, int64_t n) {
     OutDesc d{};
     d.err = g_curErr;
+    d.ncu = g_curNcu;
     d.out = o.p;
     d.o0 = o0;
     d.fs = o.fs;
@@ -695,6 +716,7 @@
     const EngineDesign& d = rt.d;
     const int64_t n = in.n;
     if (n == 0) return 0;
+    if (x.g->tailStage == si) x.g->tailValid = false;
     switch (d.kind) {
         case EngineKind::Cubic: {
             const int64_t x0 = c.x_count;
@@ -759,9 +781,35 @@
                     if (x.launch && nout > 0) HIPCHK(timedBg(x, 0, rt.fusedD, xsrc, mkOut(out, y0, nout), C));
                     materialize(x, rt, c, dv, xsrc);
                 } else {
+                    int64_t tailN = 0;
+                    bool folded = false;
+                    if (x.launch && nout > 0 && si == 0 && !rt.f64 && rt.fusedD.hx &&
+                        hxsTailFoldPossible(*rt.fusedD.hx, y0, y0 + nout, C, x.h->ncu)) {
+                        Counters t = c;
+                        bool tq = false;
+                        tailN = cntFusedFlush(t, d.dft, d.poly, tq);
+                        if (tq) tailN = 0;
+                        if (tailN > 0) x.g->tail.ensure(static_cast<size_t>(tailN) * C * sizeof(float));
+                    }
                     withHist(x, dv.xh, xsrc, c.u_base / 2, c.x_count, nout > 0, [&](HistCopy* hc) {
-                        return timedBg(x, 0, rt.fusedD, xsrc, mkOut(out, y0, nout), C, hc);
+                        if (tailN > 0) {
+                            hc->tail = x.g->tail.p;
+                            hc->tailY0 = y0 + nout;
+                            hc->tailN = tailN;
+                        }
+                        const hipError_t e = timedBg(x, 0, rt.fusedD, xsrc, mkOut(out, y0, nout), C, hc);
+                        folded = hc->tailDone;
+                        return e;
                     });
+                    if (folded) {
+                        Group& g = *x.g;
+                        g.tailValid = true;
+                        g.tailStage = si;
+                        g.tailY0 = y0 + nout;
+                        g.tailN = tailN;
+                        g.tailCnt = c;
+                        g.tailCnt.y_count = y0 + nout;
+                    }
                 }
             } else {
                 const int64_t p0 = before.x_count - before.dft_hist;
@@ -817,12 +865,20 @@
                 const SrcDesc xsrc = mkSrc(dv.xh, C, c.x_count, none);
                 Counters t = c;
                 bool quirk = false;
-                int64_t nA = 0, nB = 0;
-                if (t.dft_hist > 0) nA = cntPoly(t, d.poly, cntDft(t, d.dft, d.dft.taps), quirk);
-                if (t.poly_hist > 0) nB = cntPoly(t, d.poly, d.poly.taps, quirk);
+                const int64_t n = cntFusedFlush(t, d.dft, d.poly, quirk);
                 if (!quirk) {
-                    const int64_t y0 = c.y_count, n = nA + nB;
-                    if (x.launch && n > 0) HIPCHK(timedBg(x, 3, rt.fusedD, xsrc, mkOut(out, y0, n), C));
+                    const int64_t y0 = c.y_count;
+                    Group& g = *x.g;
+                    const bool folded = g.tailValid && g.tailStage == si && g.tailY0 == y0 && g.tailN == n && sameCounters(g.tailCnt, c);
+                    if (x.launch && n > 0 && folded) {
+                        HIPCHK(timed(x, 3, [&] {
+                            if (out.pcm) return launchConvert(g.tail.p, 0, C, 1, out.p, out.pcm, out.fs, out.cs, n, C, x.s);
+                            return launchCopy(g.tail.p, 0, C, 1, out.p, out.f64, out.fs, out.cs, n, C, x.s);
+                        }));
+                    } else if (x.launch && n > 0) {
+                        HIPCHK(timedBg(x, 3, rt.fusedD, xsrc, mkOut(out, y0, n), C));
+                    }
+                    g.tailValid = false;
                     c = t;
                     c.y_count = y0 + n;
                     c.staged = true;
@@ -1106,9 +1162,10 @@
     DeviceGuard dg(h->device);
     struct ErrScope {
         int* prev;
-        explicit ErrScope(int* e) : prev(g_curErr) { g_curErr = e; }
-        ~ErrScope() { g_curErr = prev; }
-    } es(h->errDev);
+        int prevNcu;
+        ErrScope(int* e, int ncu) : prev(g_curErr), prevNcu(g_curNcu) { g_curErr = e; g_curNcu = ncu; }
+        ~ErrScope() { g_curErr = prev; g_curNcu = prevNcu; }
+    } es(h->errDev, h->ncu);
     gar_status st = wrap([&]() -> gar_status {
         if (h->orderValid && h->lastStream != s) {
             HIPCHK(hipStreamWaitEvent(s, h->orderEv, 0));
@@ -1134,6 +1191,7 @@
     });
     if (st == GAR_ERR_DEVICE || (st == GAR_ERR_INVALID_ARGUMENT && g_launchLimit)) {
         h->poisoned = true;
+        for (auto& g : h->groups) g.tailValid = false;
         h->failEvValid = h->failEv && hipEventRecord(h->failEv, s) == hipSuccess;
     } else if (st == GAR_OK && hostSynced && devFault(h)) {
         st = GAR_ERR_DEVICE;
@@ -1204,6 +1262,7 @@
     void* d = nullptr;
     HIPCHK(hipHostGetDevicePointer(&d, w, 0));
     h->errDev = static_cast<int*>(d);
+    HIPCHK(hipDeviceGetAttribute(&h->ncu, hipDeviceAttributeMultiprocessorCount, h->device));
     return GAR_OK;
 }
 
@@ -1851,6 +1910,7 @@
                 d.xh.clear();
                 d.uh.clear();
             }
+            g.tailValid = false;
             g.statIn = g.statOut = 0;
             return;
         }
@@ -1965,12 +2025,12 @@
     return GAR_OK;
 }
 
-gar_status gar_dev_hxs_plan(const gar_resampler* r, int32_t stage, int32_t in_type, int64_t in_fs, int64_t in_cs,
-                            uint64_t in_addr, int64_t in_base, int64_t in_len, int64_t valid_end, uint64_t hist_addr,
-                            int64_t hist_len, int64_t hist_ld, int32_t out_type, uint64_t out_addr, int64_t o0,
-                            int64_t out_fs, int64_t out_cs, int64_t o_lo, int64_t o_hi, int32_t channels,
-                            int32_t cu_count, int64_t hist_keep, char* buf, int64_t cap) {
-    if (!r || !buf || cap < 1 || stage < 0 || stage >= static_cast<int32_t>(r->stages.size()) || channels < 1 ||
+static gar_status planFor(const gar_resampler* r, int32_t stage, int32_t in_type, int64_t in_fs, int64_t in_cs,
+                          uint64_t in_addr, int64_t in_base, int64_t in_len, int64_t valid_end, uint64_t hist_addr,
+                          int64_t hist_len, int64_t hist_ld, int32_t out_type, uint64_t out_addr, int64_t o0, int64_t out_fs,
+                          int64_t out_cs, int64_t o_lo, int64_t o_hi, int32_t channels, int32_t cu_count, int64_t hist_keep,
+                          int64_t tail_y0, int64_t tail_n, gar::HxsLaunchPlan& pl, OutDesc& od) {
+    if (!r || stage < 0 || stage >= static_cast<int32_t>(r->stages.size()) || channels < 1 ||
         cu_count < 1 || !ioTypeOk(in_type) || !ioTypeOk(out_type))
         return guard(GAR_ERR_INVALID_ARGUMENT, "bad launch-plan arguments");
     const gar::StageRT& st = *r->stages[stage];
@@ -1985,17 +2045,62 @@
     src.in_f64 = in_type == GAR_F64;
     src.in_pcm = isNarrow(in_type) ? in_type : 0;
     src.valid_end = valid_end;
-    OutDesc od{};
+    od = OutDesc{};
     od.out = reinterpret_cast<void*>(static_cast<uintptr_t>(out_addr));
     od.o0 = o0; od.fs = out_fs; od.cs = out_cs;
     od.f64 = out_type == GAR_F64;
     od.pcm = isNarrow(out_type) ? out_type : 0;
     od.o_lo = o_lo; od.o_hi = o_hi;
+    if (o_hi <= o_lo) return GAR_OK;
+    pl = gar::hxsPlanLaunch(*hx, src, od, channels, cu_count, gar::hxsReadKnobs(), hist_keep > 0, hist_keep, tail_y0, tail_n);
+    return GAR_OK;
+}
+
+gar_status gar_dev_hxs_plan(const gar_resampler* r, int32_t stage, int32_t in_type, int64_t in_fs, int64_t in_cs,
+                            uint64_t in_addr, int64_t in_base, int64_t in_len, int64_t valid_end, uint64_t hist_addr,
+                            int64_t hist_len, int64_t hist_ld, int32_t out_type, uint64_t out_addr, int64_t o0,
+                            int64_t out_fs, int64_t out_cs, int64_t o_lo, int64_t o_hi, int32_t channels,
+                            int32_t cu_count, int64_t hist_keep, char* buf, int64_t cap) {
+    if (!buf || cap < 1) return guard(GAR_ERR_INVALID_ARGUMENT, "bad launch-plan arguments");
     buf[0] = 0;
-    if (o_hi <= o_lo) return GAR_OK;
-    const gar::HxsLaunchPlan pl = gar::hxsPlanLaunch(*hx, src, od, channels, cu_count, gar::hxsReadKnobs(), hist_keep > 0, hist_keep);
+    gar::HxsLaunchPlan pl;
+    OutDesc od{};
+    const gar_status s = planFor(r, stage, in_type, in_fs, in_cs, in_addr, in_base, in_len, valid_end, hist_addr, hist_len,
+                                 hist_ld, out_type, out_addr, o0, out_fs, out_cs, o_lo, o_hi, channels, cu_count, hist_keep,
+                                 0, 0, pl, od);
+    if (s != GAR_OK || o_hi <= o_lo) return s;
     if (!pl.ok) std::snprintf(buf, static_cast<size_t>(cap), "not supported\n");
     else gar::hxsTraceLines(pl, od, channels, buf, static_cast<size_t>(cap));
+    return GAR_OK;
+}
+
+gar_status gar_dev_hxs_fold(const gar_resampler* r, int32_t stage, int32_t in_type, int64_t in_fs, int64_t in_cs,
+                            uint64_t in_addr, int64_t in_base, int64_t in_len, int64_t valid_end, uint64_t hist_addr,
+                            int64_t hist_len, int64_t hist_ld, int32_t out_type, uint64_t out_addr, int64_t o0,
+                            int64_t out_fs, int64_t out_cs, int64_t o_lo, int64_t o_hi, int32_t channels,
+                            int32_t cu_count, int64_t hist_keep, int64_t tail_y0, int64_t tail_n, int64_t* folded) {
+    if (!folded || tail_n < 0) return guard(GAR_ERR_INVALID_ARGUMENT, "bad launch-plan arguments");
+    *folded = 0;
+    gar::HxsLaunchPlan pl;
+    OutDesc od{};
+    const gar_status s = planFor(r, stage, in_type, in_fs, in_cs, in_addr, in_base, in_len, valid_end, hist_addr, hist_len,
+                                 hist_ld, out_type, out_addr, o0, out_fs, out_cs, o_lo, o_hi, channels, cu_count, hist_keep,
+                                 tail_y0, tail_n, pl, od);
+    if (s == GAR_OK && o_hi > o_lo && pl.ok) *folded = pl.tailN;
+    return s;
+}
+
+gar_status gar_dev_flush_tail(const gar_resampler* r, int32_t stage, int64_t* tail_n, int32_t* quirk) {
+    if (!r || !tail_n || !quirk || stage < 0 || stage >= static_cast<int32_t>(r->stages.size()) || r->groups.empty())
+        return guard(GAR_ERR_INVALID_ARGUMENT, "bad flush-tail arguments");
+    *tail_n = 0;
+    *quirk = 0;
+    const gar::EngineDesign& d = r->stages[stage]->d;
+    gar::Counters t = r->groups[0].cnt[stage];
+    if (d.kind != gar::EngineKind::DftPoly || t.staged) return GAR_OK;
+    bool q = false;
+    *tail_n = gar::cntFusedFlush(t, d.dft, d.poly, q);
+    *quirk = q ? 1 : 0;
     return GAR_OK;
 }
 
diff --git a/go-audio-resampler_amd/csrc/gar_hxs.hip b/go-audio-resampler_amd/csrc/gar_hxs.hip
--- a/go-audio-resampler_amd/csrc/gar_hxs.hip
+++ b/go-audio-resampler_amd/csrc/gar_hxs.hip
@@ -129,6 +129,8 @@
     x.dbg = k.dbg;
     x.prof = profBuf(k.prof != 0);
     x.o_lo = od.o_lo; x.o_hi = od.o_hi;
+    x.tailHi = od.o_hi + pl.tailN;
+    x.a_hiT = ceilDiv(x.tailHi, p.Pc);
     x.in_esz = pl.in_esz;
     x.in_pcm = src.in_pcm;
     x.in = reinterpret_cast<const char*>(pl.inBase);
@@ -179,10 +181,12 @@
 
 hipError_t launchHxs(const HxDev& p, const SrcDesc& src, const OutDesc& od, int C, hipStream_t stream, HistCopy* hc) {
     if (od.o_hi <= od.o_lo) return hipSuccess;
-    int dev = 0, ncu = 256;
-    if (hipGetDevice(&dev) == hipSuccess) (void)hipDeviceGetAttribute(&ncu, hipDeviceAttributeMultiprocessorCount, dev);
+    int dev = 0, ncu = od.ncu > 0 ? od.ncu : 256;
+    if (od.ncu <= 0 && hipGetDevice(&dev) == hipSuccess) (void)hipDeviceGetAttribute(&ncu, hipDeviceAttributeMultiprocessorCount, dev);
     const HxsKnobs k = hxsLaunchKnobs();
-    const HxsLaunchPlan pl = hxsPlanLaunch(p, src, od, C, ncu, k, hc && hc->dst, hc ? hc->n : 0);
+    const bool tailAsked = hc && hc->tail && hc->tailN > 0;
+    const HxsLaunchPlan pl = hxsPlanLaunch(p, src, od, C, ncu, k, hc && hc->dst, hc ? hc->n : 0, tailAsked ? hc->tailY0 : 0,
+                                           tailAsked ? hc->tailN : 0);
     if (!pl.ok) return hipErrorNotSupported;
     if (k.trace) {
         char line[512];
@@ -196,18 +200,22 @@
         x.hn = hc->n;
         hc->done = true;
     }
+    if (pl.tailN > 0) x.tail = static_cast<float*>(hc->tail);
     const int64_t blocks = pl.nblocks;
     if (pl.kernel == HxsKernel::Hxt) {
+        hipError_t e = hipErrorNotSupported;
         switch (p.NS) {
-#define GAR_HXT_NS(n) case n: return hxtFmt<n>(x, pl.lds, blocks, stream, pl.lean);
+#define GAR_HXT_NS(n) case n: e = hxtFmt<n>(x, pl.lds, blocks, stream, pl.lean); break;
 #if !GAR_HXS_QUICK
             GAR_HXT_NS(1) GAR_HXT_NS(2) GAR_HXT_NS(3) GAR_HXT_NS(4) GAR_HXT_NS(5) GAR_HXT_NS(6) GAR_HXT_NS(7)
             GAR_HXT_NS(8)
 #endif
             GAR_HXT_NS(9) GAR_HXT_NS(10)
 #undef GAR_HXT_NS
-            default: return hipErrorNotSupported;
+            default: break;
         }
+        if (e == hipSuccess && pl.tailN > 0) hc->tailDone = true;
+        return e;
     }
     switch (p.NS) {
 #define GAR_HXS_NS(n) case n: return hxsVst<n>(x, pl.lds, blocks, stream);
diff --git a/go-audio-resampler_amd/csrc/gar_hxs.hpp b/go-audio-resampler_amd/csrc/gar_hxs.hpp
--- a/go-audio-resampler_amd/csrc/gar_hxs.hpp
+++ b/go-audio-resampler_amd/csrc/gar_hxs.hpp
@@ -40,6 +40,8 @@
     int out_pcm;
     float* hdst;
     int64_t ht0, hn;
+    float* tail;
+    int64_t tailHi, a_hiT;
     char* out;
     int64_t out_fs, out_cs;
     int out_f64;
@@ -111,11 +113,15 @@
     return y;
 }
 
+__device__ __forceinline__ void hxsTailStore(float* tail, int64_t o_hi, int C, int64_t o, int c, float v) {
+    tail[(o - o_hi) * C + c] = v;
+}
+
 __device__ __forceinline__ void hxsFixup(HxsArgsP xp, int b, const int* loudLo, const int* loudHi) {
     const SrcDesc src = kload(&xp->src);
     const OutDesc od = kload(&xp->od);
     const int Pc = xp->Pc, Qc = xp->Qc, Np = xp->Np, C = xp->C, ncols = xp->ncols;
-    const int64_t a_lo = xp->a_lo, a_hi = xp->a_hi;
+    const int64_t a_lo = xp->a_lo, a_hi = xp->a_hiT, tailHi = xp->tailHi;
     for (int j = 0; j < 16; ++j) {
         const int lo = loudLo[j], hi = loudHi[j];
         const int col = b * 16 + j;
@@ -128,13 +134,16 @@
             const int64_t a = a_lo + static_cast<int64_t>(k) * Np + p;
             if (a >= a_hi) continue;
             const int64_t o = a * Pc + r;
-            if (o < od.o_lo || o >= od.o_hi) continue;
+            if (o < od.o_lo || o >= tailHi) continue;
             const int w0 = p * Qc + xp->rowOff[r], w1 = w0 + xp->rowLen[r];
             if (w1 <= lo || w0 > hi) continue;
             const int64_t t0 = a * Qc + xp->rowOff[r];
             bool loud = false;
             for (int kk = 0; kk < w1 - w0 && !loud; ++kk) loud = hxLoud(srcRead<float>(src, t0 + kk, c));
-            if (loud) outWrite<float>(od, o, c, static_cast<float>(hxsExact(xp, a, r, c)));
+            if (!loud) continue;
+            const float v = static_cast<float>(hxsExact(xp, a, r, c));
+            if (o >= od.o_hi) hxsTailStore(xp->tail, od.o_hi, C, o, c, v);
+            else outWrite<float>(od, o, c, v);
         }
     }
 }
diff --git a/go-audio-resampler_amd/csrc/gar_hxs_launch.cpp b/go-audio-resampler_amd/csrc/gar_hxs_launch.cpp
--- a/go-audio-resampler_amd/csrc/gar_hxs_launch.cpp
+++ b/go-audio-resampler_amd/csrc/gar_hxs_launch.cpp
@@ -35,6 +35,7 @@
     {"GAR_HXT_WIDE", &HxsKnobs::wide, kInt, true},
     {"GAR_HXT_LEAN", &HxsKnobs::lean, kInt, true},
     {"GAR_HXT_FAULT", &HxsKnobs::fault, kIsOne, true},
+    {"GAR_HXT_TAILFOLD", &HxsKnobs::tailFold, kInt, true},
 };
 
 void readKnobs(HxsKnobs& k, bool perLaunchOnly) {
@@ -243,6 +244,13 @@
     return 1;
 }
 
+int64_t foldTail(const HxDev& p, const HxsLaunchPlan& pl, const OutDesc& od, int64_t tailY0, int64_t tailN, const HxsKnobs& k) {
+    if (k.tailFold == 0 || tailN <= 0 || pl.kernel != HxsKernel::Hxt || tailY0 != od.o_hi || pl.a_hi <= pl.a_lo) return 0;
+    const int64_t chunk = (pl.a_hi - 1 - pl.a_lo) / pl.Np;
+    const int64_t aEnd = pl.a_lo + (chunk + 1) * pl.Np;
+    return ceilDiv(od.o_hi + tailN, p.Pc) <= aEnd ? tailN : 0;
+}
+
 }
 
 bool hxsPlanFits(const HxDev& p) {
@@ -250,8 +258,14 @@
     return hxsRingFits(p.Qc, 1, hxsRingFor(p.Qc, p.Kread, 1).Rt);
 }
 
+bool hxsTailFoldPossible(const HxDev& p, int64_t o_lo, int64_t o_hi, int C, int ncu) {
+    const HxsKnobs k = hxsLaunchKnobs();
+    if (k.tailFold == 0 || !p.rb || o_hi <= o_lo) return false;
+    return !isSmall(ceilDiv(o_hi, p.Pc) - floorDiv(o_lo, p.Pc), C, ncu > 0 ? ncu : 256, k);
+}
+
 HxsLaunchPlan hxsPlanLaunch(const HxDev& p, const SrcDesc& src, const OutDesc& od, int C, int ncu, const HxsKnobs& k,
-                            bool histKeep, int64_t histN) {
+                            bool histKeep, int64_t histN, int64_t tailY0, int64_t tailN) {
     HxsLaunchPlan pl;
     if (!p.rb || p.nw > kHxRbMaxWaves || !hxsNsBuilt(p.NS)) return pl;
     pl.a_lo = floorDiv(od.o_lo, p.Pc);
@@ -305,6 +319,7 @@
     pl.kernel = c.hxt ? HxsKernel::Hxt : pl.qRbs ? HxsKernel::Hxq : window ? HxsKernel::HxsSmall : HxsKernel::Hxs;
     pl.lds = pl.fmt == kFmtRow32 ? hxtLdsWide(pl.Rt) : hxsLds(pl.Rt);
     pl.histFolded = histKeep && histN > 0;
+    pl.tailN = foldTail(p, pl, od, tailY0, tailN, k);
     return pl;
 }
 
diff --git a/go-audio-resampler_amd/csrc/gar_hxs_launch.hpp b/go-audio-resampler_amd/csrc/gar_hxs_launch.hpp
--- a/go-audio-resampler_amd/csrc/gar_hxs_launch.hpp
+++ b/go-audio-resampler_amd/csrc/gar_hxs_launch.hpp
@@ -28,6 +28,7 @@
     int wide = 1;
     int lean = 1;
     int fault = 0;
+    int tailFold = 1;
 };
 HxsKnobs hxsReadKnobs();
 HxsKnobs hxsLaunchKnobs();
@@ -54,10 +55,12 @@
     int qRbs = 0, qGroups = 0, qOpt = 0;
     size_t lds = 0;
     bool histFolded = false;
+    int64_t tailN = 0;
 };
 
 HxsLaunchPlan hxsPlanLaunch(const HxDev& p, const SrcDesc& src, const OutDesc& od, int C, int ncu, const HxsKnobs& k,
-                            bool histKeep, int64_t histN);
+                            bool histKeep, int64_t histN, int64_t tailY0 = 0, int64_t tailN = 0);
+bool hxsTailFoldPossible(const HxDev& p, int64_t o_lo, int64_t o_hi, int C, int ncu);
 int hxsTraceLines(const HxsLaunchPlan& pl, const OutDesc& od, int C, char* buf, size_t cap);
 
 }
diff --git a/go-audio-resampler_amd/csrc/gar_hxt.hpp b/go-audio-resampler_amd/csrc/gar_hxt.hpp
--- a/go-audio-resampler_amd/csrc/gar_hxt.hpp
+++ b/go-audio-resampler_amd/csrc/gar_hxt.hpp
@@ -625,7 +625,7 @@
             const int ccol_ = ccol + 16 * h;
             const int64_t a = aCol + p;
             const int64_t o0 = a * x.Pc + oRow0;
-            const bool live = colOk && a < x.a_hi;
+            const bool live = colOk && a < x.a_hiT;
             if (fullRb && live && a * x.Pc >= x.o_lo && (a + 1) * x.Pc <= x.o_hi) {
                 char* pp = x.out + (o0 + ((VST == 2 && (lane & 1)) ? 2 : 0)) * x.out_fs + (VST == 2 ? 0 : ccol_ * x.out_cs);
                 hxsStoreFast<VST>(x, pp, y, lane);
@@ -635,6 +635,8 @@
                     const int64_t o = o0 + i;
                     if (oRow0 + i < x.Pc && o >= x.o_lo && o < x.o_hi)
                         *reinterpret_cast<float*>(x.out + o * x.out_fs + ccol_ * x.out_cs) = y[i];
+                    else if (oRow0 + i < x.Pc && o >= x.o_hi && o < x.tailHi)
+                        hxsTailStore(x.tail, x.o_hi, x.C, o, ccol_, y[i]);
                 }
             }
         }
diff --git a/go-audio-resampler_amd/csrc/gar_kernels.hpp b/go-audio-resampler_amd/csrc/gar_kernels.hpp
--- a/go-audio-resampler_amd/csrc/gar_kernels.hpp
+++ b/go-audio-resampler_amd/csrc/gar_kernels.hpp
@@ -24,6 +24,7 @@
     int pcm;
     int64_t o_lo, o_hi;
     int* err;
+    int ncu;
 };
 
 constexpr int kSampPcm24P = 280;
@@ -177,6 +178,9 @@
     void* dst = nullptr;
     int64_t t0 = 0, n = 0;
     bool done = false;
+    void* tail = nullptr;
+    int64_t tailY0 = 0, tailN = 0;
+    bool tailDone = false;
 };
 
 hipError_t launchBg(const BgDev& p, const SrcDesc& src, const OutDesc& out, int C, hipStream_t stream,
diff --git a/go-audio-resampler_amd/gar/__init__.py b/go-audio-resampler_amd/gar/__init__.py
--- a/go-audio-resampler_amd/gar/__init__.py
+++ b/go-audio-resampler_amd/gar/__init__.py
@@ -81,7 +81,7 @@
     "gar_status_string", "gar_last_error", "gar_design_engine", "gar_design_composite", "gar_profile_enable",
     "gar_profile_read", "gar_stage_state", "gar_num_stages", "gar_stage_geometry", "gar_get_statistics",
     "gar_synchronize", "gar_profile_launch_stats", "gar_profile_kinds", "gar_dev_half_convert",
-    "gar_dev_pcm24_convert", "gar_dev_hxs_plan",
+    "gar_dev_pcm24_convert", "gar_dev_hxs_plan", "gar_dev_hxs_fold", "gar_dev_flush_tail",
 ]
 
 _lib = None
@@ -145,6 +145,9 @@
         "gar_dev_pcm24_convert": (i32, [vp, i64, vp, vp]),
         "gar_dev_hxs_plan": (i32, [vp, i32, i32, i64, i64, C.c_uint64, i64, i64, i64, C.c_uint64, i64, i64, i32, C.c_uint64,
                                    i64, i64, i64, i64, i64, i32, i32, i64, C.c_char_p, i64]),
+        "gar_dev_hxs_fold": (i32, [vp, i32, i32, i64, i64, C.c_uint64, i64, i64, i64, C.c_uint64, i64, i64, i32, C.c_uint64,
+                                   i64, i64, i64, i64, i64, i32, i32, i64, i64, i64, C.POINTER(i64)]),
+        "gar_dev_flush_tail": (i32, [vp, i32, C.POINTER(i64), C.POINTER(i32)]),
     }
     ab = os.environ.get("GAR_LIB_PATH") is not None
     for name, (res, args) in sig.items():
@@ -453,6 +456,22 @@
     return buf.value.decode()
 
 
+def flush_tail(r, stage=0):
+    n, q = C.c_int64(0), C.c_int32(0)
+    _check(lib().gar_dev_flush_tail(r._h, int(stage), C.byref(n), C.byref(q)))
+    return n.value, bool(q.value)
+
+
+def hxs_fold(r, tail_y0, tail_n, in_type, in_fs, in_cs, in_addr, in_base, in_len, valid_end, hist_addr, hist_len, hist_ld,
+             out_type, out_addr, o0, out_fs, out_cs, o_lo, o_hi, channels, cu_count, hist_keep=0, stage=0):
+    n = C.c_int64(0)
+    _check(lib().gar_dev_hxs_fold(r._h, int(stage), int(in_type), int(in_fs), int(in_cs), int(in_addr), int(in_base),
+                                  int(in_len), int(valid_end), int(hist_addr), int(hist_len), int(hist_ld), int(out_type),
+                                  int(out_addr), int(o0), int(out_fs), int(out_cs), int(o_lo), int(o_hi), int(channels),
+                                  int(cu_count), int(hist_keep), int(tail_y0), int(tail_n), C.byref(n)))
+    return n.value
+
+
 def New(config):
     if config is None:
         raise ErrInvalidConfig("config is nil")
diff --git a/include/gar.h b/include/gar.h
--- a/include/gar.h
+++ b/include/gar.h
@@ -131,6 +131,14 @@
                             int64_t out_fs, int64_t out_cs, int64_t o_lo, int64_t o_hi, int32_t channels,
                             int32_t cu_count, int64_t hist_keep, char *buf, int64_t cap);
 
+gar_status gar_dev_hxs_fold(const gar_resampler *r, int32_t stage, int32_t in_type, int64_t in_fs, int64_t in_cs,
+                            uint64_t in_addr, int64_t in_base, int64_t in_len, int64_t valid_end, uint64_t hist_addr,
+                            int64_t hist_len, int64_t hist_ld, int32_t out_type, uint64_t out_addr, int64_t o0,
+                            int64_t out_fs, int64_t out_cs, int64_t o_lo, int64_t o_hi, int32_t channels,
+                            int32_t cu_count, int64_t hist_keep, int64_t tail_y0, int64_t tail_n, int64_t *folded);
+
+gar_status gar_dev_flush_tail(const gar_resampler *r, int32_t stage, int64_t *tail_n, int32_t *quirk);
+
 typedef struct gar_engine_geometry {
     int32_t kind;
     int32_t dft_factor, dft_taps;
```
